# onolab-tmu/overiva

Hardware: AMD Instinct MI355X
Metric: AuxIVA iterations/sec (2048 bins x 4000 frames x 8 mics) (higher is better)
Workload: dtype f32

## Files before the change

### include/overiva_hip.h

```cpp
#ifndef OVERIVA_HIP_H
#define OVERIVA_HIP_H

#ifdef __cplusplus
extern "C" {
#endif

#define OIVA_OK 0
#define OIVA_ERR_ARG (-1)
#define OIVA_ERR_HIP (-2)
#define OIVA_ERR_STATE (-3)
#define OIVA_ERR_NUMERIC (-4)

#define OIVA_MODEL_LAPLACE 0
#define OIVA_MODEL_GAUSS 1

#define OIVA_MAX_CHANNELS 32

#define OIVA_PREC_FAST 0
#define OIVA_PREC_UPDATE_F64 1
#define OIVA_PREC_UPDATE_ROWS 2
#define OIVA_PREC_COV_F64 4
#define OIVA_PREC_PRECISE (OIVA_PREC_UPDATE_F64 | OIVA_PREC_COV_F64)

typedef struct oiva_plan oiva_plan;

int oiva_version(void);
const char *oiva_last_error(void);
int oiva_device_count(int *n);

int oiva_plan_create(oiva_plan **out, int device, int T, int F, int M, int K, int model, int F_total,
                     void *stream);
int oiva_plan_destroy(oiva_plan *p);

int oiva_plan_set_x_host(oiva_plan *p, const void *X, long long row_pitch_bytes);
int oiva_plan_set_x_dev(oiva_plan *p, const void *X_dev);
int oiva_plan_set_x_host_c128(oiva_plan *p, const void *X, long long row_pitch_bytes);

int oiva_plan_covariance(oiva_plan *p);
int oiva_plan_get_cx(oiva_plan *p, void *Cx_host, int f64);

int oiva_plan_set_w(oiva_plan *p, const void *W0_host, int f64);

int oiva_plan_iterate(oiva_plan *p, int n);

int oiva_plan_power(oiva_plan *p);
int oiva_plan_power_buffer(oiva_plan *p, int parts_per_rank, void **parts_dev, long long *bytes);
int oiva_plan_update(oiva_plan *p, const void *parts_dev, int nparts);

int oiva_plan_demix(oiva_plan *p, void *Y_host, long long row_pitch_bytes, int proj_back);
int oiva_pool_trim(void);
int oiva_plan_set_io_slab(oiva_plan *p, long long bytes);
int oiva_host_prefault(void *ptr, long long bytes);
int oiva_plan_demix_dev(oiva_plan *p, int proj_back, void **Y_dev);
int oiva_plan_demix_c128(oiva_plan *p, void *Y_host, long long row_pitch_bytes, int proj_back);

#define OIVA_XCHG_MAX_RANKS 16
#define OIVA_XCHG_HANDLE_BYTES 64
typedef struct oiva_xchg oiva_xchg;
int oiva_xchg_create(oiva_xchg **x, int device, int rank, int world, long long part_bytes);
int oiva_xchg_export(oiva_xchg *x, void *handle);
int oiva_xchg_connect(oiva_xchg *x, const void *handles);
int oiva_xchg_push(oiva_xchg *x, void *stream, const void *part_dev, long long part_bytes, int epoch);
int oiva_xchg_wait(oiva_xchg *x, void *stream, int epoch);
int oiva_xchg_gathered(oiva_xchg *x, int epoch, void **gathered);
int oiva_xchg_poll(oiva_xchg *x, int epoch, int timeout_ms, int *arrived);
int oiva_xchg_force(oiva_xchg *x, int epoch);
int oiva_xchg_destroy(oiva_xchg *x);

int oiva_plan_set_w_pca(oiva_plan *p, double *evals_host);
int oiva_plan_set_w_eig(oiva_plan *p);
int oiva_plan_get_w(oiva_plan *p, void *W_host, int f64);

int oiva_plan_sync(oiva_plan *p);
int oiva_plan_save_w(oiva_plan *p);
int oiva_plan_restore_w(oiva_plan *p);

int oiva_plan_iterate_timed(oiva_plan *p, int n, float *total_ms, float *per_kernel_ms);
#define OIVA_N_STAGES 4

int oiva_plan_get_cov_splits(oiva_plan *p, int *nsplit);
int oiva_plan_set_cov_splits(oiva_plan *p, int nsplit);
int oiva_plan_set_cov_quad(oiva_plan *p, int enable, int *active);
int oiva_plan_set_pow_splits(oiva_plan *p, int nsplit);
int oiva_plan_set_cov_hmfma(oiva_plan *p, int enable);
int oiva_plan_set_fuse_cov_update(oiva_plan *p, int enable, int *active);
int oiva_plan_set_power_reverse(oiva_plan *p, int enable);
int oiva_plan_use_graph(oiva_plan *p, int enable);
int oiva_plan_set_precision(oiva_plan *p, int flags);

struct oiva_xchg;
#define OIVA_RESIDENT_INFO 12
#define OIVA_RESIDENT_PHASES 8
int oiva_plan_set_resident(oiva_plan *p, int enable);
int oiva_plan_resident_info(oiva_plan *p, int *info );
int oiva_plan_resident_phases(oiva_plan *p, double *phase_us , int *n_iter);
int oiva_plan_resident_debug(oiva_plan *p, int timeout_ms, int stall_block);
int oiva_plan_resident_debug_from(oiva_plan *p, int timeout_ms, int stall_block, int first_stalled_iteration);
int oiva_plan_resident_loopback(oiva_plan *p, int world);
#define OIVA_RESIDENT_STAMPS 16
int oiva_plan_resident_trace(oiva_plan *p, int enable, unsigned long long *stamps_host, int *n_wg, int *n_iter);
int oiva_plan_resident_connect(oiva_plan *p, struct oiva_xchg *x);
int oiva_plan_fused_connect(oiva_plan *p, struct oiva_xchg *x);
int oiva_plan_fused_loopback(oiva_plan *p, int world);
int oiva_plan_fused_debug(oiva_plan *p, int timeout_ms, int stall);
int oiva_plan_set_resident_splits(oiva_plan *p, int nsplit);

int oiva_test_set_rinv(oiva_plan *p, const float *rinv_host );
int oiva_test_get_rinv(oiva_plan *p, float *rinv_host , float *wscale_host );
int oiva_test_run_weighted_cov(oiva_plan *p);
int oiva_test_get_v(oiva_plan *p, void *V_host , int f64);
int oiva_test_run_update(oiva_plan *p);
int oiva_test_get_what(oiva_plan *p, void *What_host , int f64);
int oiva_test_set_what(oiva_plan *p, const void *What_host, int f64);
int oiva_test_run_power(oiva_plan *p, float *p_host );
int oiva_test_get_ppart(oiva_plan *p, float *parts_host, int *nparts);
int oiva_test_power_order(int nsplit, int tcp, int cov_splits, int cov_tc, int *order);
int oiva_test_time_stage(oiva_plan *p, int stage, int reps, float *avg_ms);
int oiva_test_live_buffers(long long *count, long long *bytes);
int oiva_test_kernel_choice(int device, int T, int F, int F_total, int M, int K, int prec_flags, int quad_on, int hmfma_on,
                            int cov_splits_req, int pow_splits_req, int *out);

#define OIVA_OGIVE_DEMIX 0
#define OIVA_OGIVE_MIX 1
#define OIVA_OGIVE_SWITCHING 2
int oiva_plan_ogive_begin(oiva_plan *p, int update_mode, int model);
int oiva_plan_ogive_iterate(oiva_plan *p, int first_epoch, int n, double step_size, double tol, int *epochs_run,
                            int *converged, double *max_delta);

typedef struct oiva_batch oiva_batch;
int oiva_batch_create(oiva_batch **out, int device, int B, int T, int F, int M, int K, int model, void *stream);
int oiva_batch_destroy(oiva_batch *b);
int oiva_batch_set_x_host(oiva_batch *b, const void *X_host, int f64);
int oiva_batch_set_x_dev(oiva_batch *b, const void *X_dev);
int oiva_batch_covariance(oiva_batch *b);
int oiva_batch_set_w(oiva_batch *b, const void *W0_host, int f64);
int oiva_batch_set_w_eig(oiva_batch *b);
int oiva_batch_iterate(oiva_batch *b, int n);
int oiva_batch_demix(oiva_batch *b, void *Y_host, int f64, int proj_back);
int oiva_batch_get_w(oiva_batch *b, void *W_host, int f64);
int oiva_batch_status(oiva_batch *b, int *status);
int oiva_batch_time_stages(oiva_batch *b, int n, float *total_ms, float *per_stage_ms);

typedef int oiva_status;
oiva_status oiva_batch_get_cx(oiva_batch *b, void *Cx_host, int f64);
oiva_status oiva_batch_ogive_begin(oiva_batch *b, int update_mode, int model);
oiva_status oiva_batch_ogive_iterate(oiva_batch *b, int first_epoch, int n, double step_size, double tol, int *epochs_run,
                                     int *converged, double *max_delta);

oiva_status oiva_batch_create_ragged(oiva_batch **out, int device, int B, const int *frames, int F, int M, int K, int model,
                                     void *stream);

oiva_status oiva_batch_set_w_pca(oiva_batch *b, double *evals_host);
oiva_status oiva_batch_project_dev(oiva_batch *b, void **Xr_dev);
oiva_status oiva_batch_compose_w(oiva_batch *outer, const oiva_batch *inner);

enum {
    OIVA_ILRMA_STAGE_T = 0,
    OIVA_ILRMA_STAGE_V = 1,
    OIVA_ILRMA_STAGE_R = 2,
    OIVA_ILRMA_STAGE_COV = 3,
    OIVA_ILRMA_STAGE_UPDATE = 4,
    OIVA_ILRMA_STAGE_POWER = 5,
    OIVA_ILRMA_STAGE_NORMALISE = 6
};
oiva_status oiva_batch_ilrma_begin(oiva_batch *b, int n_components, const double *T0, const double *V0);
oiva_status oiva_batch_ilrma_stage(oiva_batch *b, int stage);
oiva_status oiva_batch_ilrma_iterate(oiva_batch *b, int n);
oiva_status oiva_batch_ilrma_get_nmf(oiva_batch *b, double *T, double *V);
oiva_status oiva_batch_ilrma_get_pr(oiva_batch *b, double *P, double *R);
oiva_status oiva_batch_ilrma_get_cov(oiva_batch *b, double *C, double *lambda);
oiva_status oiva_batch_ilrma_time_stages(oiva_batch *b, int n, float *per_stage_ms);

typedef struct oiva_stft oiva_stft;
int oiva_stft_create(oiva_stft **out, int device, int n_samples, int n_chan, int frame, int hop, const float *win_a,
                     const float *win_s);
int oiva_stft_destroy(oiva_stft *p);
int oiva_stft_shape(oiva_stft *p, int *n_frames, int *n_freq);
int oiva_stft_analysis(oiva_stft *p, const float *x_host, void *X_host, void **X_dev);
int oiva_stft_synthesis(oiva_stft *p, const void *Y_host, int n_chan, float *y_host);

typedef struct oiva_bstft oiva_bstft;
oiva_status oiva_bstft_create(oiva_bstft **out, int device, int B, const int *n_samples, int M, int frame, int hop,
                              const float *win_a, const float *win_s, void *stream);
oiva_status oiva_bstft_destroy(oiva_bstft *p);
oiva_status oiva_bstft_shape(oiva_bstft *p, int *frames, int *n_freq);
oiva_status oiva_bstft_analysis(oiva_bstft *p, const float *x_host_packed, void **X_dev);
oiva_status oiva_bstft_synthesis_dev(oiva_bstft *p, const void *Y_dev, int K, float *y_host_packed);
oiva_status oiva_bstft_phase_ms(oiva_bstft *p, float *ms);
oiva_status oiva_batch_demix_dev(oiva_batch *b, int proj_back, void **Y_dev);
oiva_status oiva_device_to_host(void *host, const void *dev, long long bytes);

typedef struct oiva_bsseval oiva_bsseval;
oiva_status oiva_bsseval_create(oiva_bsseval **out, int device, int B, const int *n_samples, int N, int filter_length,
                                int diag_only, int max_group, void *stream);
oiva_status oiva_bsseval_destroy(oiva_bsseval *p);
oiva_status oiva_bsseval_groups(oiva_bsseval *p, int *rooms_per_group);
oiva_status oiva_bsseval_set_signals(oiva_bsseval *p, const double *ref_host_packed, const double *est_host_packed);
oiva_status oiva_bsseval_stage(oiva_bsseval *p, int stage);
oiva_status oiva_bsseval_run(oiva_bsseval *p);
oiva_status oiva_bsseval_get_gram(oiva_bsseval *p, double *G_host, double *D_host, double *E_host);
oiva_status oiva_bsseval_get_filters(oiva_bsseval *p, double *C_host, double *c_host);
oiva_status oiva_bsseval_get_criteria(oiva_bsseval *p, double *sdr, double *sir, double *sar);
oiva_status oiva_bsseval_status(oiva_bsseval *p, int *status);
oiva_status oiva_bsseval_time_stages(oiva_bsseval *p, int n, float *per_stage_ms);

#ifdef __cplusplus
}
#endif
#endif
```

### overiva_amd/_lib.py

```python
import ctypes as C
import os

import numpy as np

_PKG = os.path.dirname(os.path.abspath(__file__))
LIB_PATH = os.environ.get("OIVA_LIB") or os.path.join(_PKG, "liboveriva_hip.so")

OK, ERR_ARG, ERR_HIP, ERR_STATE, ERR_NUMERIC = 0, -1, -2, -3, -4
MODEL_IDS = {"laplace": 0, "gauss": 1}
N_STAGES = 4
PREC_FAST, PREC_UPDATE_F64, PREC_UPDATE_ROWS, PREC_COV_F64 = 0, 1, 2, 4
PREC_PRECISE = PREC_UPDATE_F64 | PREC_COV_F64
PREC_MIXED = PREC_UPDATE_F64
PREC_BY_NAME = {"fast": PREC_FAST, "mixed": PREC_MIXED, "precise": PREC_PRECISE}
STAGE_NAMES = ("demix_power", "activation", "weighted_cov", "ip_update")


class HipLibraryMissing(ImportError):
    pass


class HipError(RuntimeError):
    """a HIP runtime call failed inside the library"""


_lib = None

_vp, _i, _ll, _fp = C.c_void_p, C.c_int, C.c_longlong, C.POINTER(C.c_float)

SIGNATURES = {
    "oiva_device_count": [C.POINTER(_i)],
    "oiva_plan_create": [C.POINTER(_vp), _i, _i, _i, _i, _i, _i, _i, _vp],
    "oiva_plan_destroy": [_vp],
    "oiva_plan_set_x_host": [_vp, _vp, _ll],
    "oiva_plan_set_x_dev": [_vp, _vp],
    "oiva_plan_set_x_host_c128": [_vp, _vp, _ll],
    "oiva_plan_covariance": [_vp],
    "oiva_plan_get_cx": [_vp, _vp, _i],
    "oiva_plan_set_w": [_vp, _vp, _i],
    "oiva_plan_iterate": [_vp, _i],
    "oiva_plan_power": [_vp],
    "oiva_plan_power_buffer": [_vp, _i, C.POINTER(_vp), C.POINTER(_ll)],
    "oiva_plan_update": [_vp, _vp, _i],
    "oiva_plan_demix": [_vp, _vp, _ll, _i],
    "oiva_plan_demix_dev": [_vp, _i, _vp],
    "oiva_plan_set_io_slab": [_vp, _ll],
    "oiva_host_prefault": [_vp, _ll],
    "oiva_pool_trim": [],
    "oiva_plan_demix_c128": [_vp, _vp, _ll, _i],
    "oiva_plan_set_w_pca": [_vp, _vp],
    "oiva_plan_set_w_eig": [_vp],
    "oiva_xchg_create": [_vp, _i, _i, _i, _ll],
    "oiva_xchg_export": [_vp, _vp],
    "oiva_xchg_connect": [_vp, _vp],
    "oiva_xchg_push": [_vp, _vp, _vp, _ll, _i],
    "oiva_xchg_wait": [_vp, _vp, _i],
    "oiva_xchg_gathered": [_vp, _i, _vp],
    "oiva_xchg_poll": [_vp, _i, _i, _vp],
    "oiva_xchg_force": [_vp, _i],
    "oiva_xchg_destroy": [_vp],
    "oiva_plan_get_w": [_vp, _vp, _i],
    "oiva_plan_sync": [_vp],
    "oiva_plan_save_w": [_vp],
    "oiva_plan_restore_w": [_vp],
    "oiva_plan_iterate_timed": [_vp, _i, _fp, _fp],
    "oiva_plan_get_cov_splits": [_vp, C.POINTER(_i)],
    "oiva_plan_set_cov_splits": [_vp, _i],
    "oiva_plan_set_cov_quad": [_vp, _i, C.POINTER(_i)],
    "oiva_plan_set_pow_splits": [_vp, _i],
    "oiva_plan_set_cov_hmfma": [_vp, _i],
    "oiva_plan_set_fuse_cov_update": [_vp, _i, C.POINTER(_i)],
    "oiva_plan_set_power_reverse": [_vp, _i],
    "oiva_plan_use_graph": [_vp, _i],
    "oiva_plan_set_precision": [_vp, _i],
    "oiva_plan_set_resident": [_vp, _i],
    "oiva_plan_resident_info": [_vp, C.POINTER(_i)],
    "oiva_plan_resident_phases": [_vp, C.POINTER(C.c_double), C.POINTER(_i)],
    "oiva_plan_resident_debug": [_vp, _i, _i],
    "oiva_plan_resident_debug_from": [_vp, _i, _i, _i],
    "oiva_plan_resident_loopback": [_vp, _i],
    "oiva_plan_fused_connect": [_vp, _vp],
    "oiva_plan_fused_loopback": [_vp, _i],
    "oiva_plan_fused_debug": [_vp, _i, _i],
    "oiva_plan_resident_connect": [_vp, _vp],
    "oiva_plan_resident_trace": [_vp, _i, _vp, C.POINTER(_i), C.POINTER(_i)],
    "oiva_plan_set_resident_splits": [_vp, _i],
    "oiva_test_set_rinv": [_vp, _vp],
    "oiva_test_get_rinv": [_vp, _vp, _vp],
    "oiva_test_run_weighted_cov": [_vp],
    "oiva_test_get_v": [_vp, _vp, _i],
    "oiva_test_run_update": [_vp],
    "oiva_test_get_what": [_vp, _vp, _i],
    "oiva_test_set_what": [_vp, _vp, _i],
    "oiva_test_run_power": [_vp, _vp],
    "oiva_test_get_ppart": [_vp, _vp, C.POINTER(_i)],
    "oiva_test_power_order": [_i, _i, _i, _i, C.POINTER(_i)],
    "oiva_test_time_stage": [_vp, _i, _i, _fp],
    "oiva_test_live_buffers": [C.POINTER(C.c_longlong), C.POINTER(C.c_longlong)],
    "oiva_test_kernel_choice": [_i] * 11 + [C.POINTER(_i)],
    "oiva_plan_ogive_begin": [_vp, _i, _i],
    "oiva_plan_ogive_iterate": [_vp, _i, _i, C.c_double, C.c_double, C.POINTER(_i), C.POINTER(_i), C.POINTER(C.c_double)],
    "oiva_batch_create": [C.POINTER(_vp), _i, _i, _i, _i, _i, _i, _i, _vp],
    "oiva_batch_destroy": [_vp],
    "oiva_batch_set_x_host": [_vp, _vp, _i],
    "oiva_batch_set_x_dev": [_vp, _vp],
    "oiva_batch_covariance": [_vp],
    "oiva_batch_set_w": [_vp, _vp, _i],
    "oiva_batch_set_w_eig": [_vp],
    "oiva_batch_iterate": [_vp, _i],
    "oiva_batch_demix": [_vp, _vp, _i, _i],
    "oiva_batch_get_w": [_vp, _vp, _i],
    "oiva_batch_status": [_vp, C.POINTER(_i)],
    "oiva_batch_time_stages": [_vp, _i, _fp, _fp],
    "oiva_batch_get_cx": [_vp, _vp, _i],
    "oiva_batch_ogive_begin": [_vp, _i, _i],
    "oiva_batch_ogive_iterate": [_vp, _i, _i, C.c_double, C.c_double, C.POINTER(_i), C.POINTER(_i), C.POINTER(C.c_double)],
    "oiva_batch_create_ragged": [C.POINTER(_vp), _i, _i, C.POINTER(_i), _i, _i, _i, _i, _vp],
    "oiva_batch_set_w_pca": [_vp, _vp],
    "oiva_batch_project_dev": [_vp, C.POINTER(_vp)],
    "oiva_batch_compose_w": [_vp, _vp],
    "oiva_batch_ilrma_begin": [_vp, _i, _vp, _vp],
    "oiva_batch_ilrma_stage": [_vp, _i],
    "oiva_batch_ilrma_iterate": [_vp, _i],
    "oiva_batch_ilrma_get_nmf": [_vp, _vp, _vp],
    "oiva_batch_ilrma_get_pr": [_vp, _vp, _vp],
    "oiva_batch_ilrma_get_cov": [_vp, _vp, _vp],
    "oiva_batch_ilrma_time_stages": [_vp, _i, _fp],
    "oiva_stft_create": [C.POINTER(_vp), _i, _i, _i, _i, _i, _vp, _vp],
    "oiva_stft_destroy": [_vp],
    "oiva_stft_shape": [_vp, C.POINTER(_i), C.POINTER(_i)],
    "oiva_stft_analysis": [_vp, _vp, _vp, C.POINTER(_vp)],
    "oiva_stft_synthesis": [_vp, _vp, _i, _vp],
    "oiva_bstft_create": [C.POINTER(_vp), _i, _i, C.POINTER(_i), _i, _i, _i, _vp, _vp, _vp],
    "oiva_bstft_destroy": [_vp],
    "oiva_bstft_shape": [_vp, C.POINTER(_i), C.POINTER(_i)],
    "oiva_bstft_analysis": [_vp, _vp, C.POINTER(_vp)],
    "oiva_bstft_synthesis_dev": [_vp, _vp, _i, _vp],
    "oiva_bstft_phase_ms": [_vp, _fp],
    "oiva_batch_demix_dev": [_vp, _i, C.POINTER(_vp)],
    "oiva_device_to_host": [_vp, _vp, _ll],
    "oiva_bsseval_create": [C.POINTER(_vp), _i, _i, C.POINTER(_i), _i, _i, _i, _i, _vp],
    "oiva_bsseval_destroy": [_vp],
    "oiva_bsseval_groups": [_vp, C.POINTER(_i)],
    "oiva_bsseval_set_signals": [_vp, _vp, _vp],
    "oiva_bsseval_stage": [_vp, _i],
    "oiva_bsseval_run": [_vp],
    "oiva_bsseval_get_gram": [_vp, _vp, _vp, _vp],
    "oiva_bsseval_get_filters": [_vp, _vp, _vp],
    "oiva_bsseval_get_criteria": [_vp, _vp, _vp, _vp],
    "oiva_bsseval_status": [_vp, C.POINTER(_i)],
    "oiva_bsseval_time_stages": [_vp, _i, _fp],
}


def load():
    global _lib
    if _lib is not None:
        return _lib
    try:
        import torch
    except ImportError:
        pass
    if not os.path.exists(LIB_PATH):
        raise HipLibraryMissing(
            f"{LIB_PATH} not found: the HIP extension is not built.  Run `python -m overiva_amd.build` "
            "(needs hipcc).  overiva_amd has no CPU fallback.")
    try:
        lib = C.CDLL(LIB_PATH)
    except OSError as e:
        raise HipLibraryMissing(f"cannot load {LIB_PATH}: {e}") from e
    lib.oiva_version.restype = C.c_int
    lib.oiva_version.argtypes = []
    lib.oiva_last_error.restype = C.c_char_p
    lib.oiva_last_error.argtypes = []
    for name, args in SIGNATURES.items():
        fn = getattr(lib, name)
        fn.restype = C.c_int
        fn.argtypes = args
    _lib = lib
    return lib


def require_dmabuf_ipc(what):
    import warnings

    cur = os.environ.get("HSA_ENABLE_IPC_MODE_LEGACY")
    why = None
    if cur is None or _IPC_ENV_SET_LATE:
        os.environ["HSA_ENABLE_IPC_MODE_LEGACY"] = "0"
        try:
            import torch

            started = torch.cuda.is_initialized()
        except Exception:
            started = False
        if (started and cur is None) or _IPC_ENV_SET_LATE:
            why = (f"{what}: HSA_ENABLE_IPC_MODE_LEGACY=0 was not in the environment when the GPU runtime started; "
                   "exporting device memory to other processes may fail (import overiva_amd, or export the variable, before "
                   "the first GPU call)")
    elif cur != "0":
        why = f"{what}: HSA_ENABLE_IPC_MODE_LEGACY={cur!r}; this platform's driver supports dmabuf IPC (=0) only"
    if why:
        warnings.warn(why)
    return why


_IPC_ENV_SET_LATE = False


def _set_ipc_env_at_import():
    global _IPC_ENV_SET_LATE
    if "HSA_ENABLE_IPC_MODE_LEGACY" in os.environ:
        return
    os.environ["HSA_ENABLE_IPC_MODE_LEGACY"] = "0"
    import sys

    t = sys.modules.get("torch")
    try:
        _IPC_ENV_SET_LATE = bool(t is not None and t.cuda.is_initialized())
    except Exception:
        _IPC_ENV_SET_LATE = False


def check(rc):
    if rc == OK:
        return
    msg = load().oiva_last_error().decode("utf-8", "replace")
    if rc == ERR_ARG:
        raise ValueError(msg)
    if rc == ERR_NUMERIC:
        raise np.linalg.LinAlgError(msg)
    if rc == ERR_STATE:
        raise RuntimeError(msg)
    raise HipError(msg)


class Handle:

    h = None
    _destroy = None

    def close(self):
        if self.h:
            getattr(self.lib, self._destroy)(self.h)
            self.h = None

    def __del__(self):
        try:
            self.close()
        except Exception:
            pass

    def __enter__(self):
        return self

    def __exit__(self, *exc):
        self.close()


def ptr(a):
    assert a.flags["C_CONTIGUOUS"]
    return a.ctypes.data_as(C.c_void_p)
```

### overiva_amd/csrc/kernel_choice.h

```cpp
#pragma once
#include <algorithm>
#include <functional>

#include "overiva_hip.h"

namespace oiva {

inline int ceil_div(int a, int b) { return (a + b - 1) / b; }
inline int round_up(int a, int b) { return (a + b - 1) / b * b; }

constexpr int kNarrowMax = 16;
constexpr int kWideMax = OIVA_MAX_CHANNELS;

constexpr int kBinsPerWave = 16;
constexpr int kPhasesPerWave = 4;
constexpr int kBlock = 256;
constexpr int kWaves = kBlock / 64;

enum class CovKind { Lane, Pair32, Pair64, Quad, Half16, Hmfma, Half16F64, Hmfma64, Mfma, Wide };
enum class PowKind { Lane, Mfma, Lds, Wide };
constexpr int kCovKinds = 10, kPowKinds = 4;
static_assert((int)CovKind::Wide + 1 == kCovKinds && (int)PowKind::Wide + 1 == kPowKinds, "one traits row per kind");

struct CovGeom {
    int nsplit;
    int tc;
    int kc;
    int nbg;
    CovKind kind = CovKind::Lane;
    int pad = 0;
    int part32 = 0;
};
constexpr int kPowOrderMaxSplits = 64;
struct PowOrder {
    int cs = 0;
    int q = 0;
    int first[kPowOrderMaxSplits + 1] = {};
};
inline PowOrder make_pow_order(int n, int tcp, int cs, int ctc) {
    PowOrder o;
    if (cs < 1 || cs > kPowOrderMaxSplits || ctc < 1 || tcp < 1 || n < 1) return o;
    o.cs = cs;
    for (int s = 0; s < cs; ++s) {
        const long long c = (long long)s * ctc / tcp;
        o.first[s] = c < n ? (int)c : n;
    }
    o.first[cs] = n;
    o.q = n;
    for (int s = 0; s < cs; ++s) o.q = o.first[s + 1] - o.first[s] < o.q ? o.first[s + 1] - o.first[s] : o.q;
    return o;
}
struct PowGeom {
    int nb;
    int nsplit;
    int tcp;
    int kp;
    PowKind kind = PowKind::Lane;
    int rev = 0;
    PowOrder ord{};
    int rounds = 1;
};
constexpr int kPowMaxFrames = 512;

enum class Partials { F64, Acc, F32IfPart32 };
struct CovTraits {
    bool (*supported)(int M, int K);
    int (*sources)(int K);
    int bins;
    int quantum;
    Partials partials;
    int launches;
    bool padded_x;
    bool quad_switch;
    bool fusable;
    bool update_arith;
    CovKind unit;
};
constexpr CovTraits kCovTraits[kCovKinds] = {
     {[](int M, int K) { return M >= 1 && M <= 8 && K >= 1 && K <= M; }, nullptr, kBinsPerWave, 16, Partials::F64, 1, false, false, true, false, CovKind::Lane},
     {[](int M, int K) { return M == 8 && K >= 3; }, [](int) { return 4; }, 32, 8, Partials::F64, 2, false, false, false, true, CovKind::Pair32},
     {[](int M, int) { return M == 8; }, [](int K) { return K >= 2 ? 2 : 1; }, 32, 8, Partials::F64, 2, false, false, false, false, CovKind::Pair64},
     {[](int M, int K) { return M >= 10 && M <= 16 && M % 2 == 0 && K >= 1 && K <= 4; }, [](int K) { return K >= 2 ? 2 : 1; }, kBinsPerWave, 8, Partials::F64, 2, true, true, false, true, CovKind::Quad},
     {[](int M, int K) { return M >= 10 && M <= 16 && M % 2 == 0 && K >= 1 && K <= 16; }, [](int K) { return K <= 8 ? 8 : (K <= 12 ? 12 : 16); }, 2, 16, Partials::F64, 2, true, true, false, true, CovKind::Half16},
     {[](int M, int K) { return M >= 10 && M <= 16 && M % 2 == 0 && K >= 9 && K <= 16; }, [](int K) { return K <= 8 ? 8 : (K <= 12 ? 12 : 16); }, 2, 32, Partials::F32IfPart32, 2, true, true, false, true, CovKind::Half16},
     {[](int M, int K) { return M >= 10 && M <= 16 && M % 2 == 0 && K >= 3 && K <= 16; }, [](int K) { return K <= 4 ? 4 : 8; }, 2, 16, Partials::F64, 2, true, true, false, true, CovKind::Mfma},
     {[](int M, int K) { return M == 16 && K >= 9 && K <= 16; }, [](int K) { return K <= 4 ? 4 : 8; }, 2, 32, Partials::F64, 2, true, true, false, true, CovKind::Mfma},
     {[](int M, int K) { return M >= 9 && M <= 16 && K >= 1 && K <= M; }, [](int) { return 1; }, kBinsPerWave, 4, Partials::Acc, 2, false, false, false, true, CovKind::Mfma},
     {[](int M, int K) { return M > kNarrowMax && M <= kWideMax && K >= 1 && K <= M; }, [](int K) { return std::min(K, 2); }, 1, 4, Partials::F64, 2, false, false, false, true, CovKind::Wide},
};
constexpr const CovTraits& traits(CovKind k) { return kCovTraits[(int)k]; }
constexpr bool partials_f64(const CovGeom& g, bool cov_f64) {
    return traits(g.kind).partials == Partials::F64 || (traits(g.kind).partials == Partials::Acc ? cov_f64 : !g.part32);
}

struct PowTraits {
    bool (*supported)(int M, int K);
    int (*sources)(int K);
    int bins;
    int quantum;
    bool padded_x;
    bool occupancy;
};
constexpr int pow_sources_per_pass(int , int K) {
    return K >= 3 ? 4 : (K >= 2 ? 2 : 1);
}
constexpr PowTraits kPowTraits[kPowKinds] = {
     {[](int M, int K) { return M >= 1 && M <= kNarrowMax && K >= 1 && K <= M && (M <= 8 || K <= 4); }, [](int K) { return pow_sources_per_pass(0, K); }, kBinsPerWave * kWaves, 4, false, true},
     {[](int M, int K) { return M > 8 && M <= kNarrowMax && K > 4 && K <= M; }, [](int K) { return pow_sources_per_pass(0, K); }, kBinsPerWave * kWaves, 4, true, false},
     {[](int M, int K) { return M == 16 && K > 4 && K <= M; }, [](int K) { return pow_sources_per_pass(0, K); }, kBinsPerWave * kWaves, 4, false, false},
     {[](int M, int K) { return M > kNarrowMax && M <= kWideMax && K >= 1 && K <= M; }, [](int K) { return K >= 3 ? 4 : K; }, kBinsPerWave * kWaves, 4, false, false},
};
constexpr const PowTraits& traits(PowKind k) { return kPowTraits[(int)k]; }

struct ChoiceIn {
    int T, F, F_total, M, K;
    int n_cu;
    bool cov_f64, upd_f64;
    bool cov_quad_on = true;
    bool cov_hmfma_on = true;
    bool part32 = false;
    bool kc_wide = true;
    bool power_lds = true;
};
struct Occupancy {
    std::function<int(int M, int kc, bool f64)> cov_blocks_per_cu;
    std::function<int(int M, int kp, int tcp)> pow_blocks_per_cu;
};

inline int lane_sources_per_pass(int M, int K, bool f64, bool short_axis, bool kc_wide) {
    const int regs = M * M * (f64 ? 2 : 1);
    int kc = 1;
    if (K >= 2 && regs * 2 <= 144) kc = 2;
    if (K >= 3 && regs * 4 <= 144) kc = 4;
    if (!f64 && kc_wide) {
        if (M == 7 && (K == 3 || K == 5 || K == 6 || (K == 7 && short_axis))) kc = 3;
        if (M == 5 && K >= 5) kc = 5;
    }
    return kc;
}

inline int pick_splits(int capacity, int blocks_per_split, int T, int min_frames) {
    int ns = std::max(1, capacity / std::max(1, blocks_per_split));
    ns = std::min(ns, std::max(1, T / std::max(1, min_frames)));
    return ns;
}

inline int mixed_min_splits(int capacity, int blocks_per_split, int T) {
    if (T >= 1024) return 8;
    const int one_round = std::max(1, capacity / std::max(1, blocks_per_split));
    return std::max(1, std::min(std::min(4, one_round), T / 16));
}

constexpr bool padded_channels(int M) { return M > 8 && M <= kNarrowMax && M % 2 == 1; }

inline CovKind choose_cov_kind(const ChoiceIn& c) {
    const int M = c.M, K = c.K;
    if (M > kNarrowMax) return CovKind::Wide;
    if (M <= 8) {
        if (!c.cov_f64 && traits(CovKind::Pair32).supported(M, K)) return CovKind::Pair32;
        if (c.cov_f64 && traits(CovKind::Pair64).supported(M, K)) return CovKind::Pair64;
        return CovKind::Lane;
    }
    const int Mc = M + (padded_channels(M) ? 1 : 0);
    if (!c.cov_f64 && c.cov_quad_on && traits(CovKind::Quad).supported(Mc, K) && (K <= 2 || c.upd_f64)) return CovKind::Quad;
    if (c.cov_quad_on && (c.cov_f64 ? traits(CovKind::Half16F64).supported(Mc, K) : K > 4 && traits(CovKind::Half16).supported(Mc, K))) {
        const CovKind hm = c.cov_f64 ? CovKind::Hmfma64 : CovKind::Hmfma;
        if (c.cov_hmfma_on && traits(hm).supported(Mc, K)) return hm;
        return c.cov_f64 ? CovKind::Half16F64 : CovKind::Half16;
    }
    return CovKind::Mfma;
}

inline CovGeom choose_cov(const ChoiceIn& c, const Occupancy& occ, int nsplit_req) {
    CovGeom g{};
    g.kind = choose_cov_kind(c);
    const CovTraits& t = traits(g.kind);
    const int T = c.T, F = c.F, K = c.K, n_cu = c.n_cu;
    g.pad = padded_channels(c.M) ? 1 : 0;
    g.nbg = ceil_div(F, t.bins);
    g.kc = t.sources ? t.sources(K) : lane_sources_per_pass(c.M, K, c.cov_f64, T < 1024, c.kc_wide);
    int nsplit = nsplit_req;
    switch (g.kind) {
        case CovKind::Wide:
            if (nsplit <= 0) {
                const int groups = c.F_total * ceil_div(K, g.kc);
                nsplit = 1;
                while (groups * nsplit < 2 * n_cu && ceil_div(T, nsplit + 1) >= 128) ++nsplit;
            }
            break;
        case CovKind::Quad:
            if (nsplit <= 0) {
                const int blocks = g.nbg * ceil_div(K, g.kc);
                nsplit = std::min(32, pick_splits(n_cu * 2, blocks, T, T >= 1024 ? 128 : 64));
                if (c.upd_f64) nsplit = std::max(nsplit, mixed_min_splits(n_cu * 2, blocks, T));
            }
            break;
        case CovKind::Half16:
        case CovKind::Hmfma:
        case CovKind::Half16F64:
        case CovKind::Hmfma64: {
            const bool hm = g.kind == CovKind::Hmfma || g.kind == CovKind::Hmfma64;
            if (nsplit <= 0) {
                const int chains = hm ? 8 : 4;
                nsplit = c.cov_f64 ? (!hm && g.kc == 4 && T >= 1024 ? 2 : 1) : ceil_div(T, chains * (c.upd_f64 ? 128 : 256));
                const int per_cu = hm ? (c.cov_f64 ? 2 : 3) : c.cov_f64 && g.kc == 4 ? 4 : 2;
                const int groups = hm ? F : g.nbg * ceil_div(K, g.kc);
                while (groups * nsplit < per_cu * n_cu && ceil_div(T, nsplit + 1) >= 64) ++nsplit;
            }
            if (t.partials == Partials::F32IfPart32) g.part32 = c.part32 ? 1 : 0;
            break;
        }
        case CovKind::Mfma:
            if (nsplit <= 0) {
                nsplit = ceil_div(T, 512);
                const int waves = F * ceil_div(K, 4);
                while (waves * nsplit < 2 * 4 * n_cu && ceil_div(T, nsplit + 1) >= 64) ++nsplit;
            }
            break;
        case CovKind::Lane:
        case CovKind::Pair32:
        case CovKind::Pair64:
            if (nsplit <= 0) {
                const int nz = ceil_div(K, g.kc);
                int bpc = 2;
                if (g.kind == CovKind::Lane && (bpc = occ.cov_blocks_per_cu(c.M, g.kc, c.cov_f64)) < 1) bpc = 2;
                nsplit = pick_splits(n_cu * bpc, g.nbg * nz, T, T >= 1024 ? 128 : 64);
                if (nsplit >= 12 && g.nbg * nz * nsplit >= n_cu * bpc) nsplit = nsplit * 7 / 8;
                const int cap = (g.nbg * nz * 32 >= n_cu) ? 32 : 64;
                nsplit = std::min(nsplit, cap);
                if (g.kind == CovKind::Pair32 && c.upd_f64) {
                    const int by_chain = T >= 1024 ? 8 : std::min(4, ceil_div(T, 256));
                    nsplit = std::max(nsplit, std::min(by_chain, mixed_min_splits(n_cu * bpc, g.nbg * nz, T)));
                }
            }
            break;
    }
    g.tc = round_up(ceil_div(T, nsplit), t.quantum);
    g.nsplit = ceil_div(T, g.tc);
    return g;
}

inline PowKind choose_pow_kind(const ChoiceIn& c) {
    if (c.M > kNarrowMax) return PowKind::Wide;
    if (!traits(PowKind::Mfma).supported(c.M, c.K)) return PowKind::Lane;
    if (c.power_lds && traits(PowKind::Lds).supported(c.M, c.K) && c.F >= kBinsPerWave * kWaves && c.T >= 16) return PowKind::Lds;
    return PowKind::Mfma;
}

inline PowGeom choose_pow(const ChoiceIn& c, const Occupancy& occ, int nsplit_req) {
    PowGeom g{};
    g.kind = choose_pow_kind(c);
    const PowTraits& t = traits(g.kind);
    const int T = c.T, n_cu = c.n_cu;
    g.nb = ceil_div(c.F, t.bins);
    g.kp = t.sources(c.K);
    int nsplit = nsplit_req;
    if (g.kind == PowKind::Wide) {
        const int groups = g.nb * ceil_div(c.K, g.kp);
        if (nsplit <= 0) nsplit = pick_splits(n_cu * 4, groups, T, 16);
        g.tcp = round_up(ceil_div(T, nsplit), t.quantum);
        g.nsplit = ceil_div(T, g.tcp);
        return g;
    }
    if (nsplit <= 0) {
        const int per_cu_x12 = (g.kp == 1 && c.M <= 8) ? 24 : 12;
        nsplit = pick_splits(std::max(n_cu / 2, n_cu * per_cu_x12 / std::max(c.M, 1)), g.nb, T, 32);
    }
    int tcp = round_up(ceil_div(T, nsplit), t.quantum);
    tcp = std::min(std::max(tcp, 4), kPowMaxFrames);
    g.tcp = tcp;
    g.nsplit = ceil_div(T, tcp);
    if (t.occupancy) {
        const int bpc = occ.pow_blocks_per_cu(c.M, g.kp, g.tcp);
        if (bpc > 0) g.rounds = (int)((((long long)g.nb * g.nsplit * ceil_div(c.K, g.kp)) + (long long)bpc * n_cu - 1) / ((long long)bpc * n_cu));
    }
    return g;
}

}
```

### overiva_amd/csrc/kernels_cov.hip

```cpp

#include <cstdint>
#include <cstdlib>

#include "oiva_device.h"
#include "cov_arith.h"

namespace oiva {
namespace {

constexpr int kCovUnroll = 2;
constexpr int kChunk = 16;
constexpr int kLdsStride = kBlock + 1;

template <int M, int KC, typename ACC, typename At>
__device__ __forceinline__ void reduce_and_store_at(At&& at, ACC* lds, double* __restrict__ Vpart, int F, int K, int k0) {
    constexpr int NA = M * M;
    constexpr int NACC = NA * KC;
    const int tid = threadIdx.x;
    const int bb = tid >> 4, aa = tid & 15;
    const int fo = blockIdx.x * kBinsPerWave + bb;
    double* out = Vpart + (((size_t)blockIdx.y * F + fo) * K + k0) * NA;
#pragma unroll
    for (int r0 = 0; r0 < NACC; r0 += kChunk) {
        __syncthreads();
#pragma unroll
        for (int a = 0; a < kChunk; ++a) {
            if (r0 + a < NACC) lds[a * kLdsStride + tid] = at(r0 + a);
        }
        __syncthreads();
        double s = 0.;
#pragma unroll
        for (int qq = 0; qq < 16; ++qq) s += (double)lds[aa * kLdsStride + qq * 16 + bb];
        const int e = r0 + aa;
        const int kk = e / NA;
        if (e < NACC && fo < F && k0 + kk < K) out[e] = s;
    }
}

template <int M, int KC, typename ACC>
__device__ __forceinline__ void reduce_and_store(const ACC (&acc)[KC][M * M], ACC* lds, double* __restrict__ Vpart,
                                                 int F, int K, int k0) {
    reduce_and_store_at<M, KC, ACC>([&](int e) { return acc[e / (M * M)][e % (M * M)]; }, lds, Vpart, F, K, k0);
}

template <int M, int KC, bool UNIT, typename ACC>
__global__ __launch_bounds__(kBlock) void cov_kernel(const float2* __restrict__ X, const float* __restrict__ R,
                                                     float* __restrict__ wscale, int model, int raw,
                                                     double* __restrict__ Vpart, int T, int F, int K, int tc) {
    constexpr int NA = M * M;
    __shared__ ACC lds[kChunk * kLdsStride];

    const int tid = threadIdx.x;
    const int lane = tid & 63;
    const int wave = tid >> 6;
    const int b = lane & (kBinsPerWave - 1);
    const int q = wave * kPhasesPerWave + (lane >> 4);
    const int f = blockIdx.x * kBinsPerWave + b;
    const int fc = f < F ? f : F - 1;
    const int k0 = blockIdx.z * KC;
    const int t_begin = blockIdx.y * tc;
    const int t_end = min(T, t_begin + tc);
    const int nsteps = (t_end - t_begin + 15) >> 4;

    double ginv[KC];
#pragma unroll
    for (int kk = 0; kk < KC; ++kk) ginv[kk] = 1.;
    if constexpr (!UNIT) {
#pragma unroll
        for (int kk = 0; kk < KC; ++kk) {
            const int k = k0 + kk;
            if (raw & 1) continue;
            const double gamma = gamma_of(R, T, K, k < K ? k : K - 1);
            ginv[kk] = 1. / gamma;
            if (blockIdx.x == 0 && blockIdx.y == 0 && threadIdx.x == 0 && k < K && wscale != nullptr)
                wscale[k] = model == OIVA_MODEL_LAPLACE ? (float)gamma : (float)sqrt(gamma);
        }
    }

    ACC acc[KC][NA];
#pragma unroll
    for (int kk = 0; kk < KC; ++kk)
#pragma unroll
        for (int a = 0; a < NA; ++a) acc[kk][a] = 0;

    const size_t frame_stride = (size_t)F * M;
    const float2* pbase = X + (size_t)fc * M;
    for (int i = 0; i < nsteps; i += kCovUnroll) {
        float xr[kCovUnroll][M], xi[kCovUnroll][M], rv[kCovUnroll][KC];
#pragma unroll
        for (int u = 0; u < kCovUnroll; ++u) {
            const int t = t_begin + q + 16 * (i + u);
            const int tcl = t < t_end ? t : T - 1;
            if constexpr (!UNIT) {
#pragma unroll
                for (int kk = 0; kk < KC; ++kk) {
                    const int k = k0 + kk;
                    rv[u][kk] = R[(size_t)tcl * K + (k < K ? k : K - 1)];
                }
            }
            load_x<M>(pbase + (size_t)tcl * frame_stride, xr[u], xi[u]);
        }
#pragma unroll
        for (int u = 0; u < kCovUnroll; ++u) {
            const int t = t_begin + q + 16 * (i + u);
            const bool live = t < t_end;
            ACC w[KC], ar[M], ai[M];
#pragma unroll
            for (int kk = 0; kk < KC; ++kk) {
                const bool on = live && (UNIT || k0 + kk < K);
                if constexpr (UNIT) {
                    w[kk] = on ? ACC(1) : ACC(0);
                } else if constexpr (sizeof(ACC) == 8) {
                    double rn = (double)rv[u][kk] * ginv[kk];
                    rn = rn < (double)kEpsR ? (double)kEpsR : rn;
                    w[kk] = on ? 1. / rn : 0.;
                } else {
                    w[kk] = on ? activation_weight(rv[u][kk], (float)ginv[kk]) : 0.f;
                }
            }
#pragma unroll
            for (int c = 0; c < M; ++c) {
                ar[c] = (ACC)xr[u][c];
                ai[c] = (ACC)xi[u][c];
            }
            accumulate<M, KC, UNIT, ACC>(acc, ar, ai, w);
        }
    }

    reduce_and_store<M, KC, ACC>(acc, lds, Vpart, F, K, k0);
}

constexpr int kDmaStages = 4;

typedef __attribute__((address_space(1))) const void gvoid_t;
typedef __attribute__((address_space(3))) void lvoid_t;

template <int PIECES>
__device__ __forceinline__ void ring_read(unsigned addr, float4 (&v)[PIECES]);

template <>
__device__ __forceinline__ void ring_read<4>(unsigned addr, float4 (&v)[4]) {
    asm volatile(
        "s_waitcnt vmcnt(12)\n\t"
        "ds_read_b128 %0, %4\n\t"
        "ds_read_b128 %1, %4 offset:1024\n\t"
        "ds_read_b128 %2, %4 offset:2048\n\t"
        "ds_read_b128 %3, %4 offset:3072\n\t"
        "s_waitcnt lgkmcnt(0)"
        : "=&v"(v[0]), "=&v"(v[1]), "=&v"(v[2]), "=&v"(v[3])
        : "v"(addr)
        : "memory");
}
template <>
__device__ __forceinline__ void ring_read<2>(unsigned addr, float4 (&v)[2]) {
    asm volatile(
        "s_waitcnt vmcnt(6)\n\t"
        "ds_read_b128 %0, %2\n\t"
        "ds_read_b128 %1, %2 offset:1024\n\t"
        "s_waitcnt lgkmcnt(0)"
        : "=&v"(v[0]), "=&v"(v[1])
        : "v"(addr)
        : "memory");
}

#ifdef OIVA_COVDMA_TRACE
__device__ long long g_cd_trace[8 * 2048];
#define CD_STAMP(slot)                                                                                                            \
    do {                                                                                                                          \
        if (threadIdx.x == 0 && blockIdx.z == 0) g_cd_trace[(blockIdx.y * gridDim.x + blockIdx.x) * 8 + (slot)] = wall_clock64(); \
    } while (0)
#else
#define CD_STAMP(slot) \
    do {               \
    } while (0)
#endif

template <int M, int KC>
__global__ __launch_bounds__(kBlock, 2) void cov_dma_kernel(const float2* __restrict__ X, const float* __restrict__ R,
                                                            float* __restrict__ wscale, int model, int raw,
                                                            double* __restrict__ Vpart, int T, int F, int K, int tc) {
    constexpr int NA = M * M;
    constexpr int PIECES = M / 2;
    constexpr int STAGE = PIECES * 64;
    static_assert(M % 2 == 0 && (PIECES == 2 || PIECES == 4), "LDS-DMA path: M in {4, 8}");
    __shared__ float4 ring[kWaves * kDmaStages * STAGE];
    static_assert(sizeof(float4) * kWaves * kDmaStages * STAGE >= sizeof(float) * kChunk * kLdsStride,
                  "reduction scratch aliases the ring");

    const int tid = threadIdx.x;
    const int lane = tid & 63;
    const int wave = __builtin_amdgcn_readfirstlane(tid >> 6);
    const int b = lane & (kBinsPerWave - 1);
    const int ql = lane >> 4;
    const int q = wave * kPhasesPerWave + ql;
    const int f = blockIdx.x * kBinsPerWave + b;
    const int fc = f < F ? f : F - 1;
    const int k0 = blockIdx.z * KC;
    const int t_begin = blockIdx.y * tc;
    const int t_end = min(T, t_begin + tc);
    const int nsteps = (t_end - t_begin + 15) >> 4;

    constexpr bool kPacked = KC == 2;
    float acc[kPacked ? 1 : KC][kPacked ? 1 : NA];
    PkAcc2<M> pacc;
    if constexpr (kPacked) {
        pacc.clear();
    } else {
#pragma unroll
        for (int kk = 0; kk < KC; ++kk)
#pragma unroll
            for (int a = 0; a < NA; ++a) acc[kk][a] = 0.f;
    }

    float ginv[KC];
    float4* wring = ring + wave * kDmaStages * STAGE;
    const unsigned rd_base = (unsigned)(uintptr_t)(wring) + lane * 16;
    const size_t frame_stride = (size_t)F * M;
    const float2* pbase = X + (size_t)fc * M;

    auto issue = [&](int i, int s) {
        const int t = t_begin + q + 16 * i;
        const int tcl = (i < nsteps && t < t_end) ? t : T - 1;
        const float2* src = pbase + (size_t)tcl * frame_stride;
#pragma unroll
        for (int j = 0; j < PIECES; ++j)
            __builtin_amdgcn_global_load_lds((gvoid_t*)(src + 2 * j), (lvoid_t*)(wring + s * STAGE + j * 64), 16, 0, 0);
    };
    const float m0 = ql == 0 ? 1.f : 0.f, m1 = ql == 1 ? 1.f : 0.f, m2 = ql == 2 ? 1.f : 0.f, m3 = ql == 3 ? 1.f : 0.f;
    auto consume = [&](int i, int s) {
        const int tw = min(t_begin + wave * kPhasesPerWave + 16 * i, T);
        const float* rp = R + (size_t)tw * K;
        float w[KC];
#pragma unroll
        for (int kk = 0; kk < KC; ++kk) {
            const int k = k0 + kk < K ? k0 + kk : K - 1;
            const float r = m0 * rp[k] + m1 * rp[K + k] + m2 * rp[2 * K + k] + m3 * rp[3 * K + k];
            const float live = (t_begin + wave * kPhasesPerWave + 16 * i + ql < t_end && k0 + kk < K) ? 1.f : 0.f;
            w[kk] = activation_weight(r, ginv[kk]) * live;
        }
        float4 v[PIECES];
        ring_read<PIECES>(rd_base + s * STAGE * 16, v);
#if defined(OIVA_COVDMA_ABLATE) && (OIVA_COVDMA_ABLATE & 1)
        if constexpr (kPacked) {
            if (v[0].x == 12345.f) pacc.add(reinterpret_cast<const v2f(&)[M]>(v), v2f{w[0], w[1]});
            return;
        }
#endif
        if constexpr (kPacked) {
            v2f x[M];
#pragma unroll
            for (int j = 0; j < PIECES; ++j) {
                x[2 * j] = v2f{v[j].x, v[j].y};
                x[2 * j + 1] = v2f{v[j].z, v[j].w};
            }
            pacc.add(x, v2f{w[0], w[1]});
        } else {
            float xr[M], xi[M];
#pragma unroll
            for (int j = 0; j < PIECES; ++j) {
                xr[2 * j] = v[j].x;
                xi[2 * j] = v[j].y;
                xr[2 * j + 1] = v[j].z;
                xi[2 * j + 1] = v[j].w;
            }
            accumulate<M, KC, false, float>(acc, xr, xi, w);
        }
    };

    CD_STAMP(0);
    issue(0, 0);
    issue(1, 1);
    issue(2, 2);
#pragma unroll
    for (int kk = 0; kk < KC; ++kk) {
        const int k = k0 + kk;
        ginv[kk] = 1.f;
        if (raw & 1) continue;
#if defined(OIVA_COVDMA_ABLATE) && (OIVA_COVDMA_ABLATE & 4)
        const float gamma = R[k < K ? k : K - 1] + 1.f;
#else
        const float gamma = (float)gamma_of(R, T, K, k < K ? k : K - 1);
#endif
        ginv[kk] = 1.f / gamma;
        if (blockIdx.x == 0 && blockIdx.y == 0 && threadIdx.x == 0 && k < K && wscale != nullptr)
            wscale[k] = model == OIVA_MODEL_LAPLACE ? gamma : sqrtf(gamma);
    }

    CD_STAMP(1);
    int i = 0;
    for (; i + 4 <= nsteps; i += 4) {
        issue(i + 3, 3); consume(i, 0);
        issue(i + 4, 0); consume(i + 1, 1);
        issue(i + 5, 1); consume(i + 2, 2);
        issue(i + 6, 2); consume(i + 3, 3);
    }
    if (i < nsteps) { issue(i + 3, 3); consume(i, 0); }
    if (i + 1 < nsteps) { issue(i + 4, 0); consume(i + 1, 1); }
    if (i + 2 < nsteps) { issue(i + 5, 1); consume(i + 2, 2); }
    CD_STAMP(2);
    asm volatile("s_waitcnt vmcnt(0)" ::: "memory");
    CD_STAMP(3);
#if defined(OIVA_COVDMA_ABLATE) && (OIVA_COVDMA_ABLATE & 2)
    if constexpr (kPacked) {
        if (pacc.at(0) == 12345.f) Vpart[0] = 1.;
        return;
    }
#endif
    if constexpr (kPacked)
        reduce_and_store_at<M, KC, float>([&](int e) { return pacc.at(e); }, reinterpret_cast<float*>(ring), Vpart, F, K, k0);
    else
        reduce_and_store<M, KC, float>(acc, reinterpret_cast<float*>(ring), Vpart, F, K, k0);
    CD_STAMP(4);
}

template <typename ACC>
using CovKernel = void (*)(const float2*, const float*, float*, int, int, double*, int, int, int, int);

template <int M, typename ACC, typename Fn>
hipError_t dispatch_kc(int kc, bool unit, Fn&& fn) {
    constexpr int kRegs = M * M * (int)(sizeof(ACC) / 4);
    if (unit) return kc == 1 ? fn((CovKernel<ACC>)cov_kernel<M, 1, true, ACC>, 1) : hipErrorInvalidValue;
    if constexpr ((M == 4 || M == 8) && sizeof(ACC) == 4) {
        switch (kc) {
            case 1:
                return fn((CovKernel<ACC>)cov_dma_kernel<M, 1>, 1);
            case 2:
                if constexpr (kRegs * 2 <= 144) return fn((CovKernel<ACC>)cov_dma_kernel<M, 2>, 2);
                break;
            case 4:
                if constexpr (kRegs * 4 <= 144) return fn((CovKernel<ACC>)cov_dma_kernel<M, 4>, 4);
                break;
        }
        return hipErrorInvalidValue;
    }
    switch (kc) {
        case 1:
            return fn((CovKernel<ACC>)cov_kernel<M, 1, false, ACC>, 1);
        case 2:
            if constexpr (kRegs * 2 <= 144) return fn((CovKernel<ACC>)cov_kernel<M, 2, false, ACC>, 2);
            break;
        case 4:
            if constexpr (kRegs * 4 <= 144) return fn((CovKernel<ACC>)cov_kernel<M, 4, false, ACC>, 4);
            break;
        case 3:
            if constexpr (M == 7 && sizeof(ACC) == 4) return fn((CovKernel<ACC>)cov_kernel<M, 3, false, ACC>, 3);
            break;
        case 5:
            if constexpr (M == 5 && sizeof(ACC) == 4) return fn((CovKernel<ACC>)cov_kernel<M, 5, false, ACC>, 5);
            break;
    }
    return hipErrorInvalidValue;
}

template <typename ACC, typename Fn>
hipError_t dispatch_cov(int M, int kc, bool unit, Fn&& fn) {
    switch (M) {
        case 1: return dispatch_kc<1, ACC>(kc, unit, fn);
        case 2: return dispatch_kc<2, ACC>(kc, unit, fn);
        case 3: return dispatch_kc<3, ACC>(kc, unit, fn);
        case 4: return dispatch_kc<4, ACC>(kc, unit, fn);
        case 5: return dispatch_kc<5, ACC>(kc, unit, fn);
        case 6: return dispatch_kc<6, ACC>(kc, unit, fn);
        case 7: return dispatch_kc<7, ACC>(kc, unit, fn);
        case 8: return dispatch_kc<8, ACC>(kc, unit, fn);
    }
    return hipErrorInvalidValue;
}

}

__global__ __launch_bounds__(kBlock) void pad_channels_kernel(const float2* __restrict__ X, float2* __restrict__ Xpad, long long n, int M) {
    const long long e = (long long)blockIdx.x * kBlock + threadIdx.x;
    if (e >= n) return;
    const long long tf = e / (M + 1);
    const int c = (int)(e - tf * (M + 1));
    Xpad[e] = c < M ? X[tf * M + c] : make_float2(0.f, 0.f);
}

hipError_t launch_pad_channels(hipStream_t s, const float2* X, float2* Xpad, long long n_tf, int M) {
    const long long n = n_tf * (M + 1);
    pad_channels_kernel<<<dim3((unsigned)((n + kBlock - 1) / kBlock)), dim3(kBlock), 0, s>>>(X, Xpad, n, M);
    return hipGetLastError();
}

hipError_t launch_cov(hipStream_t s, const float2* X, const float2* Xpad, const float* R, float* Wt, float* wscale, int model, int raw,
                      void* Vpart, bool f64, int T, int F, int M, int K, const CovGeom& g) {
    const CovTraits& t = traits(g.kind);
    if (g.tc % t.quantum != 0 || (g.pad && Xpad == nullptr)) return hipErrorInvalidValue;
    const float2* Xv = g.pad && t.padded_x ? Xpad : X;
    const int Mp = g.pad && t.padded_x ? M + 1 : M;
    double* const V64 = static_cast<double*>(Vpart);
    switch (g.kind) {
        case CovKind::Wide: return launch_cov_wide(s, X, R, Wt, wscale, model, raw, V64, T, F, M, K, g);
        case CovKind::Half16: return launch_cov_half16(s, Xv, R, Wt, wscale, model, raw, V64, T, F, Mp, M, K, g);
        case CovKind::Hmfma: {
            const hipError_t e = launch_cov_half16_weights(s, R, Wt, wscale, model, raw, T, K);
            return e != hipSuccess ? e : launch_cov_hmfma(s, Xv, Wt, V64, T, F, Mp, M, K, g);
        }
        case CovKind::Half16F64: return launch_cov_half16_f64(s, Xv, R, Wt, wscale, model, raw, V64, T, F, Mp, M, K, g);
        case CovKind::Hmfma64: {
            const hipError_t e = launch_cov_half16_weights_f64(s, R, Wt, wscale, model, raw, T, K);
            return e != hipSuccess ? e : launch_cov_hmfma64(s, Xv, reinterpret_cast<const double*>(Wt), V64, T, F, Mp, M, K, g);
        }
        case CovKind::Quad: return launch_cov_quad(s, Xv, R, Wt, wscale, model, raw, V64, T, F, Mp, M, K, g);
        case CovKind::Mfma: return launch_cov_mfma(s, X, R, Wt, wscale, model, raw, Vpart, f64, T, F, M, K, g.nsplit, g.tc);
        case CovKind::Pair32: return launch_cov_pair32(s, X, R, Wt, wscale, model, raw, V64, T, F, M, K, g);
        case CovKind::Pair64: return launch_cov_pair64(s, X, R, Wt, wscale, model, raw, V64, T, F, M, K, g);
        case CovKind::Lane: break;
    }
    const int kc = R == nullptr ? 1 : g.kc;
    if (f64)
        return dispatch_cov<double>(M, kc, R == nullptr, [&](CovKernel<double> kern, int KC) {
            kern<<<dim3(g.nbg, g.nsplit, (K + KC - 1) / KC), dim3(kBlock), 0, s>>>(X, R, wscale, model, raw,
                                                                                 static_cast<double*>(Vpart), T, F, K, g.tc);
            return hipGetLastError();
        });
    return dispatch_cov<float>(M, kc, R == nullptr, [&](CovKernel<float> kern, int KC) {
        return launch_dominant(kern, dim3(g.nbg, g.nsplit, (K + KC - 1) / KC), dim3(kBlock), 0, s, X, R, wscale, model, raw,
                               static_cast<double*>(Vpart), T, F, K, g.tc);
    });
}

hipError_t cov_blocks_per_cu(int M, int kc, bool f64, int* n) {
    if (f64)
        return dispatch_cov<double>(M, kc, false, [&](CovKernel<double> kern, int) {
            return hipOccupancyMaxActiveBlocksPerMultiprocessor(n, kern, kBlock, 0);
        });
    return dispatch_cov<float>(M, kc, false, [&](CovKernel<float> kern, int) {
        return hipOccupancyMaxActiveBlocksPerMultiprocessor(n, kern, kBlock, 0);
    });
}

#ifdef OIVA_COVDMA_TRACE
extern "C" int oiva_debug_covdma_trace(long long* out) { return (int)hipMemcpyFromSymbol(out, HIP_SYMBOL(g_cd_trace), sizeof(g_cd_trace)); }
#endif

}
```

### overiva_amd/csrc/kernels_demix.hip

```cpp
#include "oiva_device.h"
#include "demix_arith.h"

namespace oiva {
namespace {

constexpr int kPowUnroll = 2;

template <int M, int KP>
__global__ __launch_bounds__(kBlock) void power_kernel(const float2* __restrict__ X, const float2* __restrict__ What,
                                                       float* __restrict__ Ppart, int T, int F, int K, int tcp, int rev, PowOrder ord) {
    extern __shared__ __attribute__((aligned(16))) float sp[];
    const int tid = threadIdx.x;
    const int lane = tid & 63;
    const int wave = tid >> 6;
    const int b = lane & 15;
    const int q = lane >> 4;
    const int f = (blockIdx.x * kWaves + wave) * kBinsPerWave + b;
    const bool fvalid = f < F;
    const int fc = fvalid ? f : F - 1;
    const int k0 = blockIdx.z * KP;
    const int chunk = ord.cs > 0 ? power_chunk_tail_first(blockIdx.y, gridDim.y, ord) : (int)blockIdx.y;
    const int t_begin = chunk * tcp;
    const int t_end = min(T, t_begin + tcp);
    const int len = t_end - t_begin;
    const int nsteps = (len + 3) >> 2;
    const int ngroups = (nsteps + kPowUnroll - 1) / kPowUnroll;

    float wr[KP][M], wi[KP][M];
    load_wconj<M, KP>(What, fc, k0, K, wr, wi);

    const size_t frame_stride = (size_t)F * M;
    const float2* pbase = X + (size_t)fc * M;
    for (int g = 0; g < ngroups; ++g) {
        const int i = (rev ? ngroups - 1 - g : g) * kPowUnroll;
        float xr[kPowUnroll][M], xi[kPowUnroll][M];
#pragma unroll
        for (int u = 0; u < kPowUnroll; ++u) {
            const int tl = 4 * (i + u) + q;
            const int t = tl < len ? t_begin + tl : T - 1;
            load_x<M>(pbase + (size_t)t * frame_stride, xr[u], xi[u]);
        }
#pragma unroll
        for (int u = 0; u < kPowUnroll; ++u) {
            const int tl = 4 * (i + u) + q;
            const bool live = tl < len;
#pragma unroll
            for (int kk = 0; kk < KP; ++kk) {
                float yr, yi;
                demix_one<M>(wr[kk], wi[kk], xr[u], xi[u], yr, yi);
                float pw = fmaf(yr, yr, yi * yi);
                pw = fvalid ? pw : 0.f;
                pw = row16_sum(pw);
                if (b == 0 && live) sp[(wave * tcp + tl) * KP + kk] = pw;
            }
        }
    }
    __syncthreads();
    for (int e = tid; e < len * KP; e += kBlock) {
        const int tl = e / KP, kk = e - tl * KP;
        float s = sp[(0 * tcp + tl) * KP + kk];
#pragma unroll
        for (int w = 1; w < kWaves; ++w) s += sp[(w * tcp + tl) * KP + kk];
        if (k0 + kk < K) Ppart[((size_t)blockIdx.x * T + t_begin + tl) * K + k0 + kk] = s;
    }
}

template <int M, int KP>
__global__ __launch_bounds__(kBlock) void stats_kernel(const float2* __restrict__ X, const float2* __restrict__ What,
                                                       float* __restrict__ Spart, int T, int F, int K, int tc) {
    __shared__ float lds[3 * KP * (kBlock + 1)];
    const int tid = threadIdx.x;
    const int b = tid & 15;
    const int q = tid >> 4;
    const int f = blockIdx.x * kBinsPerWave + b;
    const int fc = f < F ? f : F - 1;
    const int k0 = blockIdx.z * KP;
    const int t_begin = blockIdx.y * tc;
    const int t_end = min(T, t_begin + tc);
    const int nsteps = (t_end - t_begin + 15) >> 4;

    float wr[KP][M], wi[KP][M];
    load_wconj<M, KP>(What, fc, k0, K, wr, wi);
    float nr[KP], ni[KP], dn[KP];
#pragma unroll
    for (int kk = 0; kk < KP; ++kk) nr[kk] = ni[kk] = dn[kk] = 0.f;

    const size_t frame_stride = (size_t)F * M;
    const float2* px = X + ((size_t)(t_begin + q) * F + fc) * M;
    for (int i = 0; i < nsteps; ++i) {
        const int t = t_begin + q + 16 * i;
        if (t < t_end) {
            float xr[M], xi[M];
            load_x<M>(px, xr, xi);
#pragma unroll
            for (int kk = 0; kk < KP; ++kk) {
                float yr, yi;
                demix_one<M>(wr[kk], wi[kk], xr, xi, yr, yi);
                nr[kk] = fmaf(xr[0], yr, fmaf(xi[0], yi, nr[kk]));
                ni[kk] = fmaf(xr[0], yi, fmaf(-xi[0], yr, ni[kk]));
                dn[kk] = fmaf(yr, yr, fmaf(yi, yi, dn[kk]));
            }
        }
        px += 16 * frame_stride;
    }
#pragma unroll
    for (int kk = 0; kk < KP; ++kk) {
        lds[(3 * kk + 0) * (kBlock + 1) + tid] = nr[kk];
        lds[(3 * kk + 1) * (kBlock + 1) + tid] = ni[kk];
        lds[(3 * kk + 2) * (kBlock + 1) + tid] = dn[kk];
    }
    __syncthreads();
    for (int e = tid; e < 16 * 3 * KP; e += kBlock) {
        const int bb = e / (3 * KP), v = e - bb * (3 * KP);
        float s = 0.f;
#pragma unroll
        for (int qq = 0; qq < 16; ++qq) s += lds[v * (kBlock + 1) + qq * 16 + bb];
        const int fo = blockIdx.x * kBinsPerWave + bb;
        const int kk = v / 3, c = v - 3 * kk;
        if (fo < F && k0 + kk < K) Spart[(((size_t)blockIdx.y * F + fo) * K + k0 + kk) * 3 + c] = s;
    }
}

template <int M, int KP>
__global__ __launch_bounds__(kBlock) void write_kernel(const float2* __restrict__ X, const float2* __restrict__ What,
                                                       const float* __restrict__ Spart, int nsplit,
                                                       float2* __restrict__ Y, int T, int F, int K, int tc) {
    const int tid = threadIdx.x;
    const int b = tid & 15;
    const int q = tid >> 4;
    const int f = blockIdx.x * kBinsPerWave + b;
    if (f >= F) return;
    const int k0 = blockIdx.z * KP;
    const int t_begin = blockIdx.y * tc;
    const int t_end = min(T, t_begin + tc);

    float wr[KP][M], wi[KP][M];
    load_wconj<M, KP>(What, f, k0, K, wr, wi);
    if (Spart != nullptr) {
#pragma unroll
        for (int kk = 0; kk < KP; ++kk) {
            if (k0 + kk < K) {
                double sr = 0., si = 0., sd = 0.;
                for (int s = 0; s < nsplit; ++s) {
                    const float* p = Spart + (((size_t)s * F + f) * K + k0 + kk) * 3;
                    sr += p[0];
                    si += p[1];
                    sd += p[2];
                }
                float zr = 1.f, zi = 0.f;
                if (sd > 0.) {
                    zr = (float)(sr / sd);
                    zi = (float)(si / sd);
                }
#pragma unroll
                for (int m = 0; m < M; ++m) {
                    const float a = wr[kk][m], c = wi[kk][m];
                    wr[kk][m] = a * zr + c * zi;
                    wi[kk][m] = c * zr - a * zi;
                }
            }
        }
    }
    const size_t frame_stride = (size_t)F * M;
    const float2* px = X + ((size_t)(t_begin + q) * F + f) * M;
    for (int t = t_begin + q; t < t_end; t += 16) {
        float xr[M], xi[M];
        load_x<M>(px, xr, xi);
#pragma unroll
        for (int kk = 0; kk < KP; ++kk) {
            float yr, yi;
            demix_one<M>(wr[kk], wi[kk], xr, xi, yr, yi);
            if (k0 + kk < K) Y[((size_t)t * F + f) * K + k0 + kk] = make_float2(yr, yi);
        }
        px += 16 * frame_stride;
    }
}

template <int M, int KP>
hipError_t launch_power_one(hipStream_t s, const float2* X, const float2* What, float* Ppart, int T, int F, int K,
                            const PowGeom& g) {
    dim3 grid(g.nb, g.nsplit, (K + KP - 1) / KP);
    const size_t shmem = (size_t)kWaves * g.tcp * KP * sizeof(float);
    hipLaunchKernelGGL((power_kernel<M, KP>), grid, dim3(kBlock), shmem, s, X, What, Ppart, T, F, K, g.tcp, g.rev, g.ord);
    return hipGetLastError();
}

template <int M, int KP>
hipError_t launch_stats_one(hipStream_t s, const float2* X, const float2* What, float* Spart, int T, int F, int K,
                            const CovGeom& g) {
    dim3 grid(g.nbg, g.nsplit, (K + KP - 1) / KP);
    hipLaunchKernelGGL((stats_kernel<M, KP>), grid, dim3(kBlock), 0, s, X, What, Spart, T, F, K, g.tc);
    return hipGetLastError();
}

template <int M, int KP>
hipError_t launch_write_one(hipStream_t s, const float2* X, const float2* What, const float* Spart, int nsplit,
                            float2* Y, int T, int F, int K) {
    const int tc = 256;
    dim3 grid((F + kBinsPerWave - 1) / kBinsPerWave, (T + tc - 1) / tc, (K + KP - 1) / KP);
    hipLaunchKernelGGL((write_kernel<M, KP>), grid, dim3(kBlock), 0, s, X, What, Spart, nsplit, Y, T, F, K, tc);
    return hipGetLastError();
}

#define OIVA_DISPATCH_M(CALL)            \
    switch (M) {                         \
        case 1: CALL(1); break;          \
        case 2: CALL(2); break;          \
        case 3: CALL(3); break;          \
        case 4: CALL(4); break;          \
        case 5: CALL(5); break;          \
        case 6: CALL(6); break;          \
        case 7: CALL(7); break;          \
        case 8: CALL(8); break;          \
        case 9: CALL(9); break;          \
        case 10: CALL(10); break;        \
        case 11: CALL(11); break;        \
        case 12: CALL(12); break;        \
        case 13: CALL(13); break;        \
        case 14: CALL(14); break;        \
        case 15: CALL(15); break;        \
        case 16: CALL(16); break;        \
    }

}

hipError_t pow_blocks_per_cu(int M, int kp, int tcp, int* n) {
    const size_t shmem = (size_t)kWaves * tcp * kp * sizeof(float);
#define CALL(MM)                                                                                                   \
    if (kp == 1) return hipOccupancyMaxActiveBlocksPerMultiprocessor(n, power_kernel<MM, 1>, kBlock, shmem);       \
    if (kp == 2) return hipOccupancyMaxActiveBlocksPerMultiprocessor(n, power_kernel<MM, 2>, kBlock, shmem);       \
    if (kp == 4) return hipOccupancyMaxActiveBlocksPerMultiprocessor(n, power_kernel<MM, 4>, kBlock, shmem);
    OIVA_DISPATCH_M(CALL)
#undef CALL
    return hipErrorInvalidValue;
}

hipError_t launch_power(hipStream_t s, const float2* X, const float2* Xpad, const float2* What, float* Ppart, int T, int F, int M,
                        int K, const PowGeom& g) {
    if (!traits(g.kind).supported(M, K)) return hipErrorInvalidValue;
    switch (g.kind) {
        case PowKind::Wide: return launch_power_wide(s, X, What, Ppart, T, F, M, K, g);
        case PowKind::Mfma: return Xpad ? launch_power_mfma(s, Xpad, What, Ppart, T, F, M, M + 1, K) : launch_power_mfma(s, X, What, Ppart, T, F, M, M, K);
        case PowKind::Lds: return launch_power_lds(s, X, What, Ppart, T, F, M, K);
        case PowKind::Lane: break;
    }
#define CALL(MM)                                                                                        \
    if (g.kp == 1) return launch_power_one<MM, 1>(s, X, What, Ppart, T, F, K, g);                       \
    if (g.kp == 2) return launch_power_one<MM, 2>(s, X, What, Ppart, T, F, K, g);                       \
    if (g.kp == 4) return launch_power_one<MM, 4>(s, X, What, Ppart, T, F, K, g);
    OIVA_DISPATCH_M(CALL)
#undef CALL
    return hipErrorInvalidValue;
}

hipError_t launch_demix_stats(hipStream_t s, const float2* X, const float2* What, float* Spart, int T, int F, int M,
                              int K, const CovGeom& g) {
    if (M > kNarrowMax) return launch_demix_stats_wide(s, X, What, Spart, T, F, M, K, g);
#define CALL(MM) return launch_stats_one<MM, 2>(s, X, What, Spart, T, F, K, g);
    OIVA_DISPATCH_M(CALL)
#undef CALL
    return hipErrorInvalidValue;
}

hipError_t launch_demix_write(hipStream_t s, const float2* X, const float2* What, const float* Spart, int nsplit,
                              float2* Y, int T, int F, int M, int K) {
    if (M > kNarrowMax) return launch_demix_write_wide(s, X, What, Spart, nsplit, Y, T, F, M, K);
#define CALL(MM) return launch_write_one<MM, 2>(s, X, What, Spart, nsplit, Y, T, F, K);
    OIVA_DISPATCH_M(CALL)
#undef CALL
    return hipErrorInvalidValue;
}

}
```

### overiva_amd/csrc/oiva_device.h

```cpp
#pragma once
#include "oiva_internal.h"

#include <type_traits>
#include <utility>

namespace oiva {

constexpr float kEpsR = 1e-15f;

__device__ __forceinline__ double block_sum(double v, double* scratch) {
#pragma unroll
    for (int off = 32; off > 0; off >>= 1) v += __shfl_xor(v, off, 64);
    const int wave = threadIdx.x >> 6;
    __syncthreads();
    if ((threadIdx.x & 63) == 0) scratch[wave] = v;
    __syncthreads();
    double s = 0.;
#pragma unroll
    for (int w = 0; w < kWaves; ++w) s += scratch[w];
    return s;
}

__device__ __forceinline__ double gamma_of(const float* __restrict__ R, int T, int K, int k) {
    const double* S = reinterpret_cast<const double*>(R + rsum_offset_floats(T, K));
    const int nblk = rsum_blocks(T);
    double s = 0.;
    for (int b = 0; b < nblk; ++b) s += S[(size_t)b * K + k];
    return s / (double)T;
}

__device__ __forceinline__ float activation_weight(float r, float ginv) {
    float rn = r * ginv;
    rn = rn < kEpsR ? kEpsR : rn;
    return 1.f / rn;
}

template <int M>
__device__ __forceinline__ void load_x(const float2* __restrict__ p, float (&xr)[M], float (&xi)[M]) {
    if constexpr (M % 2 == 0) {
        const float4* p4 = reinterpret_cast<const float4*>(p);
#pragma unroll
        for (int i = 0; i < M / 2; ++i) {
            const float4 v = p4[i];
            xr[2 * i] = v.x;
            xi[2 * i] = v.y;
            xr[2 * i + 1] = v.z;
            xi[2 * i + 1] = v.w;
        }
    } else {
#pragma unroll
        for (int i = 0; i < M; ++i) {
            const float2 v = p[i];
            xr[i] = v.x;
            xi[i] = v.y;
        }
    }
}

using f32x4 = __attribute__((ext_vector_type(4))) float;
using f64x4 = __attribute__((ext_vector_type(4))) double;

template <typename REAL>
struct Mfma;
template <>
struct Mfma<float> {
    using acc_t = f32x4;
    static __device__ __forceinline__ acc_t run(float a, float b, acc_t c) {
        return __builtin_amdgcn_mfma_f32_16x16x4f32(a, b, c, 0, 0, 0);
    }
    static __device__ __forceinline__ int row(int lane, int r) { return (lane >> 4) * 4 + r; }
};
template <>
struct Mfma<double> {
    using acc_t = f64x4;
    static __device__ __forceinline__ acc_t run(double a, double b, acc_t c) {
        return __builtin_amdgcn_mfma_f64_16x16x4f64(a, b, c, 0, 0, 0);
    }
    static __device__ __forceinline__ int row(int lane, int r) { return (lane >> 4) + 4 * r; }
};

template <int CTRL>
__device__ __forceinline__ int dpp32(int x) {
    return __builtin_amdgcn_update_dpp(0, x, CTRL, 0xF, 0xF, true);
}
template <int CTRL>
__device__ __forceinline__ float dpp(float v) { return __int_as_float(dpp32<CTRL>(__float_as_int(v))); }
template <int CTRL>
__device__ __forceinline__ unsigned dpp(unsigned v) { return (unsigned)dpp32<CTRL>((int)v); }
template <int CTRL>
__device__ __forceinline__ double dpp(double v) {
    return __hiloint2double(dpp32<CTRL>(__double2hiint(v)), dpp32<CTRL>(__double2loint(v)));
}
template <int CTRL, int BANKS>
__device__ __forceinline__ int dpp32_banks(int old, int x) {
    return __builtin_amdgcn_update_dpp(old, x, CTRL, 0xF, BANKS, false);
}
template <int CTRL, int BANKS>
__device__ __forceinline__ float dpp_banks(float old, float v) {
    return __int_as_float(dpp32_banks<CTRL, BANKS>(__float_as_int(old), __float_as_int(v)));
}
template <int CTRL, int BANKS>
__device__ __forceinline__ double dpp_banks(double old, double v) {
    return __hiloint2double(dpp32_banks<CTRL, BANKS>(__double2hiint(old), __double2hiint(v)),
                            dpp32_banks<CTRL, BANKS>(__double2loint(old), __double2loint(v)));
}
template <typename F, int... I>
__device__ __forceinline__ void static_for_impl(F&& f, std::integer_sequence<int, I...>) {
    (f(std::integral_constant<int, I>{}), ...);
}
template <int N, typename F>
__device__ __forceinline__ void static_for(F&& f) {
    static_for_impl(f, std::make_integer_sequence<int, N>{});
}
constexpr int kDppXor1 = 0xB1;
constexpr int kDppXor2 = 0x4E;
constexpr int kDppRor4 = 0x124;
constexpr int kDppRor8 = 0x128;
constexpr int kDppHalfMirror = 0x141;
__device__ __forceinline__ float swapsum16(float v) {
    auto r = __builtin_amdgcn_permlane16_swap(__float_as_uint(v), __float_as_uint(v), false, false);
    return __uint_as_float(r[0]) + __uint_as_float(r[1]);
}
__device__ __forceinline__ float swapsum32(float v) {
    auto r = __builtin_amdgcn_permlane32_swap(__float_as_uint(v), __float_as_uint(v), false, false);
    return __uint_as_float(r[0]) + __uint_as_float(r[1]);
}
__device__ __forceinline__ double swapsum16(double v) {
    auto h = __builtin_amdgcn_permlane16_swap((unsigned)__double2hiint(v), (unsigned)__double2hiint(v), false, false);
    auto l = __builtin_amdgcn_permlane16_swap((unsigned)__double2loint(v), (unsigned)__double2loint(v), false, false);
    return __hiloint2double((int)h[0], (int)l[0]) + __hiloint2double((int)h[1], (int)l[1]);
}
__device__ __forceinline__ double swapsum32(double v) {
    auto h = __builtin_amdgcn_permlane32_swap((unsigned)__double2hiint(v), (unsigned)__double2hiint(v), false, false);
    auto l = __builtin_amdgcn_permlane32_swap((unsigned)__double2loint(v), (unsigned)__double2loint(v), false, false);
    return __hiloint2double((int)h[0], (int)l[0]) + __hiloint2double((int)h[1], (int)l[1]);
}
__device__ __forceinline__ unsigned swapmax16(unsigned v) {
    auto r = __builtin_amdgcn_permlane16_swap(v, v, false, false);
    return r[0] > r[1] ? r[0] : r[1];
}
__device__ __forceinline__ unsigned swapmax32(unsigned v) {
    auto r = __builtin_amdgcn_permlane32_swap(v, v, false, false);
    return r[0] > r[1] ? r[0] : r[1];
}


}
```

### overiva_amd/csrc/plan.hip

```cpp
#include <algorithm>
#include <cmath>
#include <cstdint>
#include <cstdlib>
#include <cstring>
#include <mutex>
#include <string>
#include <vector>

#include "host_io.h"
#include "host_util.h"
#include "oiva_internal.h"
#include "resident.h"

using namespace oiva;

namespace {

constexpr int kGraphBatch = 8;
constexpr int kGraphMaxIters = 32;
constexpr int kGraphCache = 6;

}

struct oiva_plan {
    int device = 0;
    int T = 0, F = 0, M = 0, K = 0, model = 0, F_total = 0;
    HandleStream stream;
    DeviceArena mem;

    const float2* X = nullptr;
    float2* X_owned = nullptr;
    float2* X_pad = nullptr;
    float2* What = nullptr;
    double2* What64 = nullptr;
    bool what64_valid = false;
    double* Cx = nullptr;
    void* Vpart = nullptr;
    float* Ppart = nullptr;
    int ppart_alloc = 0;
    float* Plocal = nullptr;
    void* Wwide = nullptr;
    float* R = nullptr;
    float* wscale = nullptr;
    float* Spart = nullptr;
    float2* Y = nullptr;
    double2* scratch_c = nullptr;
    double* scratch_p = nullptr;

    CovGeom cov{};
    bool cov_quad_on = true;
    bool cov_hmfma_on = true;
    bool fuse_cov_update = false;
    int power_reverse = 1;
    CovGeom stg{};
    PowGeom pw{};
    int n_cu = 256;
    int vpart_splits_alloc = 0;

    bool have_x = false, have_cx = false, have_w = false;
    bool pad_valid = false;
    bool wscale_pending = false;
    int raw_weights = 0;
    int prec = 0;
    bool upd_f64() const { return prec & OIVA_PREC_UPDATE_F64; }
    bool cov_f64() const { return prec & OIVA_PREC_COV_F64; }
    bool vpart_f64() const { return partials_f64(cov, cov_f64()); }
    int use_graph = 0;
    OgiveState og{};
    bool og_ready = false;
    int og_mode = 0, og_model = 0;
    hipGraphExec_t og_graph = nullptr;
    int og_graph_n = 0, og_graph_phase = -1;
    double og_graph_mu = 0., og_graph_tol = 0.;
    ResidentGeom rg{};
    bool res_ok = false;
    bool res_on = false;
    void* res_block = nullptr;
    float* res_parts = nullptr;
    float* res_psum = nullptr;
    double* res_vpart = nullptr;
    double* res_rsum = nullptr;
    float2* res_wpub = nullptr;
    unsigned* res_flags = nullptr;
    float2* res_what = nullptr;
    double2* res_what64 = nullptr;
    unsigned* res_code_host = nullptr;
    unsigned long long* res_stamps = nullptr;
    size_t res_block_bytes = 0;
    unsigned res_epoch = 0;
    int res_last_code = 0, res_launches = 0, res_fallbacks = 0, res_stamped = 0;
    int res_timeout_ms = 0, res_stall = -1, res_stall_iter = 0;
    char* res_loop_buf = nullptr;
    bool res_loopback = false;
    bool res_trace = false;
    unsigned long long* res_trace_buf = nullptr;
    int res_trace_iters = 0;
    char* res_gath[OIVA_XCHG_MAX_RANKS] = {};
    int res_rank = 0, res_world = 1;
    bool fx_on = false, fx_loopback = false;
    char* fx_gath[OIVA_XCHG_MAX_RANKS] = {};
    int fx_rank = 0, fx_world = 1;
    int fx_nblk_own = 1, fx_nblk_peer = 1;
    char* fx_loop_buf = nullptr;
    unsigned* fx_state = nullptr;
    unsigned* fx_flag_host = nullptr;
    int fx_timeout_ms = 0, fx_stall = 0;
    HandleStream io_stream;
    double2* io_c128[kHostRingSlots] = {};
    size_t io_c128_bytes = 0;
    size_t io_slab_bytes = 0;
    float2* ck_what = nullptr;
    double2* ck_what64 = nullptr;
    bool ck_valid = false, ck_what64_valid = false;
    GraphCache graphs{kGraphCache};
};

namespace {

ChoiceIn choice_in(const oiva_plan* p) {
    static const bool kc_wide = [] { const char* v = std::getenv("OIVA_COV_KC_WIDE"); return !(v && v[0] == '0'); }();
    static const bool power_lds = [] { const char* v = std::getenv("OIVA_POWER_LDS"); return !(v && v[0] == '0'); }();
    const char* pv = std::getenv("OIVA_HMFMA_PART32");
    ChoiceIn c{};
    c.T = p->T, c.F = p->F, c.F_total = p->F_total, c.M = p->M, c.K = p->K, c.n_cu = p->n_cu;
    c.cov_f64 = p->cov_f64(), c.upd_f64 = p->upd_f64();
    c.cov_quad_on = p->cov_quad_on, c.cov_hmfma_on = p->cov_hmfma_on;
    c.part32 = pv && pv[0] == '1';
    c.kc_wide = kc_wide, c.power_lds = power_lds;
    return c;
}
Occupancy device_occupancy(int* asked = nullptr) {
    Occupancy o;
    o.cov_blocks_per_cu = [asked](int M, int kc, bool f64) {
        int n = 0;
        if (cov_blocks_per_cu(M, kc, f64, &n) != hipSuccess) n = 0;
        if (asked) asked[0] = n;
        return n;
    };
    o.pow_blocks_per_cu = [asked](int M, int kp, int tcp) {
        int n = 0;
        if (pow_blocks_per_cu(M, kp, tcp, &n) != hipSuccess) n = 0;
        if (asked) asked[1] = n;
        return n;
    };
    return o;
}
void choose_cov_geom(oiva_plan* p, int nsplit_req) { p->cov = choose_cov(choice_in(p), device_occupancy(), nsplit_req); }
void choose_pow_geom(oiva_plan* p, int nsplit_req) { p->pw = choose_pow(choice_in(p), device_occupancy(), nsplit_req); }

void choose_stats_geom(oiva_plan* p) {
    CovGeom g;
    if (p->M > kNarrowMax) {
        g.nbg = ceil_div(p->F_total, 64);
        g.kc = 2;
        const int nsplit = std::min(16, pick_splits(p->n_cu * 4, g.nbg * ceil_div(p->K, g.kc), p->T, 128));
        g.tc = round_up(ceil_div(p->T, nsplit), 16);
        g.nsplit = ceil_div(p->T, g.tc);
        p->stg = g;
        return;
    }
    p->stg = stats_geom(p->T, p->F, p->K, p->n_cu);
}

int drop_graph(oiva_plan* p) {
    const int rc = p->graphs.clear();
    if (rc) return rc;
    if (p->og_graph) {
        OIVA_TRY_HIP(hipGraphExecDestroy(p->og_graph));
        p->og_graph = nullptr;
    }
    return OIVA_OK;
}

size_t vpart_floats(const oiva_plan* p, int nsplit) { return (size_t)nsplit * p->F * p->K * p->M * p->M; }

int ensure_vpart(oiva_plan* p) {
    if (p->cov.nsplit > p->vpart_splits_alloc) {
        p->mem.release(&p->Vpart);
        OIVA_TRY_HIP(p->mem.take_one(&p->Vpart, (vpart_floats(p, p->cov.nsplit) + 2) * sizeof(double)));
        p->vpart_splits_alloc = p->cov.nsplit;
    }
    return OIVA_OK;
}

int stage_power(oiva_plan* p) {
    PowGeom g = p->pw;
    if (p->power_reverse) {
        g.rev = 1;
        if (g.rounds > 1 || p->power_reverse > 1) g.ord = make_pow_order(g.nsplit, g.tcp, p->cov.nsplit, p->cov.tc);
    }
    OIVA_TRY_HIP(launch_power(p->stream, p->X, p->X_pad && p->pad_valid ? p->X_pad : nullptr, p->What, p->Ppart, p->T, p->F, p->M, p->K, g));
    return OIVA_OK;
}
int stage_activation(oiva_plan* p, const float* parts, int nparts) {
    if (p->fx_on && parts == p->Ppart) {
        OIVA_TRY_HIP(launch_activation_xchg(p->stream, parts, nparts, p->fx_gath, p->fx_rank, p->fx_world, p->fx_loopback ? (p->fx_stall ? 2 : 1) : 0, p->fx_nblk_own, p->fx_nblk_peer, p->fx_state + 16,
                                       p->fx_state, (long long)(p->fx_timeout_ms > 0 ? p->fx_timeout_ms : 2000) * 100000, p->R, p->T, p->K,
                                       p->model, p->F_total));
        p->raw_weights = 0;
        return OIVA_OK;
    }
    OIVA_TRY_HIP(launch_activation(p->stream, parts, nparts, p->R, p->T, p->K, p->model, p->F_total));
    p->raw_weights = 0;
    return OIVA_OK;
}
int stage_cov(oiva_plan* p) {
    OIVA_TRY_HIP(launch_cov(p->stream, p->X, p->X_pad, p->R, p->Wwide ? static_cast<float*>(p->Wwide) : p->Plocal , p->wscale, p->model,
                       p->raw_weights, p->Vpart, p->cov_f64(), p->T, p->F, p->M, p->K, p->cov));
    p->wscale_pending = !p->raw_weights;
    return OIVA_OK;
}
int stage_update(oiva_plan* p, bool init_only) {
    UpdateArgs a;
    a.What = p->What;
    a.What64 = p->upd_f64() ? p->What64 : nullptr;
    a.Cx = p->Cx;
    a.Vpart = p->Vpart;
    a.vpart_f64 = p->vpart_f64() ? 1 : 0;
    a.wscale = (!init_only && p->wscale_pending) ? p->wscale : nullptr;
    a.nsplit = p->cov.nsplit;
    a.T = p->T;
    a.F = p->F;
    a.M = p->M;
    a.K = p->K;
    a.init_only = init_only ? 1 : 0;
    a.use_double = p->upd_f64() ? 1 : 0;
    a.layout = (p->prec & OIVA_PREC_UPDATE_ROWS) ? 1 : 0;
    OIVA_TRY_HIP(launch_update(p->stream, a));
    p->what64_valid = a.What64 != nullptr;
    if (!init_only) p->wscale_pending = false;
    return OIVA_OK;
}

bool cov_update_applies(const oiva_plan* p) {
    return traits(p->cov.kind).fusable && p->fuse_cov_update && !p->cov_f64() && !p->raw_weights && !(p->prec & OIVA_PREC_UPDATE_ROWS) && p->K < p->M &&
           cov_update_supported(p->M, p->K, p->T, p->F, p->cov.nsplit, p->cov.tc);
}
int stage_cov_update(oiva_plan* p) {
    UpdateArgs a;
    a.What = p->What;
    a.What64 = p->upd_f64() ? p->What64 : nullptr;
    a.Cx = p->Cx;
    a.Vpart = nullptr;
    a.vpart_f64 = 1;
    a.wscale = nullptr;
    a.nsplit = p->cov.nsplit;
    a.T = p->T, a.F = p->F, a.M = p->M, a.K = p->K;
    a.init_only = 0;
    a.use_double = p->upd_f64() ? 1 : 0;
    a.layout = 0;
    OIVA_TRY_HIP(launch_cov_update(p->stream, p->X, p->R, p->wscale, p->model, a, p->cov.tc));
    p->what64_valid = a.What64 != nullptr;
    p->wscale_pending = false;
    return OIVA_OK;
}

int one_iteration(oiva_plan* p) {
    int rc;
    if ((rc = stage_power(p))) return rc;
    if ((rc = stage_activation(p, p->Ppart, p->pw.nb))) return rc;
    if (cov_update_applies(p)) return stage_cov_update(p);
    if ((rc = stage_cov(p))) return rc;
    return stage_update(p, false);
}

constexpr int kResidentStampIters = 256;

bool resident_applies(const oiva_plan* p) {
    const bool arith_ok = !p->cov_f64() || (p->M == 4 && p->upd_f64());
    return p->M <= kNarrowMax && p->res_on && p->res_ok && (p->F == p->F_total || p->res_world > 1) && arith_ok && !p->raw_weights && !p->wscale_pending;
}

int resident_alloc(oiva_plan* p) {
    if (p->res_block) return OIVA_OK;
    const ResidentGeom& g = p->rg;
    const size_t Fp = (size_t)g.NB * 16, NA = (size_t)p->M * p->M, K = p->K;
    auto up = [](size_t b) { return (b + 255) & ~(size_t)255; };
    const size_t b_parts = up((size_t)2 * g.NB * g.NS * g.TW * K * sizeof(float));
    const size_t b_psum = up((size_t)2 * g.NS * g.TW * K * sizeof(float));
    const size_t b_vpart = up(((size_t)g.NS * Fp * K * NA + 2) * sizeof(double));
    const size_t b_rsum = up((size_t)g.NB * ((g.NS * K + 1) & ~(size_t)1) * sizeof(double) + 16);
    const size_t b_wpub = up(Fp * K * p->M * sizeof(float2));
    const size_t b_flags = up((16 + (size_t)g.NB * g.NS) * sizeof(unsigned));
    const size_t b_stamps = up((size_t)kResidentStampIters * kResidentStamps * sizeof(unsigned long long));
    const size_t total = b_parts + b_psum + b_vpart + b_rsum + b_wpub + b_flags + b_stamps;
    if (!p->res_what) OIVA_TRY_HIP(p->mem.take_one(&p->res_what, (size_t)p->F * NA * sizeof(float2)));
    if (!p->res_what64) OIVA_TRY_HIP(p->mem.take_one(&p->res_what64, (size_t)p->F * NA * sizeof(double2)));
    if (!p->res_code_host) OIVA_TRY_HIP(p->mem.take_one(&p->res_code_host, sizeof(unsigned), Mem::pinned));
    OIVA_TRY_HIP(p->mem.take_one(&p->res_block, total));
    OIVA_TRY_HIP(hipMemsetAsync(p->res_block, 0, total, p->stream));
    char* c = static_cast<char*>(p->res_block);
    p->res_parts = reinterpret_cast<float*>(c);
    c += b_parts;
    p->res_psum = reinterpret_cast<float*>(c);
    c += b_psum;
    p->res_vpart = reinterpret_cast<double*>(c);
    c += b_vpart;
    p->res_rsum = reinterpret_cast<double*>(c);
    c += b_rsum;
    p->res_wpub = reinterpret_cast<float2*>(c);
    c += b_wpub;
    p->res_flags = reinterpret_cast<unsigned*>(c);
    c += b_flags;
    p->res_stamps = reinterpret_cast<unsigned long long*>(c);
    p->res_block_bytes = total;
    p->res_epoch = 0;
    return OIVA_OK;
}

int run_resident(oiva_plan* p, int n, bool* ran) {
    *ran = false;
    int rc = resident_alloc(p);
    if (rc) return rc;
    const ResidentGeom& g = p->rg;
    ResidentArgs a{};
    a.X = p->X;
    a.What = p->What;
    a.What64 = p->upd_f64() ? p->What64 : nullptr;
    a.What_out = p->res_what;
    a.What64_out = p->upd_f64() ? p->res_what64 : nullptr;
    a.what64_valid = p->what64_valid ? 1 : 0;
    a.Cx = p->Cx;
    a.parts = p->res_parts;
    a.psum = p->res_psum;
    a.vpart = p->res_vpart;
    a.rsum = p->res_rsum;
    a.wpub = p->res_wpub;
    a.ctrl = p->res_flags;
    a.xcc_tab = p->res_flags + 16;
    a.stamps = n <= kResidentStampIters ? p->res_stamps : nullptr;
    a.stamp_all = 0;
    if (p->res_trace && n <= 64) {
        const size_t bytes = (size_t)g.NB * g.NS * n * kResidentStamps * sizeof(unsigned long long);
        p->mem.release(&p->res_trace_buf);
        OIVA_TRY_HIP(p->mem.take_one(&p->res_trace_buf, bytes));
        OIVA_TRY_HIP(hipMemsetAsync(p->res_trace_buf, 0, bytes, p->stream));
        a.stamps = p->res_trace_buf;
        a.stamp_all = 1;
        p->res_trace_iters = n;
    }
    a.T = p->T;
    a.F = p->F;
    a.F_total = p->F_total;
    a.model = p->model;
    a.g = g;
    a.n_iter = n;
    a.epoch0 = p->res_epoch;
    a.timeout_ticks = (long long)(p->res_timeout_ms > 0 ? p->res_timeout_ms : (p->res_world > 1 && !p->res_loopback ? 2000 : 250)) * 100000;
    a.stall_block = p->res_stall;
    a.stall_iter = p->res_stall_iter;
    a.rank = p->res_rank;
    a.world = p->res_world;
    a.loopback = p->res_loopback ? 1 : 0;
    for (int r = 0; r < OIVA_XCHG_MAX_RANKS; ++r) a.gath[r] = reinterpret_cast<float*>(p->res_gath[r]);
    OIVA_TRY_HIP(launch_resident(p->stream, a, p->M, p->K, p->upd_f64(), p->cov_f64()));
    p->res_launches++;
    OIVA_TRY_HIP(hipMemcpyAsync(p->res_code_host, a.ctrl, sizeof(unsigned), hipMemcpyDeviceToHost, p->stream));
    OIVA_TRY_HIP(hipStreamSynchronize(p->stream));
    const unsigned code = *p->res_code_host;
    if (code != 0) {
        OIVA_TRY_HIP(hipMemset(p->res_block, 0, p->res_block_bytes));
        p->res_epoch = 0;
        p->res_last_code = (int)code;
        p->res_fallbacks++;
        p->res_on = false;
        p->res_stamped = 0;
        if (p->res_world > 1)
            return fail_with(OIVA_ERR_STATE, "the X-resident launch gave up waiting (code " + std::to_string(code) +
                                        "): a rank did not deliver its parts in time; W_hat of this rank is unchanged");
        return OIVA_OK;
    }
    if (!p->graphs.empty() || p->og_graph) {
        int rcg = drop_graph(p);
        if (rcg) return rcg;
    }
    std::swap(p->What, p->res_what);
    if (a.What64_out) std::swap(p->What64, p->res_what64);
    p->og.What = p->What;
    p->og.What64 = p->What64;
    p->res_epoch += (unsigned)n;
    p->res_stamped = (a.stamps && !a.stamp_all) ? n : 0;
    p->what64_valid = a.What64 != nullptr;
    p->wscale_pending = false;
    *ran = true;
    return OIVA_OK;
}

int graph_for(oiva_plan* p, int iters, hipGraphExec_t* out) {
    return p->graphs.get(p->stream, iters, [&] {
        const bool pending = p->wscale_pending;
        const int raw = p->raw_weights;
        int r = OIVA_OK;
        for (int i = 0; i < iters && r == OIVA_OK; ++i) r = one_iteration(p);
        p->wscale_pending = pending;
        p->raw_weights = raw;
        return r;
    }, out);
}

int build_graphs(oiva_plan* p) {
    hipGraphExec_t g = nullptr;
    return graph_for(p, kGraphBatch, &g);
}

int upload_what(oiva_plan* p, const std::vector<double2>& wh) {
    std::vector<float2> w32(wh.size());
    for (size_t i = 0; i < wh.size(); ++i) w32[i] = make_float2((float)wh[i].x, (float)wh[i].y);
    OIVA_TRY_HIP(hipStreamSynchronize(p->stream));
    OIVA_TRY_HIP(hipMemcpy(p->What, w32.data(), w32.size() * sizeof(float2), hipMemcpyHostToDevice));
    OIVA_TRY_HIP(hipMemcpy(p->What64, wh.data(), wh.size() * sizeof(double2), hipMemcpyHostToDevice));
    p->what64_valid = true;
    return OIVA_OK;
}

int download_what(oiva_plan* p, std::vector<double2>& wh) {
    wh.resize((size_t)p->F * p->M * p->M);
    OIVA_TRY_HIP(hipStreamSynchronize(p->stream));
    if (p->what64_valid) {
        OIVA_TRY_HIP(hipMemcpy(wh.data(), p->What64, wh.size() * sizeof(double2), hipMemcpyDeviceToHost));
        return OIVA_OK;
    }
    std::vector<float2> w32(wh.size());
    OIVA_TRY_HIP(hipMemcpy(w32.data(), p->What, w32.size() * sizeof(float2), hipMemcpyDeviceToHost));
    for (size_t i = 0; i < wh.size(); ++i) wh[i] = make_double2(w32[i].x, w32[i].y);
    return OIVA_OK;
}

int ensure_pad(oiva_plan* p) {
    if (p->X_pad == nullptr || p->pad_valid) return OIVA_OK;
    OIVA_TRY_HIP(launch_pad_channels(p->stream, p->X, p->X_pad, (long long)p->T * p->F, p->M));
    p->pad_valid = true;
    return OIVA_OK;
}

int check_ready(oiva_plan* p) {
    OIVA_NEED(p != nullptr, OIVA_ERR_ARG, "null plan");
    OIVA_NEED(p->have_x, OIVA_ERR_STATE, "X not set (oiva_plan_set_x_host/_dev)");
    OIVA_NEED(p->have_cx, OIVA_ERR_STATE, "input covariance not computed (oiva_plan_covariance)");
    OIVA_NEED(p->have_w, OIVA_ERR_STATE, "demixing matrix not set (oiva_plan_set_w)");
    return OIVA_OK;
}

int install_x(oiva_plan* p, const float2* X) {
    if (p->X != X) {
        OIVA_TRY_HIP(hipStreamSynchronize(p->stream));
        const int rc = drop_graph(p);
        if (rc) return rc;
    }
    p->X = X;
    p->have_x = true;
    p->have_cx = false;
    p->pad_valid = false;
    return OIVA_OK;
}
template <class Change>
int change_geometry(oiva_plan* p, Change&& change) {
    DeviceGuard guard(p->device);
    OIVA_TRY_HIP(hipStreamSynchronize(p->stream));
    int rc = drop_graph(p);
    if (rc || (rc = change())) return rc;
    return ensure_vpart(p);
}

}

extern "C" {

int oiva_version(void) { return 100; }

int oiva_device_count(int* n) {
    OIVA_NEED(n != nullptr, OIVA_ERR_ARG, "null pointer");
    OIVA_TRY_HIP(hipGetDeviceCount(n));
    return OIVA_OK;
}

int oiva_plan_create(oiva_plan** out, int device, int T, int F, int M, int K, int model, int F_total, void* stream) {
    OIVA_NEED(out != nullptr, OIVA_ERR_ARG, "null out pointer");
    *out = nullptr;
    OIVA_NEED(T >= 1 && F >= 1, OIVA_ERR_ARG, "T and F must be >= 1");
    OIVA_NEED(M >= 1 && M <= OIVA_MAX_CHANNELS, OIVA_ERR_ARG, "number of channels must be in 1..32");
    OIVA_NEED(K >= 1 && K <= M, OIVA_ERR_ARG, "n_src must be in 1..n_chan");
    OIVA_NEED(model == OIVA_MODEL_LAPLACE || model == OIVA_MODEL_GAUSS, OIVA_ERR_ARG, "unknown model");
    OIVA_NEED(F_total >= F, OIVA_ERR_ARG, "F_total must be >= F");
    int ndev = 0;
    OIVA_TRY_HIP(hipGetDeviceCount(&ndev));
    OIVA_NEED(device >= 0 && device < ndev, OIVA_ERR_ARG, "no such device");
    DeviceGuard guard(device);

    oiva_plan* p = new oiva_plan();
    p->device = p->mem.device = device;
    p->T = T;
    p->F = F;
    p->M = M;
    p->K = K;
    p->model = model;
    p->F_total = F_total;
    const hipError_t es = p->stream.open(stream, 0);
    if (es != hipSuccess) {
        oiva_plan_destroy(p);
        return fail_with(OIVA_ERR_HIP, std::string("hipStreamCreate: ") + hipGetErrorString(es));
    }
    {
        hipDeviceProp_t prop;
        if (hipGetDeviceProperties(&prop, device) == hipSuccess && prop.multiProcessorCount > 0)
            p->n_cu = prop.multiProcessorCount;
    }
    if (M > 8 && M <= kNarrowMax && M % 2 == 1) {
        const hipError_t ep = p->mem.take_one(&p->X_pad, (size_t)T * F * (M + 1) * sizeof(float2));
        if (ep != hipSuccess) {
            oiva_plan_destroy(p);
            return fail_with(OIVA_ERR_HIP, std::string("allocation of the padded copy of X failed: ") + hipGetErrorString(ep));
        }
    }
    {
        const char* v = std::getenv("OIVA_COV_HMFMA");
        p->cov_hmfma_on = !(v && v[0] == '0');
        const char* u = std::getenv("OIVA_COV_UPDATE");
        p->fuse_cov_update = u && u[0] == '1';
        const char* r = std::getenv("OIVA_POWER_REVERSE");
        p->power_reverse = (r && r[0] == '0') ? 0 : (r && r[0] == '2') ? 2 : 1;
    }
    choose_cov_geom(p, 0);
    choose_pow_geom(p, 0);
    choose_stats_geom(p);
    p->res_ok = resident_geometry(T, F, M, K, p->n_cu, 0, &p->rg);
    const size_t nTK = (size_t)T * K;
    const size_t nFMM = (size_t)F * M * M;
    DeviceArena& mem = p->mem;
    mem.take(&p->What, nFMM * sizeof(float2));
    mem.take(&p->What64, nFMM * sizeof(double2));
    mem.take(&p->Cx, nFMM * sizeof(double));
    mem.take(&p->Ppart, (size_t)p->pw.nb * nTK * sizeof(float));
    p->ppart_alloc = p->pw.nb;
    mem.take(&p->Plocal, std::max(nTK, ((size_t)T + 1) * 32) * sizeof(float));
    if (M > kNarrowMax) mem.take(&p->Wwide, nTK * sizeof(double));
    mem.take(&p->R, r_buffer_bytes(T, K));
    if (mem.ok()) mem.note(hipMemset(p->R, 0, r_buffer_bytes(T, K)));
    mem.take(&p->wscale, (size_t)K * sizeof(float));
    mem.take(&p->Spart, (size_t)p->stg.nsplit * F * K * 3 * sizeof(float));
    mem.take(&p->scratch_c, (size_t)K * nFMM * sizeof(double2));
    mem.take(&p->scratch_p, std::max((size_t)K * nFMM, nTK) * sizeof(double));
    if (mem.ok()) mem.note(p->stream.add_events(2));
    if (!mem.ok()) {
        const hipError_t e = mem.status();
        oiva_plan_destroy(p);
        return fail_with(OIVA_ERR_HIP, std::string("allocation failed: ") + hipGetErrorString(e));
    }
    int rc = ensure_vpart(p);
    if (rc) {
        oiva_plan_destroy(p);
        return rc;
    }
    *out = p;
    return OIVA_OK;
}

int oiva_plan_destroy(oiva_plan* p) {
    if (!p) return OIVA_OK;
    DeviceGuard guard(p->device);
    if (p->stream) (void)hipStreamSynchronize(p->stream);
    if (p->io_stream) (void)hipStreamSynchronize(p->io_stream);
    (void)p->graphs.clear();
    if (p->og_graph) (void)hipGraphExecDestroy(p->og_graph);
    p->mem.clear();
    p->io_stream.close();
    p->stream.close();
    delete p;
    return OIVA_OK;
}

int oiva_plan_set_x_host(oiva_plan* p, const void* X, long long row_pitch_bytes) {
    OIVA_NEED(p && X, OIVA_ERR_ARG, "null argument");
    DeviceGuard guard(p->device);
    const size_t row = (size_t)p->F * p->M * sizeof(float2);
    const size_t pitch = row_pitch_bytes > 0 ? (size_t)row_pitch_bytes : row;
    OIVA_NEED(pitch >= row, OIVA_ERR_ARG, "row pitch smaller than one frame of this plan's bins");
    if (!p->X_owned) OIVA_TRY_HIP(p->mem.take_one(&p->X_owned, row * p->T, Mem::pooled));
    OIVA_TRY_HIP(hipStreamSynchronize(p->stream));
    OIVA_TRY_HIP(hipMemcpy2D(p->X_owned, row, X, pitch, row, p->T, hipMemcpyHostToDevice));
    return install_x(p, p->X_owned);
}

int oiva_plan_set_x_host_c128(oiva_plan* p, const void* X, long long row_pitch_bytes) {
    OIVA_NEED(p && X, OIVA_ERR_ARG, "null argument");
    DeviceGuard guard(p->device);
    const size_t n_row = (size_t)p->F * p->M;
    const size_t row = n_row * sizeof(double2);
    const size_t pitch = row_pitch_bytes > 0 ? (size_t)row_pitch_bytes : row;
    OIVA_NEED(pitch >= row, OIVA_ERR_ARG, "row pitch smaller than one frame of this plan's bins");
    if (!p->X_owned) OIVA_TRY_HIP(p->mem.take_one(&p->X_owned, n_row * sizeof(float2) * p->T, Mem::pooled));
    OIVA_TRY_HIP(hipStreamSynchronize(p->stream));
    OIVA_TRY_HIP(staged_copy_c128(true, p->stream, const_cast<void*>(X), pitch, p->X_owned, n_row, p->T, kStageBytes, p->device, Mem::pooled));
    return install_x(p, p->X_owned);
}

int oiva_plan_set_x_dev(oiva_plan* p, const void* X_dev) {
    OIVA_NEED(p && X_dev, OIVA_ERR_ARG, "null argument");
    OIVA_NEED(((uintptr_t)X_dev & 15) == 0, OIVA_ERR_ARG, "device X must be 16-byte aligned");
    DeviceGuard guard(p->device);
    return install_x(p, (const float2*)X_dev);
}

int oiva_plan_covariance(oiva_plan* p) {
    OIVA_NEED(p, OIVA_ERR_ARG, "null plan");
    OIVA_NEED(p->have_x, OIVA_ERR_STATE, "X not set");
    DeviceGuard guard(p->device);
    p->pad_valid = false;
    int rcp = ensure_pad(p);
    if (rcp) return rcp;
    CovGeom g = p->cov;
    g.kind = traits(p->cov.kind).unit;
    g.kc = 1;
    g.part32 = 0;
    OIVA_TRY_HIP(launch_cov(p->stream, p->X, p->X_pad, nullptr, nullptr, nullptr, p->model, 0, p->Vpart, p->cov_f64(), p->T, p->F, p->M, 1, g));
    OIVA_TRY_HIP(launch_sum_parts(p->stream, p->Vpart, partials_f64(g, p->cov_f64()), g.nsplit, p->Cx, (long long)p->F * p->M * p->M, 1. / (double)p->T));
    p->have_cx = true;
    return OIVA_OK;
}

int oiva_plan_get_cx(oiva_plan* p, void* Cx_host, int f64) {
    OIVA_NEED(p && Cx_host, OIVA_ERR_ARG, "null argument");
    OIVA_NEED(p->have_cx, OIVA_ERR_STATE, "input covariance not computed");
    DeviceGuard guard(p->device);
    const size_t n = (size_t)p->F * p->M * p->M;
    OIVA_TRY_HIP(launch_unpack_herm(p->stream, p->Cx, p->scratch_c, f64 != 0, p->F, p->M));
    OIVA_TRY_HIP(hipStreamSynchronize(p->stream));
    OIVA_TRY_HIP(hipMemcpy(Cx_host, p->scratch_c, n * (f64 ? sizeof(double2) : sizeof(float2)), hipMemcpyDeviceToHost));
    return OIVA_OK;
}

int oiva_plan_set_w(oiva_plan* p, const void* W0_host, int f64) {
    OIVA_NEED(p, OIVA_ERR_ARG, "null plan");
    OIVA_NEED(p->have_cx, OIVA_ERR_STATE, "input covariance not computed (needed for the orthogonality constraint)");
    DeviceGuard guard(p->device);
    const int M = p->M, K = p->K;
    const std::vector<double2> wh = pack_what(W0_host, f64, (size_t)p->F, M, K);
    int rc = upload_what(p, wh);
    if (rc) return rc;
    p->wscale_pending = false;
    p->have_w = true;
    if (K < M) return stage_update(p, true);
    return OIVA_OK;
}

static int set_w_from_eigenvectors(oiva_plan* p, double* evals_host, bool lapack_phase);

int oiva_plan_set_w_pca(oiva_plan* p, double* evals_host) { return set_w_from_eigenvectors(p, evals_host, false); }
int oiva_plan_set_w_eig(oiva_plan* p) { return set_w_from_eigenvectors(p, nullptr, true); }

static int set_w_from_eigenvectors(oiva_plan* p, double* evals_host, bool lapack_phase) {
    OIVA_NEED(p, OIVA_ERR_ARG, "null plan");
    OIVA_NEED(p->have_cx, OIVA_ERR_STATE, "input covariance not computed (oiva_plan_covariance)");
    DeviceGuard guard(p->device);
    double* evals = evals_host ? p->scratch_p : nullptr;
    OIVA_TRY_HIP(launch_pca_subspace(p->stream, p->Cx, p->What, p->What64, evals, p->F, p->M, p->K, lapack_phase));
    p->what64_valid = true;
    p->wscale_pending = false;
    p->have_w = true;
    if (evals_host) {
        OIVA_TRY_HIP(hipStreamSynchronize(p->stream));
        OIVA_TRY_HIP(hipMemcpy(evals_host, evals, (size_t)p->F * p->M * sizeof(double), hipMemcpyDeviceToHost));
    }
    if (p->K < p->M) return stage_update(p, true);
    return OIVA_OK;
}

static int check_fused(oiva_plan* p);

int oiva_plan_demix_dev(oiva_plan* p, int proj_back, void** Y_dev) {
    int rc = check_ready(p);
    if (rc) return rc;
    OIVA_NEED(Y_dev, OIVA_ERR_ARG, "null output");
    DeviceGuard guard(p->device);
    if ((rc = check_fused(p))) return rc;
    if (!p->Y) OIVA_TRY_HIP(p->mem.take_one(&p->Y, (size_t)p->F * p->K * sizeof(float2) * p->T, Mem::pooled));
    const float* sp = nullptr;
    if (proj_back) {
        OIVA_TRY_HIP(launch_demix_stats(p->stream, p->X, p->What, p->Spart, p->T, p->F, p->M, p->K, p->stg));
        sp = p->Spart;
    }
    OIVA_TRY_HIP(launch_demix_write(p->stream, p->X, p->What, sp, p->stg.nsplit, p->Y, p->T, p->F, p->M, p->K));
    OIVA_TRY_HIP(hipStreamSynchronize(p->stream));
    *Y_dev = p->Y;
    return OIVA_OK;
}

int oiva_plan_iterate(oiva_plan* p, int n) {
    int rc = check_ready(p);
    if (rc) return rc;
    OIVA_NEED(n >= 0, OIVA_ERR_ARG, "negative iteration count");
    OIVA_NEED(p->F == p->F_total || resident_applies(p) || p->fx_on, OIVA_ERR_STATE,
              "plan owns a bin shard: drive it with oiva_plan_power / all-gather / oiva_plan_update (or connect an in-kernel exchange: "
              "oiva_plan_fused_connect, oiva_plan_resident_connect)");
    DeviceGuard guard(p->device);
    if (n == 0) return OIVA_OK;
    if (resident_applies(p)) {
        bool ran = false;
        if ((rc = run_resident(p, n, &ran))) return rc;
        if (ran) return OIVA_OK;
    }
    if (p->use_graph) {
        for (int left = n; left > 0;) {
            const int m = std::min(left, kGraphMaxIters);
            hipGraphExec_t g = nullptr;
            if ((rc = graph_for(p, m, &g))) return rc;
            OIVA_TRY_HIP(hipGraphLaunch(g, p->stream));
            left -= m;
        }
        p->wscale_pending = false;
        p->raw_weights = 0;
        p->what64_valid = p->upd_f64();
        return OIVA_OK;
    }
    for (int i = 0; i < n; ++i)
        if ((rc = one_iteration(p))) return rc;
    return OIVA_OK;
}

int oiva_plan_power(oiva_plan* p) {
    int rc = check_ready(p);
    if (rc) return rc;
    DeviceGuard guard(p->device);
    return stage_power(p);
}

int oiva_plan_power_buffer(oiva_plan* p, int parts_per_rank, void** parts_dev, long long* bytes) {
    OIVA_NEED(p && parts_dev, OIVA_ERR_ARG, "null argument");
    OIVA_NEED(parts_per_rank >= p->pw.nb, OIVA_ERR_ARG, "parts_per_rank smaller than this plan's own bin batches");
    DeviceGuard guard(p->device);
    const size_t part = (size_t)p->T * p->K * sizeof(float);
    if (parts_per_rank > p->ppart_alloc) {
        OIVA_TRY_HIP(hipStreamSynchronize(p->stream));
        int rc = drop_graph(p);
        if (rc) return rc;
        p->mem.release(&p->Ppart);
        OIVA_TRY_HIP(p->mem.take_one(&p->Ppart, part * parts_per_rank));
        OIVA_TRY_HIP(hipMemsetAsync(p->Ppart, 0, part * parts_per_rank, p->stream));
        p->ppart_alloc = parts_per_rank;
    }
    *parts_dev = p->Ppart;
    if (bytes) *bytes = (long long)(part * parts_per_rank);
    return OIVA_OK;
}

int oiva_plan_update(oiva_plan* p, const void* parts_dev, int nparts) {
    int rc = check_ready(p);
    if (rc) return rc;
    OIVA_NEED(parts_dev && nparts >= 1, OIVA_ERR_ARG, "need at least one part");
    DeviceGuard guard(p->device);
    if ((rc = stage_activation(p, (const float*)parts_dev, nparts))) return rc;
    if (cov_update_applies(p)) return stage_cov_update(p);
    if ((rc = stage_cov(p))) return rc;
    return stage_update(p, false);
}

static int demix_to_host(oiva_plan* p, void* Y_host, long long row_pitch_bytes, int proj_back, bool c128) {
    int rc = check_ready(p);
    if (rc) return rc;
    OIVA_NEED(Y_host, OIVA_ERR_ARG, "null output");
    DeviceGuard guard(p->device);
    const size_t n_row = (size_t)p->F * p->K;
    const size_t row_dev = n_row * sizeof(float2);
    const size_t row = c128 ? n_row * sizeof(double2) : row_dev;
    const size_t pitch = row_pitch_bytes > 0 ? (size_t)row_pitch_bytes : row;
    OIVA_NEED(pitch >= row, OIVA_ERR_ARG, "row pitch smaller than one frame of this plan's bins");
    if ((rc = check_fused(p))) return rc;
    if (!p->Y) OIVA_TRY_HIP(p->mem.take_one(&p->Y, row_dev * p->T, Mem::pooled));
    const float* sp = nullptr;
    if (proj_back) {
        OIVA_TRY_HIP(launch_demix_stats(p->stream, p->X, p->What, p->Spart, p->T, p->F, p->M, p->K, p->stg));
        sp = p->Spart;
    }
    static const int mode = [] {
        const char* v = std::getenv("OIVA_DEMIX_IO");
        if (v && !std::strcmp(v, "legacy")) return 0;
        if (v && !std::strcmp(v, "register")) return 2;
        return 1;
    }();
    const size_t slab_target = p->io_slab_bytes ? p->io_slab_bytes : ((size_t)8 << 20);
    if (mode == 0 || (size_t)p->T * row < slab_target / 2) {
        OIVA_TRY_HIP(launch_demix_write(p->stream, p->X, p->What, sp, p->stg.nsplit, p->Y, p->T, p->F, p->M, p->K));
        if (!c128) {
            OIVA_TRY_HIP(hipStreamSynchronize(p->stream));
            OIVA_TRY_HIP(hipMemcpy2D(Y_host, pitch, p->Y, row, row, p->T, hipMemcpyDeviceToHost));
            return OIVA_OK;
        }
        OIVA_TRY_HIP(staged_copy_c128(false, p->stream, Y_host, pitch, p->Y, n_row, p->T, kStageBytes, p->device, Mem::plain));
        return OIVA_OK;
    }
    const int slab = (int)std::max<size_t>(1, std::min<size_t>((size_t)p->T, slab_target / row));
    const int nslab = ceil_div(p->T, slab);
    const size_t slab_bytes = (size_t)slab * row;
    if (!p->io_stream) OIVA_TRY_HIP(p->io_stream.open(nullptr, 0));
    if (p->io_stream.events.size() < 2 * kHostRingSlots)
        OIVA_TRY_HIP(p->io_stream.add_events(2 * kHostRingSlots - (int)p->io_stream.events.size(),  false));
    hipEvent_t* io_written = p->io_stream.events.data();
    hipEvent_t* io_copied = io_written + kHostRingSlots;
    if (c128 && p->io_c128_bytes < slab_bytes) {
        OIVA_TRY_HIP(hipStreamSynchronize(p->stream));
        for (auto& b : p->io_c128) p->mem.release(&b);
        p->io_c128_bytes = 0;
        for (auto& b : p->io_c128) p->mem.take(&b, slab_bytes, Mem::pooled);
        if (!p->mem.ok()) {
            for (auto& b : p->io_c128) p->mem.release(&b);
            OIVA_TRY_HIP(p->mem.status());
        }
        p->io_c128_bytes = slab_bytes;
    }
    bool registered = false;
    void* pinned[kHostRingSlots] = {};
    if (mode == 2) {
        registered = hipHostRegister(Y_host, pitch * (size_t)(p->T - 1) + row, hipHostRegisterDefault) == hipSuccess;
        if (!registered) (void)hipGetLastError();
    }
    static std::mutex io_mutex;
    std::unique_lock<std::mutex> io_lock(io_mutex, std::defer_lock);
    if (!registered) {
        io_lock.lock();
        OIVA_TRY_HIP(host_ring_slots(slab_bytes, pinned));
    }
    auto finish = [&](hipError_t e) -> int {
        (void)hipStreamSynchronize(p->io_stream);
        if (registered) (void)hipHostUnregister(Y_host);
        if (e != hipSuccess) return fail_with(OIVA_ERR_HIP, std::string("final demix: ") + hipGetErrorString(e));
        return OIVA_OK;
    };
    auto issue = [&](int k) -> hipError_t {
        const int s = k % kHostRingSlots;
        const int t0 = k * slab, nt = std::min(slab, p->T - t0);
        float2* ydev = p->Y + (size_t)t0 * n_row;
        hipError_t e = launch_demix_write(p->stream, p->X + (size_t)t0 * p->F * p->M, p->What, sp, p->stg.nsplit, ydev, nt, p->F, p->M, p->K);
        const void* src = ydev;
        if (e == hipSuccess && c128) {
            e = launch_cast_c64_to_c128(p->stream, ydev, p->io_c128[s], (long long)nt * n_row);
            src = p->io_c128[s];
        }
        if (e == hipSuccess) e = hipEventRecord(io_written[s], p->stream);
        if (e == hipSuccess) e = hipStreamWaitEvent(p->io_stream, io_written[s], 0);
        if (e == hipSuccess) {
            if (registered)
                e = hipMemcpy2DAsync(static_cast<char*>(Y_host) + (size_t)t0 * pitch, pitch, src, row, row, nt, hipMemcpyDeviceToHost, p->io_stream);
            else
                e = hipMemcpyAsync(pinned[s], src, (size_t)nt * row, hipMemcpyDeviceToHost, p->io_stream);
        }
        if (e == hipSuccess) e = hipEventRecord(io_copied[s], p->io_stream);
        return e;
    };
    int issued = 0;
    for (int k = 0; k < nslab; ++k) {
        hipError_t e = hipSuccess;
        while (issued < nslab && issued - k < kHostRingSlots && e == hipSuccess) e = issue(issued++);
        if (k == 0 && !registered && e == hipSuccess) {
            host_prefault(Y_host, pitch * (size_t)(p->T - 1) + row,  pitch == row);
        }
        if (e == hipSuccess) e = hipEventSynchronize(io_copied[k % kHostRingSlots]);
        if (e != hipSuccess) return finish(e);
        if (!registered) {
            const int t0 = k * slab, nt = std::min(slab, p->T - t0);
            host_copy_rows(static_cast<char*>(Y_host) + (size_t)t0 * pitch, pitch, pinned[k % kHostRingSlots], row, row, nt);
        }
    }
    return finish(hipStreamSynchronize(p->stream));
}

int oiva_plan_set_io_slab(oiva_plan* p, long long bytes) {
    OIVA_NEED(p && bytes >= 0, OIVA_ERR_ARG, "bad arguments");
    p->io_slab_bytes = (size_t)bytes;
    return OIVA_OK;
}

int oiva_plan_demix(oiva_plan* p, void* Y_host, long long row_pitch_bytes, int proj_back) {
    return demix_to_host(p, Y_host, row_pitch_bytes, proj_back, false);
}

int oiva_plan_demix_c128(oiva_plan* p, void* Y_host, long long row_pitch_bytes, int proj_back) {
    return demix_to_host(p, Y_host, row_pitch_bytes, proj_back, true);
}

int oiva_plan_get_w(oiva_plan* p, void* W_host, int f64) {
    OIVA_NEED(p && W_host, OIVA_ERR_ARG, "null argument");
    OIVA_NEED(p->have_w, OIVA_ERR_STATE, "demixing matrix not set");
    DeviceGuard guard(p->device);
    int rc = check_fused(p);
    if (rc) return rc;
    std::vector<double2> wh;
    rc = download_what(p, wh);
    if (rc) return rc;
    const bool finite = unpack_w(wh, 0, (size_t)p->F, p->M, p->K, W_host, f64);
    if (!finite) return fail_with(OIVA_ERR_NUMERIC, "demixing matrix holds non-finite values (singular W_hat^H V)");
    return OIVA_OK;
}

static int check_fused(oiva_plan* p) {
    if (!p->fx_state || !p->fx_on) return OIVA_OK;
    if (!p->fx_flag_host) OIVA_TRY_HIP(p->mem.take_one(&p->fx_flag_host, sizeof(unsigned), Mem::pinned));
    OIVA_TRY_HIP(hipMemcpyAsync(p->fx_flag_host, p->fx_state, sizeof(unsigned), hipMemcpyDeviceToHost, p->stream));
    OIVA_TRY_HIP(hipStreamSynchronize(p->stream));
    const unsigned code = *p->fx_flag_host;
    if (code != 0)
        return fail_with(OIVA_ERR_STATE, "the exchange inside the activation kernel gave up waiting for a rank's partial powers (workgroup " +
                                        std::to_string(code - 1) + "): the state of this plan is undefined (oiva_plan_restore_w brings back the "
                                        "demixing matrices saved by oiva_plan_save_w; oiva_plan_fused_connect(p, NULL) clears the condition)");
    return OIVA_OK;
}

int oiva_plan_sync(oiva_plan* p) {
    OIVA_NEED(p, OIVA_ERR_ARG, "null plan");
    DeviceGuard guard(p->device);
    OIVA_TRY_HIP(hipStreamSynchronize(p->stream));
    return check_fused(p);
}

int oiva_plan_save_w(oiva_plan* p) {
    OIVA_NEED(p, OIVA_ERR_ARG, "null plan");
    OIVA_NEED(p->have_w, OIVA_ERR_STATE, "demixing matrix not set");
    DeviceGuard guard(p->device);
    const size_t n = (size_t)p->F * p->M * p->M;
    if (!p->ck_what) OIVA_TRY_HIP(p->mem.take_one(&p->ck_what, n * sizeof(float2)));
    if (!p->ck_what64) OIVA_TRY_HIP(p->mem.take_one(&p->ck_what64, n * sizeof(double2)));
    OIVA_TRY_HIP(hipMemcpyAsync(p->ck_what, p->What, n * sizeof(float2), hipMemcpyDeviceToDevice, p->stream));
    OIVA_TRY_HIP(hipMemcpyAsync(p->ck_what64, p->What64, n * sizeof(double2), hipMemcpyDeviceToDevice, p->stream));
    p->ck_what64_valid = p->what64_valid;
    p->ck_valid = true;
    return OIVA_OK;
}

int oiva_plan_restore_w(oiva_plan* p) {
    OIVA_NEED(p, OIVA_ERR_ARG, "null plan");
    OIVA_NEED(p->ck_valid, OIVA_ERR_STATE, "nothing saved (oiva_plan_save_w)");
    DeviceGuard guard(p->device);
    const size_t n = (size_t)p->F * p->M * p->M;
    OIVA_TRY_HIP(hipMemcpyAsync(p->What, p->ck_what, n * sizeof(float2), hipMemcpyDeviceToDevice, p->stream));
    OIVA_TRY_HIP(hipMemcpyAsync(p->What64, p->ck_what64, n * sizeof(double2), hipMemcpyDeviceToDevice, p->stream));
    p->what64_valid = p->ck_what64_valid;
    p->wscale_pending = false;
    p->have_w = true;
    return OIVA_OK;
}

static int fused_setup(oiva_plan* p) {
    const size_t words = 16 + (size_t)rsum_blocks(p->T) * p->K;
    if (!p->fx_state) OIVA_TRY_HIP(p->mem.take_one(&p->fx_state, words * sizeof(unsigned)));
    OIVA_TRY_HIP(hipStreamSynchronize(p->stream));
    OIVA_TRY_HIP(hipMemset(p->fx_state, 0, words * sizeof(unsigned)));
    return drop_graph(p);
}

int oiva_plan_fused_connect(oiva_plan* p, oiva_xchg* x) {
    OIVA_NEED(p, OIVA_ERR_ARG, "null plan");
    OIVA_NEED(!p->fx_loopback, OIVA_ERR_STATE, "the plan runs the loop-back exchange (oiva_plan_fused_loopback(p, 0) switches it off)");
    DeviceGuard guard(p->device);
    if (!x) {
        OIVA_TRY_HIP(hipStreamSynchronize(p->stream));
        p->fx_on = false;
        p->fx_world = 1;
        p->fx_rank = 0;
        for (auto& g : p->fx_gath) g = nullptr;
        if (p->fx_state) OIVA_TRY_HIP(hipMemset(p->fx_state, 0, sizeof(unsigned)));
        return drop_graph(p);
    }
    char* peers[OIVA_XCHG_MAX_RANKS];
    int rank = 0, world = 1;
    size_t slot = 0;
    OIVA_NEED(xchg_peers(x, peers, &rank, &world, &slot) == 0, OIVA_ERR_STATE, "exchange not connected");
    const size_t word_bytes = (size_t)p->T * p->K * 8;
    OIVA_NEED(slot % word_bytes == 0 && slot / word_bytes >= 1 && slot / word_bytes <= (size_t)kCanonBlocks, OIVA_ERR_ARG,
              "exchange slot size must be nblk * T * K * 8 bytes, nblk = 1 ... 8 block sums per rank");
    const int nblk = (int)(slot / word_bytes);
    OIVA_NEED(p->pw.nb % nblk == 0, OIVA_ERR_ARG, "the plan's 64-bin parts do not divide into that many blocks");
    OIVA_NEED((world - 1) * nblk <= kCanonBlocks, OIVA_ERR_ARG, "the activation kernel polls at most 8 words of the other ranks per frame and source (9 ranks of one sum each)");
    int rc = fused_setup(p);
    if (rc) return rc;
    OIVA_TRY_HIP(hipMemset(peers[rank], 0, (size_t)2 * world * slot));
    OIVA_TRY_HIP(hipDeviceSynchronize());
    p->fx_nblk_own = p->fx_nblk_peer = nblk;
    for (int r = 0; r < OIVA_XCHG_MAX_RANKS; ++r) p->fx_gath[r] = peers[r];
    p->fx_rank = rank;
    p->fx_world = world;
    p->fx_on = true;
    return OIVA_OK;
}

int oiva_plan_fused_loopback(oiva_plan* p, int world) {
    OIVA_NEED(p, OIVA_ERR_ARG, "null plan");
    OIVA_NEED(world >= 0 && world <= OIVA_XCHG_MAX_RANKS, OIVA_ERR_ARG, "bad number of ranks");
    DeviceGuard guard(p->device);
    OIVA_TRY_HIP(hipStreamSynchronize(p->stream));
    p->mem.release(&p->fx_loop_buf);
    if (p->fx_loopback) {
        p->fx_on = p->fx_loopback = false;
        p->fx_world = 1;
        for (auto& g : p->fx_gath) g = nullptr;
        int rc = drop_graph(p);
        if (rc) return rc;
    }
    if (world <= 1) return OIVA_OK;
    OIVA_NEED(!p->fx_on, OIVA_ERR_STATE, "the plan is connected to other ranks (oiva_plan_fused_connect(p, NULL) disconnects)");
    OIVA_NEED(p->F == p->F_total, OIVA_ERR_STATE, "loop-back plays the other ranks with zeros: the plan must own all bins");
    const int bsz = (p->pw.nb + kCanonBlocks - 1) / kCanonBlocks;
    p->fx_nblk_own = (p->pw.nb + bsz - 1) / bsz;
    p->fx_nblk_peer = std::max(1, kCanonBlocks / world);
    OIVA_NEED((world - 1) * p->fx_nblk_peer <= kCanonBlocks, OIVA_ERR_ARG, "at most 9 ranks");
    const size_t bytes = (size_t)2 * world * p->fx_nblk_peer * p->T * p->K * 8;
    OIVA_TRY_HIP(p->mem.take_one(&p->fx_loop_buf, bytes, Mem::fine));
    OIVA_TRY_HIP(hipMemset(p->fx_loop_buf, 0, bytes));
    int rc = fused_setup(p);
    if (rc) return rc;
    for (int r = 0; r < world; ++r) p->fx_gath[r] = p->fx_loop_buf;
    p->fx_rank = 0;
    p->fx_world = world;
    p->fx_loopback = true;
    p->fx_on = true;
    return OIVA_OK;
}

int oiva_plan_fused_debug(oiva_plan* p, int timeout_ms, int stall) {
    OIVA_NEED(p, OIVA_ERR_ARG, "null plan");
    DeviceGuard guard(p->device);
    p->fx_timeout_ms = timeout_ms;
    p->fx_stall = stall;
    OIVA_TRY_HIP(hipStreamSynchronize(p->stream));
    return drop_graph(p);
}

int oiva_plan_iterate_timed(oiva_plan* p, int n, float* total_ms, float* per_kernel_ms) {
    int rc = check_ready(p);
    if (rc) return rc;
    OIVA_NEED(n >= 1 && total_ms, OIVA_ERR_ARG, "bad arguments");
    OIVA_NEED(p->F == p->F_total, OIVA_ERR_STATE, "timed iterate needs a plan that owns all bins");
    DeviceGuard guard(p->device);
    if (!per_kernel_ms) return p->stream.elapsed_ms(0, 1, [&] { return oiva_plan_iterate(p, n); }, total_ms);
    for (int s = 0; s < OIVA_N_STAGES; ++s) per_kernel_ms[s] = 0.f;
    *total_ms = 0.f;
    const int per_it = OIVA_N_STAGES + 1;
    HandleStream bracket, kern;
    hipError_t err = bracket.add_events(n * per_it);
    if (err != hipSuccess) return fail_with(OIVA_ERR_HIP, std::string("hipEventCreate: ") + hipGetErrorString(err));
    if (kern.add_events(2 * n) != hipSuccess) (void)hipGetLastError();
    std::vector<hipEvent_t>& pool = bracket.events;
    std::vector<hipEvent_t> kev = kern.events;
    kev.resize((size_t)2 * n, nullptr);
    for (int it = 0; it < n && err == hipSuccess && rc == OIVA_OK; ++it) {
        hipEvent_t* e = pool.data() + (size_t)it * per_it;
        err = hipEventRecord(e[0], p->stream);
        if (err == hipSuccess && !(rc = stage_power(p))) err = hipEventRecord(e[1], p->stream);
        if (err == hipSuccess && !rc && !(rc = stage_activation(p, p->Ppart, p->pw.nb))) err = hipEventRecord(e[2], p->stream);
        const bool fused = cov_update_applies(p);
        if (err == hipSuccess && !rc) {
            arm_kernel_timer(kev[2 * it], kev[2 * it + 1]);
            rc = fused ? stage_cov_update(p) : stage_cov(p);
            arm_kernel_timer(nullptr, nullptr);
            if (!rc) err = hipEventRecord(e[3], p->stream);
        }
        if (err == hipSuccess && !rc && !(fused ? OIVA_OK : (rc = stage_update(p, false)))) err = hipEventRecord(e[4], p->stream);
    }
    if (err == hipSuccess && rc == OIVA_OK) err = hipStreamSynchronize(p->stream);
    for (int it = 0; it < n && err == hipSuccess && rc == OIVA_OK; ++it) {
        hipEvent_t* e = pool.data() + (size_t)it * per_it;
        for (int s = 0; s < OIVA_N_STAGES && err == hipSuccess; ++s) {
            float ms = 0.f;
            err = hipEventElapsedTime(&ms, e[s], e[s + 1]);
            float kms = 0.f;
            const bool one_launch = traits(p->cov.kind).launches == 1;
            if (s == 2 && one_launch && kev[2 * it] && kev[2 * it + 1] && hipEventElapsedTime(&kms, kev[2 * it], kev[2 * it + 1]) == hipSuccess &&
                kms > 0.f && kms <= ms)
                ms = kms;
            else if (s == 2)
                (void)hipGetLastError();
            per_kernel_ms[s] += ms;
        }
    }
    if (err == hipSuccess && rc == OIVA_OK) err = hipEventElapsedTime(total_ms, pool[0], pool[(size_t)n * per_it - 1]);
    if (rc) return rc;
    OIVA_TRY_HIP(err);
    return OIVA_OK;
}

int oiva_plan_get_cov_splits(oiva_plan* p, int* nsplit) {
    OIVA_NEED(p && nsplit, OIVA_ERR_ARG, "null argument");
    *nsplit = p->cov.nsplit;
    return OIVA_OK;
}

int oiva_plan_set_cov_splits(oiva_plan* p, int nsplit) {
    OIVA_NEED(p, OIVA_ERR_ARG, "null plan");
    OIVA_NEED(nsplit >= 0 && nsplit <= p->T, OIVA_ERR_ARG, "bad split count");
    return change_geometry(p, [&] { choose_cov_geom(p, nsplit); return OIVA_OK; });
}

int oiva_plan_set_cov_quad(oiva_plan* p, int enable, int* active) {
    OIVA_NEED(p, OIVA_ERR_ARG, "null plan");
    return change_geometry(p, [&] {
        p->cov_quad_on = enable != 0;
        choose_cov_geom(p, 0);
        if (active) *active = traits(p->cov.kind).quad_switch;
        return OIVA_OK;
    });
}

int oiva_plan_set_fuse_cov_update(oiva_plan* p, int enable, int* active) {
    OIVA_NEED(p, OIVA_ERR_ARG, "null plan");
    if (enable >= 0) {
        const int rc = change_geometry(p, [&] { p->fuse_cov_update = enable != 0; return OIVA_OK; });
        if (rc) return rc;
    }
    if (active) *active = cov_update_applies(p) ? 1 : 0;
    return OIVA_OK;
}

int oiva_plan_set_cov_hmfma(oiva_plan* p, int enable) {
    OIVA_NEED(p, OIVA_ERR_ARG, "null plan");
    return change_geometry(p, [&] { p->cov_hmfma_on = enable != 0; choose_cov_geom(p, 0); return OIVA_OK; });
}

int oiva_plan_set_pow_splits(oiva_plan* p, int nsplit) {
    OIVA_NEED(p, OIVA_ERR_ARG, "null plan");
    OIVA_NEED(nsplit >= 0 && nsplit <= p->T, OIVA_ERR_ARG, "bad split count");
    return change_geometry(p, [&] { choose_pow_geom(p, nsplit); return OIVA_OK; });
}

int oiva_plan_set_power_reverse(oiva_plan* p, int enable) {
    OIVA_NEED(p, OIVA_ERR_ARG, "null plan");
    return change_geometry(p, [&] { p->power_reverse = enable < 0 ? 0 : enable > 2 ? 2 : enable; return OIVA_OK; });
}

int oiva_plan_use_graph(oiva_plan* p, int enable) {
    OIVA_NEED(p, OIVA_ERR_ARG, "null plan");
    DeviceGuard guard(p->device);
    p->use_graph = enable ? 1 : 0;
    if (!enable) return drop_graph(p);
    if (p->have_x && p->have_cx && p->have_w && (p->F == p->F_total || p->fx_on)) return build_graphs(p);
    return OIVA_OK;
}

int oiva_plan_set_precision(oiva_plan* p, int flags) {
    OIVA_NEED(p, OIVA_ERR_ARG, "null plan");
    OIVA_NEED((flags & ~(OIVA_PREC_UPDATE_F64 | OIVA_PREC_UPDATE_ROWS | OIVA_PREC_COV_F64)) == 0, OIVA_ERR_ARG, "unknown precision flag");
    return change_geometry(p, [&] {
        if ((flags & OIVA_PREC_UPDATE_F64) && p->have_w && !p->what64_valid) {
            std::vector<double2> wh;
            int rc;
            if ((rc = download_what(p, wh)) || (rc = upload_what(p, wh))) return rc;
        }
        const bool cov_changed = ((flags ^ p->prec) & (OIVA_PREC_COV_F64 | (traits(p->cov.kind).update_arith ? OIVA_PREC_UPDATE_F64 : 0))) != 0;
        p->prec = flags;
        if (cov_changed) choose_cov_geom(p, 0);
        return (int)OIVA_OK;
    });
}

int oiva_plan_set_resident(oiva_plan* p, int enable) {
    OIVA_NEED(p, OIVA_ERR_ARG, "null plan");
    if (!enable) {
        p->res_on = false;
        return OIVA_OK;
    }
    OIVA_NEED(p->res_ok, OIVA_ERR_ARG,
              "shape does not qualify for the X-resident iteration (4 or 8 channels, 1 or 2 sources with background channels, "
              "16 bins x <= 256 frames per compute unit)");
    DeviceGuard guard(p->device);
    int rc = resident_alloc(p);
    if (rc) return rc;
    p->res_on = true;
    return OIVA_OK;
}

int oiva_plan_set_resident_splits(oiva_plan* p, int nsplit) {
    OIVA_NEED(p && nsplit >= 0, OIVA_ERR_ARG, "bad arguments");
    OIVA_NEED(!p->res_on, OIVA_ERR_STATE, "switch the resident iteration off before changing its geometry");
    DeviceGuard guard(p->device);
    ResidentGeom g;
    const bool ok = resident_geometry(p->T, p->F, p->M, p->K, p->n_cu, nsplit, &g);
    OIVA_NEED(ok || nsplit == 0, OIVA_ERR_ARG, "the shape does not fit on chip with that many frame splits");
    if (p->res_block) {
        OIVA_TRY_HIP(hipStreamSynchronize(p->stream));
        p->mem.release(&p->res_block);
    }
    p->res_ok = ok;
    if (ok) p->rg = g;
    return OIVA_OK;
}

int oiva_plan_resident_loopback(oiva_plan* p, int world) {
    OIVA_NEED(p, OIVA_ERR_ARG, "null plan");
    OIVA_NEED(world >= 0 && world <= OIVA_XCHG_MAX_RANKS, OIVA_ERR_ARG, "bad number of ranks");
    OIVA_NEED(!p->res_on, OIVA_ERR_STATE, "switch the resident iteration off before changing its exchange");
    DeviceGuard guard(p->device);
    if (p->res_loop_buf) {
        OIVA_TRY_HIP(hipStreamSynchronize(p->stream));
        p->mem.release(&p->res_loop_buf);
    }
    p->res_loopback = false;
    p->res_world = 1;
    p->res_rank = 0;
    for (auto& g : p->res_gath) g = nullptr;
    if (world <= 1) return OIVA_OK;
    OIVA_NEED(p->res_ok, OIVA_ERR_ARG, "shape does not qualify for the X-resident iteration");
    OIVA_NEED(p->F == p->F_total, OIVA_ERR_STATE, "loop-back plays the other ranks with zeros: the plan must own all bins");
    const size_t bytes = (size_t)2 * world * p->rg.NS * p->rg.TW * p->K * sizeof(float);
    OIVA_TRY_HIP(p->mem.take_one(&p->res_loop_buf, bytes, Mem::fine));
    OIVA_TRY_HIP(hipMemset(p->res_loop_buf, 0, bytes));
    for (int r = 0; r < world; ++r) p->res_gath[r] = p->res_loop_buf;
    p->res_world = world;
    p->res_loopback = true;
    if (p->res_block) {
        OIVA_TRY_HIP(hipStreamSynchronize(p->stream));
        OIVA_TRY_HIP(hipMemset(p->res_block, 0, p->res_block_bytes));
        p->res_epoch = 0;
    }
    return OIVA_OK;
}

int oiva_plan_resident_connect(oiva_plan* p, oiva_xchg* x) {
    OIVA_NEED(p, OIVA_ERR_ARG, "null plan");
    OIVA_NEED(!p->res_loopback, OIVA_ERR_STATE, "the plan runs the loop-back exchange (oiva_plan_resident_loopback(p, 0) switches it off)");
    if (!x) {
        p->res_world = 1;
        p->res_rank = 0;
        for (auto& g : p->res_gath) g = nullptr;
        return OIVA_OK;
    }
    OIVA_NEED(p->res_ok, OIVA_ERR_ARG, "shape does not qualify for the X-resident iteration");
    char* peers[OIVA_XCHG_MAX_RANKS];
    int rank = 0, world = 1;
    size_t slot = 0;
    OIVA_NEED(xchg_peers(x, peers, &rank, &world, &slot) == 0, OIVA_ERR_STATE, "exchange not connected");
    const size_t want = (size_t)p->rg.NS * p->rg.TW * p->K * sizeof(float);
    OIVA_NEED(slot == want, OIVA_ERR_ARG, "exchange slot size must be frame_splits * frames_per_split * K * 4 bytes of THIS plan "
                                     "(every rank must run the same split geometry)");
    for (int r = 0; r < OIVA_XCHG_MAX_RANKS; ++r) p->res_gath[r] = peers[r];
    p->res_rank = rank;
    p->res_world = world;
    return OIVA_OK;
}

int oiva_plan_resident_info(oiva_plan* p, int* info) {
    OIVA_NEED(p && info, OIVA_ERR_ARG, "null argument");
    const ResidentGeom& g = p->rg;
    const int v[OIVA_RESIDENT_INFO] = {p->res_ok ? 1 : 0, p->res_on ? 1 : 0, g.NB, g.NS, g.TW, g.J, g.JR, g.lds_bytes,
                                       p->res_last_code, p->res_launches, p->res_fallbacks, g.J * kBlock * p->M * 8};
    for (int i = 0; i < OIVA_RESIDENT_INFO; ++i) info[i] = v[i];
    return OIVA_OK;
}

int oiva_plan_resident_phases(oiva_plan* p, double* phase_us, int* n_iter) {
    OIVA_NEED(p && phase_us && n_iter, OIVA_ERR_ARG, "null argument");
    for (int i = 0; i < OIVA_RESIDENT_PHASES; ++i) phase_us[i] = 0.;
    *n_iter = 0;
    if (!p->res_stamps || p->res_stamped <= 0) return OIVA_OK;
    DeviceGuard guard(p->device);
    const int n = p->res_stamped;
    std::vector<unsigned long long> st((size_t)n * kResidentStamps);
    OIVA_TRY_HIP(hipStreamSynchronize(p->stream));
    OIVA_TRY_HIP(hipMemcpy(st.data(), p->res_stamps, st.size() * sizeof(unsigned long long), hipMemcpyDeviceToHost));
    static_assert(OIVA_RESIDENT_PHASES <= kResidentStamps - 1, "one phase between consecutive stamps");
    for (int it = 0; it < n; ++it)
        for (int i = 0; i < OIVA_RESIDENT_PHASES; ++i)
            phase_us[i] += (double)(st[(size_t)it * kResidentStamps + i + 1] - st[(size_t)it * kResidentStamps + i]) * 0.01 / n;
    *n_iter = n;
    return OIVA_OK;
}

int oiva_plan_resident_trace(oiva_plan* p, int enable, unsigned long long* stamps_host, int* n_wg, int* n_iter) {
    OIVA_NEED(p, OIVA_ERR_ARG, "null plan");
    DeviceGuard guard(p->device);
    p->res_trace = enable != 0;
    if (n_wg) *n_wg = p->rg.NB * p->rg.NS;
    if (n_iter) *n_iter = p->res_trace_buf ? p->res_trace_iters : 0;
    if (stamps_host && p->res_trace_buf) {
        OIVA_TRY_HIP(hipStreamSynchronize(p->stream));
        OIVA_TRY_HIP(hipMemcpy(stamps_host, p->res_trace_buf,
                          (size_t)p->rg.NB * p->rg.NS * p->res_trace_iters * kResidentStamps * sizeof(unsigned long long), hipMemcpyDeviceToHost));
    }
    return OIVA_OK;
}

int oiva_plan_resident_debug(oiva_plan* p, int timeout_ms, int stall_block) {
    OIVA_NEED(p, OIVA_ERR_ARG, "null plan");
    p->res_timeout_ms = timeout_ms;
    p->res_stall = stall_block;
    p->res_stall_iter = 0;
    return OIVA_OK;
}

int oiva_plan_resident_debug_from(oiva_plan* p, int timeout_ms, int stall_block, int first_stalled_iteration) {
    OIVA_NEED(p && first_stalled_iteration >= 0, OIVA_ERR_ARG, "bad arguments");
    p->res_timeout_ms = timeout_ms;
    p->res_stall = stall_block;
    p->res_stall_iter = first_stalled_iteration;
    return OIVA_OK;
}

int oiva_plan_ogive_begin(oiva_plan* p, int update_mode, int model) {
    OIVA_NEED(p, OIVA_ERR_ARG, "null plan");
    OIVA_NEED(p->M <= kNarrowMax, OIVA_ERR_ARG, "OGIVE runs on 1..16 channels (its per-bin state is sized for them)");
    int rc = check_ready(p);
    if (rc) return rc;
    OIVA_NEED(p->K == 1, OIVA_ERR_ARG, "OGIVE extracts one source: create the plan with K = 1");
    OIVA_NEED(p->F == p->F_total, OIVA_ERR_STATE, "OGIVE is not bin-sharded");
    OIVA_NEED(update_mode >= OIVA_OGIVE_DEMIX && update_mode <= OIVA_OGIVE_SWITCHING, OIVA_ERR_ARG, "unknown update mode");
    OIVA_NEED(model == OIVA_MODEL_LAPLACE || model == OIVA_MODEL_GAUSS, OIVA_ERR_ARG, "unknown model");
    DeviceGuard guard(p->device);
    const size_t F = p->F, M = p->M;
    if (!p->og.maxdelta) {
        const size_t before = p->mem.mark();
        alloc_ogive_state(p->og, F, M, p->mem);
        if (!p->mem.ok()) {
            p->mem.release_to(before);
            return fail_with(OIVA_ERR_HIP, std::string("allocation failed: ") + hipGetErrorString(p->mem.status()));
        }
    }
    if (!p->what64_valid) {
        std::vector<double2> wh;
        if ((rc = download_what(p, wh)) || (rc = upload_what(p, wh))) return rc;
    }
    if (p->og_graph) {
        OIVA_TRY_HIP(hipStreamSynchronize(p->stream));
        OIVA_TRY_HIP(hipGraphExecDestroy(p->og_graph));
        p->og_graph = nullptr;
    }
    p->og.Cx = p->Cx;
    p->og.What = p->What;
    p->og.What64 = p->What64;
    p->og_mode = update_mode;
    p->og_model = model;
    OIVA_TRY_HIP(launch_ogive_init(p->stream, p->og, p->F, p->M, update_mode));
    p->og_ready = true;
    return OIVA_OK;
}

int oiva_plan_ogive_iterate(oiva_plan* p, int first_epoch, int n, double step_size, double tol, int* epochs_run,
                            int* converged, double* max_delta) {
    int rc = check_ready(p);
    if (rc) return rc;
    OIVA_NEED(p->og_ready, OIVA_ERR_STATE, "call oiva_plan_ogive_begin first");
    OIVA_NEED(n >= 0 && first_epoch >= 0, OIVA_ERR_ARG, "negative epoch count");
    DeviceGuard guard(p->device);
    int before[2] = {0, 0};
    OIVA_TRY_HIP(hipStreamSynchronize(p->stream));
    OIVA_TRY_HIP(hipMemcpy(before, p->og.ctrl, sizeof(before), hipMemcpyDeviceToHost));
    const int amodel = p->og_model == OIVA_MODEL_LAPLACE ? kModelOgiveLaplace : OIVA_MODEL_GAUSS;
    auto epochs = [&](int e0, int count) -> int {
        for (int e = e0; e < e0 + count; ++e) {
            if (p->og_mode == OIVA_OGIVE_SWITCHING && e % 10 == 0) OIVA_TRY_HIP(launch_ogive_switch(p->stream, p->og, p->F, p->M));
            int r = stage_power(p);
            if (r) return r;
            OIVA_TRY_HIP(launch_activation(p->stream, p->Ppart, p->pw.nb, p->R, p->T, 1, amodel, p->F));
            OIVA_TRY_HIP(launch_cov(p->stream, p->X, p->X_pad, p->R, p->Plocal, p->wscale, p->model,  1, p->Vpart,
                               p->cov_f64(), p->T, p->F, p->M, 1, p->cov));
            OIVA_TRY_HIP(launch_ogive_step(p->stream, p->og, p->Vpart, p->vpart_f64(), p->cov.nsplit, p->T, p->F, p->M, step_size,
                                      tol));
        }
        return OIVA_OK;
    };
    constexpr int kMinGraphEpochs = 8;
    if (n >= kMinGraphEpochs) {
        const int phase = first_epoch % 10;
        if (!p->og_graph || p->og_graph_n != n || p->og_graph_phase != phase || p->og_graph_mu != step_size ||
            p->og_graph_tol != tol) {
            if (p->og_graph) OIVA_TRY_HIP(hipGraphExecDestroy(p->og_graph));
            p->og_graph = nullptr;
            rc = capture_graph(p->stream, [&] { return epochs(phase, n); }, &p->og_graph, false);
            if (rc) return rc;
            p->og_graph_n = n;
            p->og_graph_phase = phase;
            p->og_graph_mu = step_size;
            p->og_graph_tol = tol;
        }
        OIVA_TRY_HIP(hipGraphLaunch(p->og_graph, p->stream));
    } else if ((rc = epochs(first_epoch, n))) {
        return rc;
    }
    p->wscale_pending = false;
    int after[2] = {0, 0};
    OIVA_TRY_HIP(hipStreamSynchronize(p->stream));
    OIVA_TRY_HIP(hipMemcpy(after, p->og.ctrl, sizeof(after), hipMemcpyDeviceToHost));
    if (epochs_run) *epochs_run = after[1] - before[1];
    if (converged) *converged = after[0];
    if (max_delta) OIVA_TRY_HIP(hipMemcpy(max_delta, p->og.maxdelta, sizeof(double), hipMemcpyDeviceToHost));
    return OIVA_OK;
}

int oiva_test_set_rinv(oiva_plan* p, const float* rinv_host) {
    OIVA_NEED(p && rinv_host, OIVA_ERR_ARG, "null argument");
    DeviceGuard guard(p->device);
    std::vector<float> r((size_t)p->T * p->K);
    for (size_t i = 0; i < r.size(); ++i) r[i] = 1.f / rinv_host[i];
    OIVA_TRY_HIP(hipStreamSynchronize(p->stream));
    OIVA_TRY_HIP(hipMemcpy(p->R, r.data(), r.size() * sizeof(float), hipMemcpyHostToDevice));
    p->raw_weights = 1;
    return OIVA_OK;
}

int oiva_test_get_rinv(oiva_plan* p, float* rinv_host, float* wscale_host) {
    OIVA_NEED(p, OIVA_ERR_ARG, "null plan");
    DeviceGuard guard(p->device);
    OIVA_TRY_HIP(hipStreamSynchronize(p->stream));
    if (rinv_host) {
        const int T = p->T, K = p->K;
        std::vector<float> r((size_t)T * K);
        OIVA_TRY_HIP(hipMemcpy(r.data(), p->R, r.size() * sizeof(float), hipMemcpyDeviceToHost));
        for (int k = 0; k < K; ++k) {
            double s = 0.;
            for (int t = 0; t < T; ++t) s += (double)r[(size_t)t * K + k];
            const float ginv = p->raw_weights ? 1.f : 1.f / (float)(s / (double)T);
            for (int t = 0; t < T; ++t) {
                float rn = r[(size_t)t * K + k] * ginv;
                rn = rn < 1e-15f ? 1e-15f : rn;
                rinv_host[(size_t)t * K + k] = 1.f / rn;
            }
        }
    }
    if (wscale_host) OIVA_TRY_HIP(hipMemcpy(wscale_host, p->wscale, (size_t)p->K * sizeof(float), hipMemcpyDeviceToHost));
    return OIVA_OK;
}

int oiva_test_run_weighted_cov(oiva_plan* p) {
    OIVA_NEED(p, OIVA_ERR_ARG, "null plan");
    OIVA_NEED(p->have_x, OIVA_ERR_STATE, "X not set");
    DeviceGuard guard(p->device);
    int rc = ensure_pad(p);
    if (rc) return rc;
    return stage_cov(p);
}

int oiva_test_get_v(oiva_plan* p, void* V_host, int f64) {
    OIVA_NEED(p && V_host, OIVA_ERR_ARG, "null argument");
    DeviceGuard guard(p->device);
    const int F = p->F, M = p->M, K = p->K;
    const long long nfk = (long long)F * K * M * M;
    OIVA_TRY_HIP(launch_sum_parts(p->stream, p->Vpart, p->vpart_f64(), p->cov.nsplit, p->scratch_p, nfk, 1. / (double)p->T));
    OIVA_TRY_HIP(launch_unpack_herm(p->stream, p->scratch_p, p->scratch_c, f64 != 0, (long long)F * K, M));
    OIVA_TRY_HIP(hipStreamSynchronize(p->stream));
    const size_t esz = f64 ? sizeof(double2) : sizeof(float2);
    std::vector<char> fk((size_t)nfk * esz);
    OIVA_TRY_HIP(hipMemcpy(fk.data(), p->scratch_c, fk.size(), hipMemcpyDeviceToHost));
    char* out = (char*)V_host;
    const size_t mm = (size_t)M * M * esz;
    for (int f = 0; f < F; ++f)
        for (int k = 0; k < K; ++k)
            std::memcpy(out + ((size_t)k * F + f) * mm, fk.data() + ((size_t)f * K + k) * mm, mm);
    return OIVA_OK;
}

int oiva_test_run_update(oiva_plan* p) {
    int rc = check_ready(p);
    if (rc) return rc;
    DeviceGuard guard(p->device);
    return stage_update(p, false);
}

int oiva_test_get_what(oiva_plan* p, void* What_host, int f64) {
    OIVA_NEED(p && What_host, OIVA_ERR_ARG, "null argument");
    DeviceGuard guard(p->device);
    std::vector<double2> wh;
    int rc = download_what(p, wh);
    if (rc) return rc;
    if (f64) {
        std::memcpy(What_host, wh.data(), wh.size() * sizeof(double2));
    } else {
        float2* o = static_cast<float2*>(What_host);
        for (size_t i = 0; i < wh.size(); ++i) o[i] = make_float2((float)wh[i].x, (float)wh[i].y);
    }
    return OIVA_OK;
}

int oiva_test_set_what(oiva_plan* p, const void* What_host, int f64) {
    OIVA_NEED(p && What_host, OIVA_ERR_ARG, "null argument");
    DeviceGuard guard(p->device);
    std::vector<double2> wh((size_t)p->F * p->M * p->M);
    if (f64) {
        std::memcpy(wh.data(), What_host, wh.size() * sizeof(double2));
    } else {
        const float2* in = static_cast<const float2*>(What_host);
        for (size_t i = 0; i < wh.size(); ++i) wh[i] = make_double2(in[i].x, in[i].y);
    }
    int rc = upload_what(p, wh);
    if (rc) return rc;
    p->have_w = true;
    p->wscale_pending = false;
    return OIVA_OK;
}

int oiva_test_time_stage(oiva_plan* p, int stage, int reps, float* avg_ms) {
    int rc = check_ready(p);
    if (rc) return rc;
    OIVA_NEED(reps >= 1 && avg_ms && stage >= 0 && stage < OIVA_N_STAGES, OIVA_ERR_ARG, "bad arguments");
    DeviceGuard guard(p->device);
    auto run = [&]() -> int {
        switch (stage) {
            case 0: return stage_power(p);
            case 1: return stage_activation(p, p->Ppart, p->pw.nb);
            case 2: return cov_update_applies(p) ? stage_cov_update(p) : stage_cov(p);
            default: return cov_update_applies(p) ? OIVA_OK : stage_update(p, false);
        }
    };
    if ((rc = run())) return rc;
    float ms = 0.f;
    rc = p->stream.elapsed_ms(0, 1, [&] {
        int r = OIVA_OK;
        for (int i = 0; i < reps && r == OIVA_OK; ++i) r = run();
        return r;
    }, &ms);
    if (rc) return rc;
    *avg_ms = ms / reps;
    return OIVA_OK;
}

int oiva_test_run_power(oiva_plan* p, float* p_host) {
    OIVA_NEED(p && p_host, OIVA_ERR_ARG, "null argument");
    OIVA_NEED(p->have_x && p->have_w, OIVA_ERR_STATE, "X / W not set");
    DeviceGuard guard(p->device);
    int rc = stage_power(p);
    if (rc) return rc;
    const size_t n = (size_t)p->T * p->K;
    OIVA_TRY_HIP(launch_sum_parts(p->stream, p->Ppart, false, p->pw.nb, p->scratch_p, (long long)n, 1.));
    OIVA_TRY_HIP(hipStreamSynchronize(p->stream));
    std::vector<double> sum(n);
    OIVA_TRY_HIP(hipMemcpy(sum.data(), p->scratch_p, n * sizeof(double), hipMemcpyDeviceToHost));
    for (size_t i = 0; i < n; ++i) p_host[i] = (float)sum[i];
    return OIVA_OK;
}

int oiva_test_get_ppart(oiva_plan* p, float* parts_host, int* nparts) {
    OIVA_NEED(p && nparts, OIVA_ERR_ARG, "null argument");
    *nparts = p->pw.nb;
    if (!parts_host) return OIVA_OK;
    DeviceGuard guard(p->device);
    OIVA_TRY_HIP(hipStreamSynchronize(p->stream));
    OIVA_TRY_HIP(hipMemcpy(parts_host, p->Ppart, (size_t)p->pw.nb * p->T * p->K * sizeof(float), hipMemcpyDeviceToHost));
    return OIVA_OK;
}

int oiva_test_power_order(int nsplit, int tcp, int cov_splits, int cov_tc, int* order) {
    OIVA_NEED(order && nsplit >= 1 && tcp >= 1 && cov_splits >= 1 && cov_tc >= 1, OIVA_ERR_ARG, "bad arguments");
    OIVA_NEED(cov_splits <= kPowOrderMaxSplits, OIVA_ERR_ARG, "more covariance splits than the order table holds");
    const PowOrder o = make_pow_order(nsplit, tcp, cov_splits, cov_tc);
    for (int y = 0; y < nsplit; ++y) order[y] = power_chunk_tail_first(y, nsplit, o);
    return OIVA_OK;
}

int oiva_test_kernel_choice(int device, int T, int F, int F_total, int M, int K, int prec_flags, int quad_on, int hmfma_on,
                            int cov_splits_req, int pow_splits_req, int* out) {
    OIVA_NEED(out && T >= 1 && F >= 1 && F_total >= F && M >= 1 && M <= OIVA_MAX_CHANNELS && K >= 1 && K <= M, OIVA_ERR_ARG, "bad arguments");
    OIVA_NEED(cov_splits_req >= 0 && pow_splits_req >= 0, OIVA_ERR_ARG, "bad split count");
    DeviceGuard guard(device);
    oiva_plan p;
    p.device = device, p.T = T, p.F = F, p.F_total = F_total, p.M = M, p.K = K, p.prec = prec_flags;
    p.cov_quad_on = quad_on != 0, p.cov_hmfma_on = hmfma_on != 0;
    hipDeviceProp_t prop;
    if (hipGetDeviceProperties(&prop, device) == hipSuccess && prop.multiProcessorCount > 0) p.n_cu = prop.multiProcessorCount;
    int asked[2] = {-1, -1};
    const ChoiceIn c = choice_in(&p);
    const CovGeom g = choose_cov(c, device_occupancy(asked), cov_splits_req);
    const PowGeom w = choose_pow(c, device_occupancy(asked), pow_splits_req);
    const int o[18] = {(int)g.kind, g.nsplit, g.tc, g.kc, g.nbg, g.pad, g.part32, partials_f64(g, c.cov_f64) ? 1 : 0, (int)traits(g.kind).unit,
                       (int)w.kind, w.nb, w.nsplit, w.tcp, w.kp, w.rounds, asked[0], asked[1], p.n_cu};
    std::copy(o, o + 18, out);
    return OIVA_OK;
}

}
```

### overiva_amd/plan.py

```python
import ctypes as C

import numpy as np

from . import _lib


def _is_f64(a):
    if a.dtype == np.complex128:
        return 1
    if a.dtype == np.complex64:
        return 0
    raise TypeError(f"complex64 or complex128 expected, got {a.dtype}")


class DeviceX:

    def __init__(self, ptr, shape, owner=None, host_dtype=np.complex64):
        self.ptr = int(ptr)
        self.shape = tuple(int(v) for v in shape)
        self.owner = owner
        self.dtype = np.dtype(host_dtype)
        self.ndim = 3


class Plan(_lib.Handle):

    _destroy = "oiva_plan_destroy"

    def __init__(self, T, F, M, K, model="laplace", device=0, F_total=None, stream=None):
        if model not in _lib.MODEL_IDS:
            raise ValueError(f"model must be 'laplace' or 'gauss', got {model!r}")
        self.lib = _lib.load()
        self.T, self.F, self.M, self.K = int(T), int(F), int(M), int(K)
        self.model = model
        self.F_total = int(F if F_total is None else F_total)
        self.device = int(device)
        h = C.c_void_p()
        _lib.check(self.lib.oiva_plan_create(C.byref(h), self.device, self.T, self.F, self.M, self.K,
                                             _lib.MODEL_IDS[model], self.F_total,
                                             C.c_void_p(stream) if stream else None))
        self.h = h
        self._keep = None

    def set_x(self, X, f0=0):
        if isinstance(X, DeviceX):
            if X.shape != (self.T, self.F, self.M) or f0:
                raise ValueError(f"device X has shape {X.shape}, plan expects ({self.T}, {self.F}, {self.M})")
            return self.set_x_device(X.ptr, X.owner)
        X = np.asarray(X)
        if X.ndim != 3 or X.shape[0] != self.T or X.shape[2] != self.M or X.shape[1] < f0 + self.F:
            raise ValueError(f"X has shape {X.shape}, plan expects ({self.T}, >={f0 + self.F}, {self.M})")
        if X.dtype == np.complex128 and X.flags["C_CONTIGUOUS"]:
            pitch = X.shape[1] * self.M * 16
            base = X.ctypes.data + f0 * self.M * 16
            _lib.check(self.lib.oiva_plan_set_x_host_c128(self.h, C.c_void_p(base), pitch))
            return
        if X.dtype != np.complex64 or not X.flags["C_CONTIGUOUS"]:
            X = np.ascontiguousarray(X[:, f0:f0 + self.F, :], dtype=np.complex64)
            f0 = 0
        pitch = X.shape[1] * self.M * 8
        base = X.ctypes.data + f0 * self.M * 8
        _lib.check(self.lib.oiva_plan_set_x_host(self.h, C.c_void_p(base), pitch))

    def set_x_device(self, dev_ptr, keepalive=None):
        self._keep = keepalive
        _lib.check(self.lib.oiva_plan_set_x_dev(self.h, C.c_void_p(int(dev_ptr))))

    def covariance(self):
        _lib.check(self.lib.oiva_plan_covariance(self.h))

    def get_cx(self, dtype=np.complex128):
        out = np.empty((self.F, self.M, self.M), dtype)
        _lib.check(self.lib.oiva_plan_get_cx(self.h, _lib.ptr(out), _is_f64(out)))
        return out

    def set_w(self, W0=None):
        if W0 is None:
            _lib.check(self.lib.oiva_plan_set_w(self.h, None, 0))
            return
        W0 = np.asarray(W0)
        dt = np.complex64 if W0.dtype == np.complex64 else np.complex128
        W0 = np.ascontiguousarray(np.broadcast_to(W0, (self.F, self.M, self.K)), dtype=dt)
        _lib.check(self.lib.oiva_plan_set_w(self.h, _lib.ptr(W0), _is_f64(W0)))

    def set_w_pca(self, return_eigenvalues=False):
        ev = np.empty((self.F, self.M), np.float64) if return_eigenvalues else None
        _lib.check(self.lib.oiva_plan_set_w_pca(self.h, _lib.ptr(ev) if ev is not None else None))
        return ev

    def set_w_eig(self):
        _lib.check(self.lib.oiva_plan_set_w_eig(self.h))

    def iterate(self, n=1):
        _lib.check(self.lib.oiva_plan_iterate(self.h, int(n)))

    def power(self):
        _lib.check(self.lib.oiva_plan_power(self.h))

    BINS_PER_PART = 64

    @classmethod
    def power_parts(cls, n_bins):
        return (n_bins + cls.BINS_PER_PART - 1) // cls.BINS_PER_PART

    def power_buffer(self, parts_per_rank):
        p, nbytes = C.c_void_p(), C.c_longlong()
        _lib.check(self.lib.oiva_plan_power_buffer(self.h, int(parts_per_rank), C.byref(p), C.byref(nbytes)))
        return p.value, nbytes.value

    def update(self, parts_dev_ptr, nparts):
        _lib.check(self.lib.oiva_plan_update(self.h, C.c_void_p(int(parts_dev_ptr)), int(nparts)))

    def ogive_begin(self, update="demix", model="laplace"):
        _lib.check(self.lib.oiva_plan_ogive_begin(self.h, {"demix": 0, "mix": 1, "switching": 2}[update],
                                                  _lib.MODEL_IDS[model]))

    def ogive_iterate(self, first_epoch, n, step_size=0.1, tol=1e-3):
        ran, conv, md = C.c_int(), C.c_int(), C.c_double()
        _lib.check(self.lib.oiva_plan_ogive_iterate(self.h, int(first_epoch), int(n), float(step_size), float(tol),
                                                    C.byref(ran), C.byref(conv), C.byref(md)))
        return ran.value, bool(conv.value), md.value

    def iterate_timed(self, n, per_kernel=False):
        total = C.c_float()
        if per_kernel:
            arr = (C.c_float * _lib.N_STAGES)()
            _lib.check(self.lib.oiva_plan_iterate_timed(self.h, int(n), C.byref(total), arr))
            return total.value, dict(zip(_lib.STAGE_NAMES, list(arr)))
        _lib.check(self.lib.oiva_plan_iterate_timed(self.h, int(n), C.byref(total), None))
        return total.value, None

    def demix(self, proj_back=True, out=None, f0=0, dtype=np.complex64):
        if out is None:
            out = np.empty((self.T, self.F, self.K), dtype)
            f0 = 0
        assert out.dtype in (np.complex64, np.complex128) and out.flags["C_CONTIGUOUS"]
        size = out.dtype.itemsize
        pitch = out.shape[1] * self.K * size
        base = out.ctypes.data + f0 * self.K * size
        fn = self.lib.oiva_plan_demix if size == 8 else self.lib.oiva_plan_demix_c128
        _lib.check(fn(self.h, C.c_void_p(base), pitch, 1 if proj_back else 0))
        return out

    def set_io_slab(self, nbytes=0):
        _lib.check(self.lib.oiva_plan_set_io_slab(self.h, int(nbytes)))

    def demix_device(self, proj_back=False):
        dev = C.c_void_p()
        _lib.check(self.lib.oiva_plan_demix_dev(self.h, 1 if proj_back else 0, C.byref(dev)))
        return DeviceX(dev.value, (self.T, self.F, self.K), owner=self)

    def get_w(self, dtype=np.complex64):
        out = np.empty((self.F, self.M, self.K), dtype)
        _lib.check(self.lib.oiva_plan_get_w(self.h, _lib.ptr(out), _is_f64(out)))
        return out

    def sync(self):
        _lib.check(self.lib.oiva_plan_sync(self.h))

    def save_w(self):
        _lib.check(self.lib.oiva_plan_save_w(self.h))

    def restore_w(self):
        _lib.check(self.lib.oiva_plan_restore_w(self.h))

    def cov_splits(self):
        n = C.c_int()
        _lib.check(self.lib.oiva_plan_get_cov_splits(self.h, C.byref(n)))
        return n.value

    def set_cov_splits(self, n):
        _lib.check(self.lib.oiva_plan_set_cov_splits(self.h, int(n)))

    def set_cov_quad(self, enable=True):
        a = C.c_int()
        _lib.check(self.lib.oiva_plan_set_cov_quad(self.h, 1 if enable else 0, C.byref(a)))
        return bool(a.value)

    def set_cov_hmfma(self, enable=True):
        _lib.check(self.lib.oiva_plan_set_cov_hmfma(self.h, 1 if enable else 0))

    def set_fuse_cov_update(self, enable=True):
        a = C.c_int()
        _lib.check(self.lib.oiva_plan_set_fuse_cov_update(self.h, -1 if enable is None else (1 if enable else 0), C.byref(a)))
        return bool(a.value)

    def set_pow_splits(self, n):
        _lib.check(self.lib.oiva_plan_set_pow_splits(self.h, int(n)))

    def set_power_reverse(self, enable=True):
        _lib.check(self.lib.oiva_plan_set_power_reverse(self.h, int(enable)))

    def use_graph(self, enable=True):
        _lib.check(self.lib.oiva_plan_use_graph(self.h, 1 if enable else 0))

    def set_precision(self, mode="fast", row_layout=False):
        flags = _lib.PREC_BY_NAME[mode] if isinstance(mode, str) else int(mode)
        if row_layout:
            flags |= _lib.PREC_UPDATE_ROWS
        _lib.check(self.lib.oiva_plan_set_precision(self.h, flags))

    RESIDENT_INFO = ("qualifies", "enabled", "bin_groups", "frame_splits", "frames_per_split", "frames_per_lane",
                     "frames_in_registers", "lds_bytes", "last_give_up_code", "launches", "fallbacks", "x_bytes_per_cu")
    RESIDENT_PHASES = ("demix_power", "parts", "activation", "cov_accumulate", "cov_reduce", "wait_partials", "ip_update", "wait_w")

    def set_resident(self, enable=True):
        _lib.check(self.lib.oiva_plan_set_resident(self.h, 1 if enable else 0))

    def resident_info(self):
        arr = (C.c_int * len(self.RESIDENT_INFO))()
        _lib.check(self.lib.oiva_plan_resident_info(self.h, arr))
        return dict(zip(self.RESIDENT_INFO, list(arr)))

    def resident_phases(self):
        arr = (C.c_double * len(self.RESIDENT_PHASES))()
        n = C.c_int()
        _lib.check(self.lib.oiva_plan_resident_phases(self.h, arr, C.byref(n)))
        return dict(zip(self.RESIDENT_PHASES, list(arr))), n.value

    def set_resident_splits(self, nsplit=0):
        _lib.check(self.lib.oiva_plan_set_resident_splits(self.h, int(nsplit)))

    def resident_connect(self, xchg_handle):
        _lib.check(self.lib.oiva_plan_resident_connect(self.h, xchg_handle))

    def fused_connect(self, xchg_handle):
        _lib.check(self.lib.oiva_plan_fused_connect(self.h, xchg_handle))

    def fused_loopback(self, world=2):
        _lib.check(self.lib.oiva_plan_fused_loopback(self.h, int(world)))

    def fused_debug(self, timeout_ms=0, stall=False):
        _lib.check(self.lib.oiva_plan_fused_debug(self.h, int(timeout_ms), 1 if stall else 0))

    def resident_trace(self, enable=True, fetch=False):
        nw, ni = C.c_int(), C.c_int()
        _lib.check(self.lib.oiva_plan_resident_trace(self.h, 1 if enable else 0, None, C.byref(nw), C.byref(ni)))
        if not fetch or ni.value == 0:
            return None
        out = np.zeros((nw.value, ni.value, 16), np.uint64)
        _lib.check(self.lib.oiva_plan_resident_trace(self.h, 1 if enable else 0, _lib.ptr(out), C.byref(nw), C.byref(ni)))
        return out

    def resident_debug(self, timeout_ms=0, stall_block=-1, from_iteration=0):
        _lib.check(self.lib.oiva_plan_resident_debug_from(self.h, int(timeout_ms), int(stall_block), int(from_iteration)))

    def resident_loopback(self, world=8):
        _lib.check(self.lib.oiva_plan_resident_loopback(self.h, int(world)))

    def t_set_rinv(self, rinv):
        rinv = np.ascontiguousarray(rinv, dtype=np.float32)
        assert rinv.shape == (self.T, self.K)
        _lib.check(self.lib.oiva_test_set_rinv(self.h, _lib.ptr(rinv)))

    def t_get_rinv(self):
        r = np.empty((self.T, self.K), np.float32)
        w = np.empty((self.K,), np.float32)
        _lib.check(self.lib.oiva_test_get_rinv(self.h, _lib.ptr(r), _lib.ptr(w)))
        return r, w

    def t_run_weighted_cov(self):
        _lib.check(self.lib.oiva_test_run_weighted_cov(self.h))

    def t_get_v(self, dtype=np.complex64):
        v = np.empty((self.K, self.F, self.M, self.M), dtype)
        _lib.check(self.lib.oiva_test_get_v(self.h, _lib.ptr(v), _is_f64(v)))
        return v

    def t_run_update(self):
        _lib.check(self.lib.oiva_test_run_update(self.h))

    def t_get_what(self, dtype=np.complex64):
        w = np.empty((self.F, self.M, self.M), dtype)
        _lib.check(self.lib.oiva_test_get_what(self.h, _lib.ptr(w), _is_f64(w)))
        return w

    def t_set_what(self, What):
        What = np.asarray(What)
        What = np.ascontiguousarray(What, dtype=np.complex64 if What.dtype == np.complex64 else np.complex128)
        assert What.shape == (self.F, self.M, self.M)
        _lib.check(self.lib.oiva_test_set_what(self.h, _lib.ptr(What), _is_f64(What)))

    def t_time_stage(self, stage, reps=20):
        ms = C.c_float()
        _lib.check(self.lib.oiva_test_time_stage(self.h, _lib.STAGE_NAMES.index(stage), int(reps), C.byref(ms)))
        return ms.value

    def t_get_ppart(self):
        n = C.c_int()
        _lib.check(self.lib.oiva_test_get_ppart(self.h, None, C.byref(n)))
        out = np.empty((n.value, self.T, self.K), np.float32)
        _lib.check(self.lib.oiva_test_get_ppart(self.h, _lib.ptr(out), C.byref(n)))
        return out

    def t_run_power(self):
        p = np.empty((self.T, self.K), np.float32)
        _lib.check(self.lib.oiva_test_run_power(self.h, _lib.ptr(p)))
        return p


COV_KINDS = ("Lane", "Pair32", "Pair64", "Quad", "Half16", "Hmfma", "Half16F64", "Hmfma64", "Mfma", "Wide")
POW_KINDS = ("Lane", "Mfma", "Lds", "Wide")
KERNEL_CHOICE = ("cov_kind", "nsplit", "tc", "kc", "nbg", "pad", "part32", "vpart_f64", "unit_kind", "pow_kind", "nb", "pow_nsplit",
                 "tcp", "kp", "rounds", "occ_cov", "occ_pow", "n_cu")


def kernel_choice(T, F, M, K, mode="fast", F_total=None, cov_quad=True, cov_hmfma=True, cov_splits=0, pow_splits=0, device=0):
    flags = _lib.PREC_BY_NAME[mode] if isinstance(mode, str) else int(mode)
    out = (C.c_int * len(KERNEL_CHOICE))()
    _lib.check(_lib.load().oiva_test_kernel_choice(int(device), int(T), int(F), int(F if F_total is None else F_total), int(M), int(K),
                                                   flags, int(bool(cov_quad)), int(bool(cov_hmfma)), int(cov_splits), int(pow_splits), out))
    d = dict(zip(KERNEL_CHOICE, out))
    d["cov_kind"], d["unit_kind"], d["pow_kind"] = COV_KINDS[d["cov_kind"]], COV_KINDS[d["unit_kind"]], POW_KINDS[d["pow_kind"]]
    return d
```

Before: 5071.

## Keep a budgeted share of X cache-resident by streaming the rest non-temporally

Adds a policy that compares the X footprint with a default budget of about 268 MB. When X does not fit, a fixed fraction of each 16-frame group period is read normally and the remaining groups are read with non-temporal global_load_lds row loads in both the covariance DMA kernel and the power kernel. The idea is that the plainly read part of X stays in the last-level cache across iterations while the streamed part does not evict it, which cuts HBM traffic. In exchange it adds an LDS-staged row layout path, a new templated power kernel and geometry constraints. It only engages for the Lane kernels with M=8.

```diff
diff --git a/include/overiva_hip.h b/include/overiva_hip.h
--- a/include/overiva_hip.h
+++ b/include/overiva_hip.h
@@ -85,6 +85,8 @@
 int oiva_plan_set_cov_hmfma(oiva_plan *p, int enable);
 int oiva_plan_set_fuse_cov_update(oiva_plan *p, int enable, int *active);
 int oiva_plan_set_power_reverse(oiva_plan *p, int enable);
+int oiva_plan_set_x_resident_mb(oiva_plan *p, double mb);
+int oiva_plan_get_x_resident(oiva_plan *p, int *n16, int *nt, int *reason);
 int oiva_plan_use_graph(oiva_plan *p, int enable);
 int oiva_plan_set_precision(oiva_plan *p, int flags);
 
@@ -117,6 +119,9 @@
 int oiva_test_power_order(int nsplit, int tcp, int cov_splits, int cov_tc, int *order);
 int oiva_test_time_stage(oiva_plan *p, int stage, int reps, float *avg_ms);
 int oiva_test_live_buffers(long long *count, long long *bytes);
+int oiva_test_x_policy(int T, int F, int M, int cov_tc, int pow_tcp, double budget_mb, int *out, signed char *cov_walk, signed char *pow_walk);
+int oiva_test_x_choice(int T, int F, int M, int prec_flags, int cov_kind, int cov_tc, int pow_kind, int pow_tcp, double budget_mb, int from_env,
+                       int *out, double *budget_used);
 int oiva_test_kernel_choice(int device, int T, int F, int F_total, int M, int K, int prec_flags, int quad_on, int hmfma_on,
                             int cov_splits_req, int pow_splits_req, int *out);
 
diff --git a/overiva_amd/_lib.py b/overiva_amd/_lib.py
--- a/overiva_amd/_lib.py
+++ b/overiva_amd/_lib.py
@@ -71,6 +71,8 @@
     "oiva_plan_set_cov_hmfma": [_vp, _i],
     "oiva_plan_set_fuse_cov_update": [_vp, _i, C.POINTER(_i)],
     "oiva_plan_set_power_reverse": [_vp, _i],
+    "oiva_plan_set_x_resident_mb": [_vp, C.c_double],
+    "oiva_plan_get_x_resident": [_vp, C.POINTER(_i), C.POINTER(_i), C.POINTER(_i)],
     "oiva_plan_use_graph": [_vp, _i],
     "oiva_plan_set_precision": [_vp, _i],
     "oiva_plan_set_resident": [_vp, _i],
@@ -95,6 +97,8 @@
     "oiva_test_run_power": [_vp, _vp],
     "oiva_test_get_ppart": [_vp, _vp, C.POINTER(_i)],
     "oiva_test_power_order": [_i, _i, _i, _i, C.POINTER(_i)],
+    "oiva_test_x_choice": [_i] * 8 + [C.c_double, _i, C.POINTER(_i), C.POINTER(C.c_double)],
+    "oiva_test_x_policy": [_i, _i, _i, _i, _i, C.c_double, C.POINTER(_i), _vp, _vp],
     "oiva_test_time_stage": [_vp, _i, _i, _fp],
     "oiva_test_live_buffers": [C.POINTER(C.c_longlong), C.POINTER(C.c_longlong)],
     "oiva_test_kernel_choice": [_i] * 11 + [C.POINTER(_i)],
diff --git a/overiva_amd/csrc/kernel_choice.h b/overiva_amd/csrc/kernel_choice.h
--- a/overiva_amd/csrc/kernel_choice.h
+++ b/overiva_amd/csrc/kernel_choice.h
@@ -30,6 +30,7 @@
     CovKind kind = CovKind::Lane;
     int pad = 0;
     int part32 = 0;
+    int xplain = 16;
 };
 constexpr int kPowOrderMaxSplits = 64;
 struct PowOrder {
@@ -59,8 +60,36 @@
     int rev = 0;
     PowOrder ord{};
     int rounds = 1;
+    int xplain = 16;
+    int xctc = 0;
 };
 constexpr int kPowMaxFrames = 512;
+
+constexpr int kXGroup = 16, kXPeriod = 16;
+constexpr bool x_group_plain(int frame_in_split, int xplain) { return ((frame_in_split / kXGroup) % kXPeriod) < xplain; }
+constexpr int x_split_offset(int off0, int tl, int ctc) { return off0 + tl >= ctc ? off0 + tl - ctc : off0 + tl; }
+enum class XReason { Off, Fits, Kernels, Geometry, Share };
+constexpr double kXResidentDefaultMB = 268.;
+struct XPolicy {
+    int n16 = 0;
+    bool nt = false;
+    XReason why = XReason::Off;
+    int xplain() const { return nt ? n16 : kXPeriod; }
+};
+inline XPolicy choose_x_policy(double budget_mb, int T, int F, int M, bool cov_f64, const CovGeom& cg, const PowGeom& pg) {
+    XPolicy x;
+    if (!(budget_mb > 0.)) return x;
+    const double frame_bytes = (double)F * M * 8., budget = budget_mb * 1e6;
+    x.why = XReason::Fits, x.n16 = kXPeriod;
+    if (frame_bytes * T <= budget) return x;
+    x.why = XReason::Kernels, x.n16 = 0;
+    if (cg.kind != CovKind::Lane || pg.kind != PowKind::Lane || cov_f64 || M != 8) return x;
+    x.why = XReason::Geometry;
+    if (cg.tc % kXGroup != 0 || pg.tcp % 4 != 0 || pg.tcp > cg.tc) return x;
+    x.why = XReason::Share, x.nt = true;
+    x.n16 = std::min(kXPeriod - 1, (int)(budget * kXPeriod / (frame_bytes * T)));
+    return x;
+}
 
 enum class Partials { F64, Acc, F32IfPart32 };
 struct CovTraits {
diff --git a/overiva_amd/csrc/kernels_cov.hip b/overiva_amd/csrc/kernels_cov.hip
--- a/overiva_amd/csrc/kernels_cov.hip
+++ b/overiva_amd/csrc/kernels_cov.hip
@@ -46,7 +46,7 @@
 template <int M, int KC, bool UNIT, typename ACC>
 __global__ __launch_bounds__(kBlock) void cov_kernel(const float2* __restrict__ X, const float* __restrict__ R,
                                                      float* __restrict__ wscale, int model, int raw,
-                                                     double* __restrict__ Vpart, int T, int F, int K, int tc) {
+                                                     double* __restrict__ Vpart, int T, int F, int K, int tc, int ) {
     constexpr int NA = M * M;
     __shared__ ACC lds[kChunk * kLdsStride];
 
@@ -132,11 +132,10 @@
 
 constexpr int kDmaStages = 4;
 
-typedef __attribute__((address_space(1))) const void gvoid_t;
-typedef __attribute__((address_space(3))) void lvoid_t;
-
 template <int PIECES>
 __device__ __forceinline__ void ring_read(unsigned addr, float4 (&v)[PIECES]);
+template <int PIECES>
+__device__ __forceinline__ void ring_read_rows(unsigned addr, float4 (&v)[PIECES]);
 
 template <>
 __device__ __forceinline__ void ring_read<4>(unsigned addr, float4 (&v)[4]) {
@@ -163,6 +162,31 @@
         : "memory");
 }
 
+template <>
+__device__ __forceinline__ void ring_read_rows<4>(unsigned addr, float4 (&v)[4]) {
+    asm volatile(
+        "s_waitcnt vmcnt(12)\n\t"
+        "ds_read_b128 %0, %4\n\t"
+        "ds_read_b128 %1, %4 offset:16\n\t"
+        "ds_read_b128 %2, %4 offset:32\n\t"
+        "ds_read_b128 %3, %4 offset:48\n\t"
+        "s_waitcnt lgkmcnt(0)"
+        : "=&v"(v[0]), "=&v"(v[1]), "=&v"(v[2]), "=&v"(v[3])
+        : "v"(addr)
+        : "memory");
+}
+template <>
+__device__ __forceinline__ void ring_read_rows<2>(unsigned addr, float4 (&v)[2]) {
+    asm volatile(
+        "s_waitcnt vmcnt(6)\n\t"
+        "ds_read_b128 %0, %2\n\t"
+        "ds_read_b128 %1, %2 offset:16\n\t"
+        "s_waitcnt lgkmcnt(0)"
+        : "=&v"(v[0]), "=&v"(v[1])
+        : "v"(addr)
+        : "memory");
+}
+
 #ifdef OIVA_COVDMA_TRACE
 __device__ long long g_cd_trace[8 * 2048];
 #define CD_STAMP(slot)                                                                                                            \
@@ -178,7 +202,7 @@
 template <int M, int KC>
 __global__ __launch_bounds__(kBlock, 2) void cov_dma_kernel(const float2* __restrict__ X, const float* __restrict__ R,
                                                             float* __restrict__ wscale, int model, int raw,
-                                                            double* __restrict__ Vpart, int T, int F, int K, int tc) {
+                                                            double* __restrict__ Vpart, int T, int F, int K, int tc, int xplain) {
     constexpr int NA = M * M;
     constexpr int PIECES = M / 2;
     constexpr int STAGE = PIECES * 64;
@@ -217,8 +241,16 @@
     const unsigned rd_base = (unsigned)(uintptr_t)(wring) + lane * 16;
     const size_t frame_stride = (size_t)F * M;
     const float2* pbase = X + (size_t)fc * M;
+    using Rows = XRows<M>;
+    const int row_off = Rows::offset(lane, blockIdx.x * kBinsPerWave, F);
+    const unsigned rd_rows = (unsigned)(uintptr_t)(wring) + Rows::slot(b, ql) * 16;
+    auto plain = [&](int i) { return M != 8 || x_group_plain(kXGroup * i, xplain); };
 
     auto issue = [&](int i, int s) {
+        if (!plain(i)) {
+            Rows::issue_nt(X, frame_stride, row_off, lane, t_begin + wave * kPhasesPerWave + 16 * i, i < nsteps ? t_end : 0, T, wring + s * STAGE);
+            return;
+        }
         const int t = t_begin + q + 16 * i;
         const int tcl = (i < nsteps && t < t_end) ? t : T - 1;
         const float2* src = pbase + (size_t)tcl * frame_stride;
@@ -239,7 +271,10 @@
             w[kk] = activation_weight(r, ginv[kk]) * live;
         }
         float4 v[PIECES];
-        ring_read<PIECES>(rd_base + s * STAGE * 16, v);
+        if (plain(i))
+            ring_read<PIECES>(rd_base + s * STAGE * 16, v);
+        else
+            ring_read_rows<PIECES>(rd_rows + s * STAGE * 16, v);
 #if defined(OIVA_COVDMA_ABLATE) && (OIVA_COVDMA_ABLATE & 1)
         if constexpr (kPacked) {
             if (v[0].x == 12345.f) pacc.add(reinterpret_cast<const v2f(&)[M]>(v), v2f{w[0], w[1]});
@@ -314,7 +349,7 @@
 }
 
 template <typename ACC>
-using CovKernel = void (*)(const float2*, const float*, float*, int, int, double*, int, int, int, int);
+using CovKernel = void (*)(const float2*, const float*, float*, int, int, double*, int, int, int, int, int);
 
 template <int M, typename ACC, typename Fn>
 hipError_t dispatch_kc(int kc, bool unit, Fn&& fn) {
@@ -412,12 +447,12 @@
     if (f64)
         return dispatch_cov<double>(M, kc, R == nullptr, [&](CovKernel<double> kern, int KC) {
             kern<<<dim3(g.nbg, g.nsplit, (K + KC - 1) / KC), dim3(kBlock), 0, s>>>(X, R, wscale, model, raw,
-                                                                                 static_cast<double*>(Vpart), T, F, K, g.tc);
+                                                                                 static_cast<double*>(Vpart), T, F, K, g.tc, g.xplain);
             return hipGetLastError();
         });
     return dispatch_cov<float>(M, kc, R == nullptr, [&](CovKernel<float> kern, int KC) {
         return launch_dominant(kern, dim3(g.nbg, g.nsplit, (K + KC - 1) / KC), dim3(kBlock), 0, s, X, R, wscale, model, raw,
-                               static_cast<double*>(Vpart), T, F, K, g.tc);
+                               static_cast<double*>(Vpart), T, F, K, g.tc, g.xplain);
     });
 }
 
diff --git a/overiva_amd/csrc/kernels_demix.hip b/overiva_amd/csrc/kernels_demix.hip
--- a/overiva_amd/csrc/kernels_demix.hip
+++ b/overiva_amd/csrc/kernels_demix.hip
@@ -6,13 +6,14 @@
 
 constexpr int kPowUnroll = 2;
 
-template <int M, int KP>
+template <int M, int KP, bool NT = false>
 __global__ __launch_bounds__(kBlock) void power_kernel(const float2* __restrict__ X, const float2* __restrict__ What,
-                                                       float* __restrict__ Ppart, int T, int F, int K, int tcp, int rev, PowOrder ord) {
+                                                       float* __restrict__ Ppart, int T, int F, int K, int tcp, int rev, PowOrder ord,
+                                                       int xplain, int xctc) {
     extern __shared__ __attribute__((aligned(16))) float sp[];
     const int tid = threadIdx.x;
     const int lane = tid & 63;
-    const int wave = tid >> 6;
+    const int wave = NT ? __builtin_amdgcn_readfirstlane(tid >> 6) : tid >> 6;
     const int b = lane & 15;
     const int q = lane >> 4;
     const int f = (blockIdx.x * kWaves + wave) * kBinsPerWave + b;
@@ -31,19 +32,45 @@
 
     const size_t frame_stride = (size_t)F * M;
     const float2* pbase = X + (size_t)fc * M;
+    int off0 = 0, row_off = 0;
+    float4* wrows = nullptr;
+    if constexpr (NT) {
+        __shared__ float4 rows[kWaves * kPowUnroll * 32 * M];
+        off0 = t_begin % xctc;
+        row_off = XRows<M>::offset(lane, (blockIdx.x * kWaves + wave) * kBinsPerWave, F);
+        wrows = rows + wave * kPowUnroll * 32 * M;
+    }
     for (int g = 0; g < ngroups; ++g) {
         const int i = (rev ? ngroups - 1 - g : g) * kPowUnroll;
         float xr[kPowUnroll][M], xi[kPowUnroll][M];
+        bool plain[kPowUnroll];
 #pragma unroll
         for (int u = 0; u < kPowUnroll; ++u) {
             const int tl = 4 * (i + u) + q;
             const int t = tl < len ? t_begin + tl : T - 1;
+            plain[u] = !NT || x_group_plain(x_split_offset(off0, 4 * (i + u), xctc), xplain);
+            if constexpr (NT) {
+                if (!plain[u]) {
+                    XRows<M>::issue_nt(X, frame_stride, row_off, lane, t_begin + 4 * (i + u), t_end, T, wrows + u * 32 * M);
+                    continue;
+                }
+            }
             load_x<M>(pbase + (size_t)t * frame_stride, xr[u], xi[u]);
         }
 #pragma unroll
         for (int u = 0; u < kPowUnroll; ++u) {
             const int tl = 4 * (i + u) + q;
             const bool live = tl < len;
+            if constexpr (NT) {
+                if (!plain[u]) {
+                    const float4* v = wrows + u * 32 * M + XRows<M>::slot(b, q);
+#pragma unroll
+                    for (int j = 0; j < M / 2; ++j) {
+                        const float4 p = v[j];
+                        xr[u][2 * j] = p.x, xi[u][2 * j] = p.y, xr[u][2 * j + 1] = p.z, xi[u][2 * j + 1] = p.w;
+                    }
+                }
+            }
 #pragma unroll
             for (int kk = 0; kk < KP; ++kk) {
                 float yr, yi;
@@ -181,7 +208,14 @@
                             const PowGeom& g) {
     dim3 grid(g.nb, g.nsplit, (K + KP - 1) / KP);
     const size_t shmem = (size_t)kWaves * g.tcp * KP * sizeof(float);
-    hipLaunchKernelGGL((power_kernel<M, KP>), grid, dim3(kBlock), shmem, s, X, What, Ppart, T, F, K, g.tcp, g.rev, g.ord);
+    if constexpr (M == 8) {
+        if (g.xplain < kXPeriod) {
+            if (g.xctc < g.tcp || g.xctc % kXGroup != 0) return hipErrorInvalidValue;
+            hipLaunchKernelGGL((power_kernel<M, KP, true>), grid, dim3(kBlock), shmem, s, X, What, Ppart, T, F, K, g.tcp, g.rev, g.ord, g.xplain, g.xctc);
+            return hipGetLastError();
+        }
+    }
+    hipLaunchKernelGGL((power_kernel<M, KP, false>), grid, dim3(kBlock), shmem, s, X, What, Ppart, T, F, K, g.tcp, g.rev, g.ord, kXPeriod, 0);
     return hipGetLastError();
 }
 
diff --git a/overiva_amd/csrc/oiva_device.h b/overiva_amd/csrc/oiva_device.h
--- a/overiva_amd/csrc/oiva_device.h
+++ b/overiva_amd/csrc/oiva_device.h
@@ -56,6 +56,31 @@
         }
     }
 }
+
+typedef __attribute__((address_space(1))) const void gvoid_t;
+typedef __attribute__((address_space(3))) void lvoid_t;
+template <int M>
+struct XRows {
+    static_assert(M == 4 || M == 8, "whole 1-KB instructions of 16-byte pieces");
+    static constexpr int kPieces = M / 2;
+    static constexpr int kLanesPerRow = 16 * kPieces;
+    static constexpr int kFramesPerInstr = 64 / kLanesPerRow;
+    static __device__ __forceinline__ int frame(int lane, int j) { return j * kFramesPerInstr + lane / kLanesPerRow; }
+    static __device__ __forceinline__ int offset(int lane, int f0, int F) {
+        const int r = lane % kLanesPerRow, f = f0 + r / kPieces;
+        return (f < F ? f : F - 1) * M + (r % kPieces) * 2;
+    }
+    static __device__ __forceinline__ int slot(int b, int q) { return (q * 16 + b) * kPieces; }
+    static __device__ __forceinline__ void issue_nt(const float2* __restrict__ X, size_t frame_stride, int off, int lane, int t0, int t_lim,
+                                                    int T, float4* stage) {
+#pragma unroll
+        for (int j = 0; j < kPieces; ++j) {
+            const int t = t0 + frame(lane, j);
+            const float2* src = X + (size_t)(t < t_lim ? t : T - 1) * frame_stride + off;
+            __builtin_amdgcn_global_load_lds((gvoid_t*)src, (lvoid_t*)(stage + j * 64), 16, 0,  2);
+        }
+    }
+};
 
 using f32x4 = __attribute__((ext_vector_type(4))) float;
 using f64x4 = __attribute__((ext_vector_type(4))) double;
diff --git a/overiva_amd/csrc/plan.hip b/overiva_amd/csrc/plan.hip
--- a/overiva_amd/csrc/plan.hip
+++ b/overiva_amd/csrc/plan.hip
@@ -52,6 +52,7 @@
     bool cov_hmfma_on = true;
     bool fuse_cov_update = false;
     int power_reverse = 1;
+    double x_resident_mb = kXResidentDefaultMB;
     CovGeom stg{};
     PowGeom pw{};
     int n_cu = 256;
@@ -183,8 +184,17 @@
     return OIVA_OK;
 }
 
+XPolicy x_policy(const oiva_plan* p) { return choose_x_policy(p->x_resident_mb, p->T, p->F, p->M, p->cov_f64(), p->cov, p->pw); }
+CovGeom cov_geom_now(const oiva_plan* p) {
+    CovGeom g = p->cov;
+    g.xplain = x_policy(p).xplain();
+    return g;
+}
+
 int stage_power(oiva_plan* p) {
     PowGeom g = p->pw;
+    g.xplain = x_policy(p).xplain();
+    g.xctc = p->cov.tc;
     if (p->power_reverse) {
         g.rev = 1;
         if (g.rounds > 1 || p->power_reverse > 1) g.ord = make_pow_order(g.nsplit, g.tcp, p->cov.nsplit, p->cov.tc);
@@ -206,7 +216,7 @@
 }
 int stage_cov(oiva_plan* p) {
     OIVA_TRY_HIP(launch_cov(p->stream, p->X, p->X_pad, p->R, p->Wwide ? static_cast<float*>(p->Wwide) : p->Plocal , p->wscale, p->model,
-                       p->raw_weights, p->Vpart, p->cov_f64(), p->T, p->F, p->M, p->K, p->cov));
+                       p->raw_weights, p->Vpart, p->cov_f64(), p->T, p->F, p->M, p->K, cov_geom_now(p)));
     p->wscale_pending = !p->raw_weights;
     return OIVA_OK;
 }
@@ -519,6 +529,8 @@
         p->fuse_cov_update = u && u[0] == '1';
         const char* r = std::getenv("OIVA_POWER_REVERSE");
         p->power_reverse = (r && r[0] == '0') ? 0 : (r && r[0] == '2') ? 2 : 1;
+        const char* x = std::getenv("OIVA_X_RESIDENT_MB");
+        if (x && x[0]) p->x_resident_mb = std::atof(x);
     }
     choose_cov_geom(p, 0);
     choose_pow_geom(p, 0);
@@ -1124,6 +1136,19 @@
     return change_geometry(p, [&] { p->power_reverse = enable < 0 ? 0 : enable > 2 ? 2 : enable; return OIVA_OK; });
 }
 
+int oiva_plan_set_x_resident_mb(oiva_plan* p, double mb) {
+    OIVA_NEED(p, OIVA_ERR_ARG, "null plan");
+    OIVA_NEED(mb == mb, OIVA_ERR_ARG, "the budget is not a number");
+    return change_geometry(p, [&] { p->x_resident_mb = mb; return OIVA_OK; });
+}
+
+int oiva_plan_get_x_resident(oiva_plan* p, int* n16, int* nt, int* reason) {
+    OIVA_NEED(p && n16 && nt && reason, OIVA_ERR_ARG, "null argument");
+    const XPolicy x = x_policy(p);
+    *n16 = x.n16, *nt = x.nt ? 1 : 0, *reason = (int)x.why;
+    return OIVA_OK;
+}
+
 int oiva_plan_use_graph(oiva_plan* p, int enable) {
     OIVA_NEED(p, OIVA_ERR_ARG, "null plan");
     DeviceGuard guard(p->device);
@@ -1347,7 +1372,7 @@
             if (r) return r;
             OIVA_TRY_HIP(launch_activation(p->stream, p->Ppart, p->pw.nb, p->R, p->T, 1, amodel, p->F));
             OIVA_TRY_HIP(launch_cov(p->stream, p->X, p->X_pad, p->R, p->Plocal, p->wscale, p->model,  1, p->Vpart,
-                               p->cov_f64(), p->T, p->F, p->M, 1, p->cov));
+                               p->cov_f64(), p->T, p->F, p->M, 1, cov_geom_now(p)));
             OIVA_TRY_HIP(launch_ogive_step(p->stream, p->og, p->Vpart, p->vpart_f64(), p->cov.nsplit, p->T, p->F, p->M, step_size,
                                       tol));
         }
@@ -1540,6 +1565,49 @@
     return OIVA_OK;
 }
 
+int oiva_test_x_policy(int T, int F, int M, int cov_tc, int pow_tcp, double budget_mb, int* out, signed char* cov_walk, signed char* pow_walk) {
+    OIVA_NEED(out && cov_walk && pow_walk && T >= 1 && F >= 1 && M >= 1 && cov_tc >= 1 && pow_tcp >= 1, OIVA_ERR_ARG, "bad arguments");
+    CovGeom cg{};
+    cg.tc = cov_tc, cg.nsplit = ceil_div(T, cov_tc);
+    PowGeom pg{};
+    pg.tcp = pow_tcp, pg.nsplit = ceil_div(T, pow_tcp);
+    const XPolicy x = choose_x_policy(budget_mb, T, F, M, false, cg, pg);
+    out[0] = x.n16, out[1] = x.nt ? 1 : 0, out[2] = (int)x.why;
+    std::fill(cov_walk, cov_walk + T, (signed char)-1);
+    std::fill(pow_walk, pow_walk + T, (signed char)-1);
+    auto mark = [T](signed char* walk, int t, int frames, bool plain) {
+        for (int u = t; u < std::min(T, t + frames); ++u) walk[u] = walk[u] == -1 ? (plain ? 0 : 1) : 2;
+    };
+    const int xplain = x.xplain();
+    for (int t_begin = 0; t_begin < T; t_begin += cov_tc)
+        for (int i = 0; t_begin + 16 * i < std::min(T, t_begin + cov_tc); ++i)
+            mark(cov_walk, t_begin + 16 * i, std::min(16, cov_tc - 16 * i), x_group_plain(kXGroup * i, xplain));
+    for (int t_begin = 0; t_begin < T; t_begin += pow_tcp) {
+        const int off0 = t_begin % cov_tc;
+        for (int tl = 0; t_begin + tl < std::min(T, t_begin + pow_tcp); tl += 4)
+            mark(pow_walk, t_begin + tl, std::min(4, pow_tcp - tl), !x.nt || x_group_plain(x_split_offset(off0, tl, cov_tc), xplain));
+    }
+    return OIVA_OK;
+}
+
+int oiva_test_x_choice(int T, int F, int M, int prec_flags, int cov_kind, int cov_tc, int pow_kind, int pow_tcp, double budget_mb, int from_env, int* out,
+                       double* budget_used) {
+    OIVA_NEED(out && T >= 1 && F >= 1 && M >= 1 && cov_tc >= 1 && pow_tcp >= 1, OIVA_ERR_ARG, "bad arguments");
+    OIVA_NEED(cov_kind >= 0 && cov_kind < kCovKinds && pow_kind >= 0 && pow_kind < kPowKinds, OIVA_ERR_ARG, "unknown kernel kind");
+    if (from_env) {
+        const char* x = std::getenv("OIVA_X_RESIDENT_MB");
+        budget_mb = x && x[0] ? std::atof(x) : kXResidentDefaultMB;
+    }
+    CovGeom cg{};
+    cg.kind = (CovKind)cov_kind, cg.tc = cov_tc, cg.nsplit = ceil_div(T, cov_tc);
+    PowGeom pg{};
+    pg.kind = (PowKind)pow_kind, pg.tcp = pow_tcp, pg.nsplit = ceil_div(T, pow_tcp);
+    const XPolicy x = choose_x_policy(budget_mb, T, F, M, (prec_flags & OIVA_PREC_COV_F64) != 0, cg, pg);
+    out[0] = x.n16, out[1] = x.nt ? 1 : 0, out[2] = (int)x.why;
+    if (budget_used) *budget_used = budget_mb;
+    return OIVA_OK;
+}
+
 int oiva_test_kernel_choice(int device, int T, int F, int F_total, int M, int K, int prec_flags, int quad_on, int hmfma_on,
                             int cov_splits_req, int pow_splits_req, int* out) {
     OIVA_NEED(out && T >= 1 && F >= 1 && F_total >= F && M >= 1 && M <= OIVA_MAX_CHANNELS && K >= 1 && K <= M, OIVA_ERR_ARG, "bad arguments");
diff --git a/overiva_amd/plan.py b/overiva_amd/plan.py
--- a/overiva_amd/plan.py
+++ b/overiva_amd/plan.py
@@ -191,6 +191,16 @@
     def set_power_reverse(self, enable=True):
         _lib.check(self.lib.oiva_plan_set_power_reverse(self.h, int(enable)))
 
+    X_RESIDENT_REASONS = ("off", "fits", "kernels", "geometry", "share")
+
+    def set_x_resident_mb(self, mb):
+        _lib.check(self.lib.oiva_plan_set_x_resident_mb(self.h, float(mb)))
+
+    def x_resident(self):
+        n16, nt, why = C.c_int(), C.c_int(), C.c_int()
+        _lib.check(self.lib.oiva_plan_get_x_resident(self.h, C.byref(n16), C.byref(nt), C.byref(why)))
+        return n16.value, bool(nt.value), self.X_RESIDENT_REASONS[why.value]
+
     def use_graph(self, enable=True):
         _lib.check(self.lib.oiva_plan_use_graph(self.h, 1 if enable else 0))
 
@@ -305,11 +315,16 @@
                  "tcp", "kp", "rounds", "occ_cov", "occ_pow", "n_cu")
 
 
-def kernel_choice(T, F, M, K, mode="fast", F_total=None, cov_quad=True, cov_hmfma=True, cov_splits=0, pow_splits=0, device=0):
+def kernel_choice(T, F, M, K, mode="fast", F_total=None, cov_quad=True, cov_hmfma=True, cov_splits=0, pow_splits=0, device=0,
+                  x_resident_mb=None):
     flags = _lib.PREC_BY_NAME[mode] if isinstance(mode, str) else int(mode)
     out = (C.c_int * len(KERNEL_CHOICE))()
     _lib.check(_lib.load().oiva_test_kernel_choice(int(device), int(T), int(F), int(F if F_total is None else F_total), int(M), int(K),
                                                    flags, int(bool(cov_quad)), int(bool(cov_hmfma)), int(cov_splits), int(pow_splits), out))
     d = dict(zip(KERNEL_CHOICE, out))
+    x, mb = (C.c_int * 3)(), C.c_double()
+    _lib.check(_lib.load().oiva_test_x_choice(int(T), int(F), int(M), flags, d["cov_kind"], d["tc"], d["pow_kind"], d["tcp"],
+                                              0. if x_resident_mb is None else float(x_resident_mb), int(x_resident_mb is None), x, C.byref(mb)))
+    d["x_n16"], d["x_nt"], d["x_why"], d["x_budget_mb"] = x[0], bool(x[1]), Plan.X_RESIDENT_REASONS[x[2]], mb.value
     d["cov_kind"], d["unit_kind"], d["pow_kind"] = COV_KINDS[d["cov_kind"]], COV_KINDS[d["unit_kind"]], POW_KINDS[d["pow_kind"]]
     return d
```

Measured after the change: 5408, median of 6. +6.6%, better.
